# 4paradigm/OpenEmbedding

Measured on AMD Instinct MI355X. Metric: samples/sec DeepFM Criteo, higher is better.
Workload: dtype bf16; 1 GPU; model=deepfm-dim9, global_batch=4096, fields=26, dense_features=13, optimizer=adagrad, graph=True, prefetch=False, table=array, cache_mb=0, parallelism=single-gpu

## Files before the change

### openembedding_amd/core/tiered_gpu.py

```python

from __future__ import annotations

from typing import Optional

import torch

from .variable import VariableMeta, VariableShard
from .variable_gpu import HipVariableShard


class HipTieredVariableShard(HipVariableShard):
    HOST_INITIAL_ROWS = 1 << 14
    HOST_INITIAL_TABLE = 1 << 16

    def __init__(self, meta: VariableMeta, shard_id: int = 0,
                 shard_num: int = 1, device: str = "cuda", seed: int = 0,
                 cache_rows: int = 1 << 22):
        if not meta.use_hash_table:
            raise ValueError("the capacity tier requires hash mode")
        super().__init__(meta, shard_id, shard_num, device, seed)
        self.cache_rows = int(cache_rows)
        self.work_id = 0
        dev = self.device
        self._touch = torch.zeros(self.weights.shape[0] + 1,
                                  dtype=torch.int64, device=dev)
        self._host_cap = self.HOST_INITIAL_TABLE
        self.host_tk = torch.full((self._host_cap,), -1, dtype=torch.int64,
                                  device=dev)
        self.host_tv = torch.empty(self._host_cap, dtype=torch.int32,
                                   device=dev)
        self.host_nrows_dev = torch.zeros(1, dtype=torch.int32, device=dev)
        self.host_slot_keys = torch.empty(self.HOST_INITIAL_ROWS,
                                          dtype=torch.int64, device=dev)
        pin = torch.cuda.is_available()
        self._host_weights = torch.zeros((self.HOST_INITIAL_ROWS, self.dim),
                                         dtype=self.dtype, pin_memory=pin)
        self._host_state = torch.zeros((self.HOST_INITIAL_ROWS, 0),
                                       dtype=self.dtype, pin_memory=pin)
        self._host_rows_upper = 0
        self._host_live = False
        self._faulted = torch.zeros(1, dtype=torch.int32, device=dev)
        self._evict_epoch = 0
        self._last_batch_upper = 0
        self._evict_streak = 0
        self._checkpoint_work_id = None
        self._cache_full_since_ckpt = False


    def _host_ensure(self, rows: int) -> None:
        cap = self._host_weights.shape[0]
        if rows <= cap:
            return
        new_cap = max(rows, cap * 2)
        torch.cuda.synchronize()
        pin = torch.cuda.is_available()
        hw = torch.zeros((new_cap, self.dim), dtype=self.dtype,
                         pin_memory=pin)
        hw[:cap] = self._host_weights
        self._host_weights = hw
        hs = torch.zeros((new_cap, self._host_state.shape[1]),
                         dtype=self.dtype, pin_memory=pin)
        hs[:cap] = self._host_state
        self._host_state = hs
        sk = torch.empty(new_cap, dtype=torch.int64, device=self.device)
        sk[:self.host_slot_keys.shape[0]] = self.host_slot_keys
        self.host_slot_keys = sk

    def _host_maybe_rehash(self) -> None:
        if self._host_rows_upper * 2 <= self._host_cap:
            return
        new_cap = self._host_cap
        while self._host_rows_upper * 2 > new_cap:
            new_cap *= 2
        tk_new = torch.empty(new_cap, dtype=torch.int64, device=self.device)
        tv_new = torch.empty(new_cap, dtype=torch.int32, device=self.device)
        self.ext.ht_rehash(self.host_tk, self.host_tv, tk_new, tv_new)
        self.host_tk, self.host_tv = tk_new, tv_new
        self._host_cap = new_cap

    def set_optimizer(self, category: str, **cfg) -> None:
        super().set_optimizer(category, **cfg)
        if self._host_state.shape[1] != self.state_dim:
            if self._host_live:
                raise RuntimeError("cannot change optimizer state layout "
                                   "after rows were spilled to the host "
                                   "tier")
            pin = torch.cuda.is_available()
            self._host_state = torch.zeros(
                (self._host_weights.shape[0], self.state_dim),
                dtype=self.dtype, pin_memory=pin)

    def _ensure_rows(self, need: int) -> None:
        super()._ensure_rows(need)
        if self._touch.numel() < self.weights.shape[0] + 1:
            t = torch.zeros(self.weights.shape[0] + 1, dtype=torch.int64,
                            device=self.device)
            t[:self._touch.numel()] = self._touch
            self._touch = t

    def reserve_rows(self, rows: int) -> None:
        super().reserve_rows(min(int(rows), self.cache_rows))


    def _lookup_or_insert(self, keys: torch.Tensor, u_dev=None):
        if self._in_graph_capture():
            raise RuntimeError("the capacity tier is not hipGraph-"
                               "capturable (evictions need host control); "
                               "run eager with prefetch overlap")
        slots, new_mask = super()._lookup_or_insert(keys, u_dev)
        if self._host_live:
            self.ext.fault_in(keys, u_dev, self.host_tk, self.host_tv,
                              self._host_weights,
                              self._host_state if self.state_dim else None,
                              self.weights, self.state, slots, new_mask,
                              self._faulted)
        self._touch.scatter_(0, slots + 1, self.work_id)
        slots._oe_epoch = self._evict_epoch
        self._last_batch_upper = max(self._last_batch_upper, keys.numel())
        return slots, new_mask

    def push_slots(self, keys_buf, u_dev, slots, grads, counts) -> None:
        if getattr(slots, "_oe_epoch", self._evict_epoch) != self._evict_epoch:
            raise RuntimeError(
                "stale pull handle: the cache was compacted (eviction) "
                "after this pull; pull handles must be pushed before the "
                "commit that follows them")
        super().push_slots(keys_buf, u_dev, slots, grads, counts)

    def pull_readonly(self, keys: torch.Tensor) -> torch.Tensor:
        slots = self._lookup_readonly(keys)
        empty = torch.empty(0, dtype=torch.uint8, device=self.device)
        out = self.ext.gather_init(self.weights, self.state, slots, empty,
                                   keys, None, 0, 0.0, 0.0, 0.0, self.seed,
                                   torch.empty(0, dtype=self.dtype,
                                               device=self.device), True,
                                   None)
        if self._host_live:
            self.ext.gather_host(keys, slots, self.host_tk, self.host_tv,
                                 self._host_weights, out)
        return out

    fused_pooled_readonly = False

    def pull_pooled_readonly(self, values: torch.Tensor,
                             offsets: torch.Tensor, mode: str,
                             weights: torch.Tensor = None) -> torch.Tensor:
        return VariableShard.pull_pooled_readonly(self, values, offsets,
                                                  mode, weights)

    def update_weights(self) -> None:
        super().update_weights()
        self.work_id += 1
        if self._nrows_upper + self._last_batch_upper > self.cache_rows:
            self._evict()
        else:
            self._evict_streak = 0


    def _sync_nrows(self) -> None:
        self._nrows_exact = int(self.nrows_dev.item())
        self._nrows_upper = self._nrows_exact

    def _spill(self, evict_slots: torch.Tensor) -> None:
        n_ev = evict_slots.numel()
        if n_ev == 0:
            return
        keys = self.host_keys_of_slots(evict_slots)
        self._host_ensure(self._host_rows_upper + n_ev)
        self._host_rows_upper += n_ev
        self._host_maybe_rehash()
        hslots, _ = self.ext.ht_lookup(self.host_tk, self.host_tv, keys,
                                       self.host_nrows_dev,
                                       self.host_slot_keys, True, None)
        self.ext.spill_rows(evict_slots, hslots, self.weights, self.state,
                            self._host_weights,
                            self._host_state if self.state_dim else None)
        self._host_live = True
        self._host_rows_upper = int(self.host_nrows_dev.item())

    def host_keys_of_slots(self, slots: torch.Tensor) -> torch.Tensor:
        return self.slot_keys.index_select(0, slots)

    def _evict(self) -> None:
        self._sync_nrows()
        n = self._nrows_exact
        margin = self._last_batch_upper
        if n + margin <= self.cache_rows:
            return
        self._evict_streak += 1
        keep_frac = 4 if self._evict_streak >= 4 else (4 * 3)
        keep_target = max(1, (self.cache_rows * keep_frac) // 16 - margin)
        n_evict = n - keep_target
        if n_evict <= 0:
            return
        self._cache_full_since_ckpt = True
        touches = self._touch[1:n + 1]
        evict_slots = torch.topk(touches, n_evict, largest=False,
                                 sorted=False).indices
        evict_mask = torch.zeros(n, dtype=torch.bool, device=self.device)
        evict_mask[evict_slots] = True
        self._spill(evict_slots)
        keep_slots = (~evict_mask).nonzero(as_tuple=True)[0]
        kk = self.slot_keys.index_select(0, keep_slots)
        kw = self.weights.index_select(0, keep_slots)
        ks = (self.state.index_select(0, keep_slots)
              if self.state_dim else None)
        kt = touches.index_select(0, keep_slots)
        self.tk.fill_(-1)
        self.nrows_dev.zero_()
        self._nrows_upper = 0
        self._nrows_exact = 0
        m = keep_slots.numel()
        if m:
            slots, _ = self.ext.ht_lookup(self.tk, self.tv, kk,
                                          self.nrows_dev, self.slot_keys,
                                          True, None)
            self.weights[slots] = kw
            if ks is not None:
                self.state[slots] = ks
            self._touch.zero_()
            self._touch.scatter_(0, slots + 1, kt)
            self._nrows_exact = m
            self._nrows_upper = m
        else:
            self._touch.zero_()
        self._evict_epoch += 1


    def fault_count(self) -> int:
        return int(self._faulted.item())


    def should_persist(self) -> bool:
        return self._cache_full_since_ckpt and self._checkpoint_work_id is None

    def persist(self) -> int:
        self._sync_nrows()
        n = self._nrows_exact
        if n:
            self._spill(torch.arange(n, dtype=torch.int64,
                                     device=self.device))
        self._checkpoint_work_id = self.work_id
        self._cache_full_since_ckpt = False
        return self.work_id

    def checkpoint_committed(self) -> None:
        self._checkpoint_work_id = None

    def _host_only(self):
        hn = int(self.host_nrows_dev.item())
        if hn == 0:
            e = torch.empty(0, dtype=torch.int64, device=self.device)
            return e, e
        hkeys = self.host_slot_keys[:hn]
        cache_slots, _ = self.ext.ht_lookup(self.tk, self.tv, hkeys,
                                            self.nrows_dev, self.slot_keys,
                                            False, None)
        mask = cache_slots < 0
        return hkeys[mask], torch.arange(hn, device=self.device)[mask]

    @property
    def num_rows(self) -> int:
        n = int(self.nrows_dev.item())
        hkeys, _ = self._host_only()
        return n + hkeys.numel()

    def export_rows(self, include_state: bool = True):
        keys_c, w_c, s_c = super().export_rows(include_state)
        hkeys, hslots = self._host_only()
        if hkeys.numel() == 0:
            return keys_c, w_c, s_c
        hs_cpu = hslots.cpu()
        keys = torch.cat([keys_c, hkeys])
# ... 24 lines not shown
```

### openembedding_amd/core/variable_gpu.py

```python

from __future__ import annotations

from typing import Optional, Tuple

import torch

from ..ops import require_hip
from .variable import VariableMeta, VariableShard

_OPT_IDS = {"default": 0, "adadelta": 1, "adagrad": 2, "adam": 3,
            "adamax": 4, "ftrl": 5, "rmsprop": 6, "sgd": 7, "test": 8}

_INIT_IDS = {"constant": 0, "uniform": 1, "normal": 2}


def _opt_cfg_vector(opt) -> list:
    c = opt.cfg
    cat = opt.category
    if cat == "default":
        return [c["learning_rate"]]
    if cat == "adadelta":
        return [c["learning_rate"], c["rho"], c["epsilon"]]
    if cat == "adagrad":
        return [c["learning_rate"], c["initial_accumulator_value"], c["epsilon"]]
    if cat == "adam" or cat == "adamax":
        return [c["learning_rate"], c["beta_1"], c["beta_2"], c["epsilon"]]
    if cat == "ftrl":
        return [c["learning_rate"], c["l1_regularization_strength"],
                c["l2_regularization_strength"],
                c["l2_shrinkage_regularization_strength"],
                c["learning_rate_power"], c["beta"]]
    if cat == "rmsprop":
        return [c["learning_rate"], c["rho"], c["momentum"], c["epsilon"]]
    if cat == "sgd":
        return [c["learning_rate"], c["momentum"], 1.0 if c["nesterov"] else 0.0]
    if cat == "test":
        return [c["learning_rate"], c["flip"]]
    raise ValueError(cat)


def _init_params(init) -> Tuple[int, float, float, float]:
    cat = _INIT_IDS[init.category]
    c = init.cfg
    if init.category == "constant":
        return cat, c["value"], 0.0, 0.0
    if init.category == "uniform":
        return cat, c["minval"], c["maxval"], 0.0
    return cat, c["mean"], c["stddev"], c["truncated"]


class HipVariableShard(VariableShard):

    INITIAL_TABLE_CAP = 1 << 16
    INITIAL_ROW_CAP = 1 << 14
    fused_pooled_readonly = True

    def __init__(self, meta: VariableMeta, shard_id: int = 0, shard_num: int = 1,
                 device: str = "cuda", seed: int = 0):
        self.ext = require_hip()
        if self.ext is None:
            raise RuntimeError("HIP extension missing (OEAMD_ALLOW_TORCH_FALLBACK "
                               "cannot be used with HipVariableShard)")
        if meta.dtype != torch.float32:
            raise NotImplementedError("GPU shards are float32 (reference default); "
                                      "float64 runs on the CPU backend")
        super().__init__(meta, shard_id, shard_num, device, seed)
        self._pending_bounded = []
        dev = self.device
        if meta.use_hash_table:
            self._cap = self.INITIAL_TABLE_CAP
            self.tk = torch.full((self._cap,), -1, dtype=torch.int64, device=dev)
            self.tv = torch.empty(self._cap, dtype=torch.int32, device=dev)
            self.nrows_dev = torch.zeros(1, dtype=torch.int32, device=dev)
            self.slot_keys = torch.empty(self.INITIAL_ROW_CAP, dtype=torch.int64,
                                         device=dev)
            self.weights = torch.zeros((self.INITIAL_ROW_CAP, self.dim),
                                       dtype=self.dtype, device=dev)
            self.state = torch.zeros((self.INITIAL_ROW_CAP, 0),
                                     dtype=self.dtype, device=dev)
            self._nrows_upper = 0
            self._nrows_exact = 0
        else:
            self.valid_u8 = torch.zeros(self._array_cap, dtype=torch.uint8,
                                        device=dev)
            del self.valid


    def _ensure_rows(self, need: int) -> None:
        cap = self.weights.shape[0]
        if need <= cap:
            return
        new_cap = max(need, cap * 2)
        for name in ("weights", "state"):
            old = getattr(self, name)
            neww = torch.zeros((new_cap, old.shape[1]), dtype=self.dtype,
                               device=self.device)
            neww[:cap] = old
            setattr(self, name, neww)
        sk = torch.empty(new_cap, dtype=torch.int64, device=self.device)
        sk[:self.slot_keys.shape[0]] = self.slot_keys
        self.slot_keys = sk
        if self._tracking:
            self._grow_row_epoch(new_cap)

    def _maybe_rehash(self) -> None:
        if self._nrows_upper * 2 <= self._cap:
            return
        new_cap = self._cap
        while self._nrows_upper * 2 > new_cap:
            new_cap *= 2
        tk_new = torch.empty(new_cap, dtype=torch.int64, device=self.device)
        tv_new = torch.empty(new_cap, dtype=torch.int32, device=self.device)
        self.ext.ht_rehash(self.tk, self.tv, tk_new, tv_new)
        self.tk, self.tv, self._cap = tk_new, tv_new, new_cap


    def reserve_rows(self, rows: int) -> None:
        rows = int(rows)
        self._ensure_rows(max(rows, 1024))
        want_cap = 1 << max(16, (2 * rows - 1).bit_length())
        if want_cap > self._cap:
            old_upper = self._nrows_upper
            self._nrows_upper = want_cap // 2
            self._maybe_rehash()
            self._nrows_upper = old_upper
        self._reserved_rows = rows

    def _lookup_or_insert(self, keys: torch.Tensor, u_dev=None):
        n = keys.numel()
        if self.meta.use_hash_table:
            if self._in_graph_capture():
                if getattr(self, "_reserved_rows", 0) <= 0:
                    raise RuntimeError(
                        "hash-table insert path is not hipGraph-capturable "
                        "without reserve_rows()")
            else:
                self._ensure_rows(self._nrows_upper + n)
                self._maybe_rehash()
                self._nrows_upper += n
            slots, new_mask = self.ext.ht_lookup(self.tk, self.tv, keys,
                                                 self.nrows_dev, self.slot_keys,
                                                 True, u_dev)
        else:
            slots, new_mask = self.ext.array_touch(self.valid_u8, keys,
                                                   self.shard_num, u_dev)
        if self._tracking:
            self._mark(slots, new_mask, u_dev)
        return slots, new_mask

    def _mark(self, slots, mask=None, u_dev=None) -> None:
        self.ext.mark_rows(slots, mask, u_dev, self.epoch_dev,
                           self.row_epoch)

    def _apply(self, opt_id, slots, grads, counts, cfg, u_dev) -> None:
        self.ext.apply_optimizer(opt_id, self.weights, self.state, slots,
                                 grads.contiguous(), counts, cfg, u_dev)
        if self._tracking:
            self._mark(slots, None, u_dev)

    def _lookup_readonly(self, keys: torch.Tensor) -> torch.Tensor:
        if self.meta.use_hash_table:
            slots, _ = self.ext.ht_lookup(self.tk, self.tv, keys,
                                          self.nrows_dev, self.slot_keys,
                                          False, None)
            return slots
        slots = torch.div(keys, self.shard_num, rounding_mode="floor")
        hit = self.valid_u8[slots.clamp(0, self._array_cap - 1)] != 0
        return torch.where(hit, slots, torch.full_like(slots, -1))


    def _gather(self, keys, slots, new_mask, want_out: bool,
                inverse=None, u_dev=None) -> torch.Tensor:
        cat, p0, p1, p2 = _init_params(self.initializer)
        sir = self._state_init_row
        if sir is None:
            sir = self._make_state_init_row()
            self._state_init_row = sir
        return self.ext.gather_init(self.weights, self.state, slots,
                                    new_mask if new_mask is not None
                                    else torch.empty(0, dtype=torch.uint8,
                                                     device=self.device),
                                    keys, inverse, cat, p0, p1, p2, self.seed,
                                    sir.reshape(-1), want_out, u_dev)

    def pull(self, keys: torch.Tensor) -> torch.Tensor:
        slots, new_mask = self._lookup_or_insert(keys)
        return self._gather(keys, slots, new_mask, True)

    def pull_bounded(self, keys_buf: torch.Tensor, u_dev: torch.Tensor,
                     inverse: torch.Tensor):
        slots, new_mask = self._lookup_or_insert(keys_buf, u_dev)
        out = self._gather(keys_buf, slots, new_mask, True,
                           inverse=inverse, u_dev=u_dev)
        return out, slots

    def pull_pooled_bounded(self, keys_buf: torch.Tensor,
                            u_dev: torch.Tensor, inverse: torch.Tensor,
                            offsets: torch.Tensor, mode: int,
                            weights: torch.Tensor = None):
        slots, new_mask = self._lookup_or_insert(keys_buf, u_dev)
        self._gather(keys_buf, slots, new_mask, False, u_dev=u_dev)
        if weights is not None:
            out, bag_of, bag_scale = self.ext.pool_fwd_weighted(
                self.weights, inverse, slots, offsets, weights, mode)
            return out, slots, bag_of, bag_scale
        out, bag_of = self.ext.pool_fwd(self.weights, inverse, slots,
                                        offsets, mode, True)
        return out, slots, bag_of

    def pool_wgrad_slots(self, inverse: torch.Tensor, slots: torch.Tensor,
                         weights: torch.Tensor, bag_of: torch.Tensor,
                         bag_scale: torch.Tensor, out: torch.Tensor,
                         grad_out: torch.Tensor, mode: int) -> torch.Tensor:
        return self.ext.pool_wgrad(self.weights, inverse, slots, weights,
                                   bag_of, bag_scale, out, grad_out, mode)

    def push_slots(self, keys_buf, u_dev, slots, grads, counts) -> None:
        self._pending_bounded.append((keys_buf, u_dev, slots, grads, counts))

    def pull_readonly(self, keys: torch.Tensor) -> torch.Tensor:
        slots = self._lookup_readonly(keys)
        empty = torch.empty(0, dtype=torch.uint8, device=self.device)
        return self.ext.gather_init(self.weights, self.state, slots, empty,
                                    keys, None, 0, 0.0, 0.0, 0.0, self.seed,
                                    torch.empty(0, dtype=self.dtype,
                                                device=self.device), True,
                                    None)

    def pull_pooled_readonly(self, values: torch.Tensor,
                             offsets: torch.Tensor, mode: str,
                             weights: torch.Tensor = None) -> torch.Tensor:
        from ..ops.dispatch import POOL_MODES
        if mode not in POOL_MODES:
            raise ValueError(f"unknown pooling mode {mode!r}")
        if weights is not None:
            weights = weights.to(self.dtype).contiguous()
        values = values.contiguous()
        offsets = offsets.contiguous()
        if self.meta.use_hash_table:
            return self.ext.pool_lookup(self.weights, values, offsets,
                                        POOL_MODES[mode], weights,
                                        tk=self.tk, tv=self.tv)
        return self.ext.pool_lookup(self.weights, values, offsets,
                                    POOL_MODES[mode], weights,
                                    valid=self.valid_u8,
                                    shard_num=self.shard_num)

    def update_weights(self) -> None:
        if not self._pending and not self._pending_bounded:
            return
        if self.optimizer is None:
            raise RuntimeError("update_weights called before set_optimizer")
        opt_id = _OPT_IDS[self.optimizer.category]
        cfg = _opt_cfg_vector(self.optimizer)
        blocks = self._pending_bounded
        self._pending_bounded = []
        if len(blocks) > 1:
            blocks = [self._merge_bounded(blocks)]
        for keys_buf, u_dev, slots, grads, counts in blocks:
            self._apply(opt_id, slots, grads, counts, cfg, u_dev)
        if self._pending:
            if len(self._pending) == 1:
                keys, grads, counts = self._pending[0]
            else:
                keys0 = torch.cat([b[0] for b in self._pending])
                grads0 = torch.cat([b[1] for b in self._pending])
                counts0 = torch.cat([b[2] for b in self._pending])
                keys, inv = self.ext.unique_inverse(keys0)
                grads, _ = self.ext.reduce_by_inverse(inv, grads0, keys.numel())
                counts = torch.zeros(keys.numel(), dtype=counts0.dtype,
                                     device=self.device)
                counts.index_add_(0, inv, counts0)
            self._pending = []
            slots, new_mask = self._lookup_or_insert(keys)
            self._gather(keys, slots, new_mask, False)
            self._apply(opt_id, slots, grads, counts, cfg, None)
        if self.meta.use_hash_table and not self._in_graph_capture():
            self._commits = getattr(self, "_commits", 0) + 1
            if self._commits % 16 == 0 or self._nrows_upper > (
                    self.weights.shape[0] * 3) // 4:
                self._nrows_exact = int(self.nrows_dev.item())
                self._nrows_upper = self._nrows_exact

    def _merge_bounded(self, blocks):
        ks, ps = [], []
        for keys_buf, u_dev, slots, grads, counts in blocks:
            self.ext.mask_tail(keys_buf, grads, counts, u_dev)
            ks.append(keys_buf)
            ps.append(torch.cat([grads,
                                 counts.to(grads.dtype).unsqueeze(1)],
                                dim=1))
        keys = torch.cat(ks)
        payload = torch.cat(ps)
        uk, inv, u_dev = self.ext.unique_bounded(keys)
        g2c, _ = self.ext.reduce_by_inverse(inv, payload.contiguous(),
                                            keys.numel())
        g2, c2 = self.ext.split_payload(g2c, u_dev)
        slots, new_mask = self._lookup_or_insert(uk, u_dev)
        self._gather(uk, slots, new_mask, False, u_dev=u_dev)
        return uk, u_dev, slots, g2, c2

    @staticmethod
    def _in_graph_capture() -> bool:
        try:
            return torch.cuda.is_current_stream_capturing()
        except Exception:
            return False


    @property
    def num_rows(self) -> int:
        if self.meta.use_hash_table:
            return int(self.nrows_dev.item())
        return int((self.valid_u8 != 0).sum())

    def export_rows(self, include_state: bool = True):
        if self.meta.use_hash_table:
            n = int(self.nrows_dev.item())
            keys = self.slot_keys[:n].clone()
            w = self.weights[:n].clone()
            s = self.state[:n].clone() if (include_state and self.state_dim) else None
            return keys, w, s
        slots = (self.valid_u8 != 0).nonzero(as_tuple=True)[0]
        keys = slots * self.shard_num + self.shard_id
        w = self.weights[slots].clone()
        s = self.state[slots].clone() if (include_state and self.state_dim) else None
        return keys, w, s

    def import_rows(self, keys, weights, state=None):
        slots, new_mask = self._lookup_or_insert(keys)
        self._gather(keys, slots, new_mask, False)
        self.weights[slots] = weights.to(self.device, self.dtype)
        if state is not None and self.state_dim:
            self.state[slots] = state.to(self.device, self.dtype)
        if self._tracking:
            self._mark(slots)
        if self.meta.use_hash_table:
            self._nrows_exact = int(self.nrows_dev.item())
            self._nrows_upper = self._nrows_exact

    def get_weights(self, keys):
        return self.pull_readonly(keys)

    def clear(self) -> None:
        if self.meta.use_hash_table:
            self.tk.fill_(-1)
            self.nrows_dev.zero_()
            self._nrows_upper = 0
            self._nrows_exact = 0
        else:
            self.valid_u8.zero_()
            self.weights.zero_()
            self.state.zero_()
        if self._tracking:
            self.row_epoch.zero_()


    def track_changes(self, enable: bool = True) -> None:
        was = self._tracking
        super().track_changes(enable)
        if enable and not was:
            self.epoch_dev = torch.ones(1, dtype=torch.int32,
                                        device=self.device)

    def set_epoch(self, epoch: int, reset: bool = False) -> None:
        super().set_epoch(epoch, reset)
        self.epoch_dev.fill_(self._epoch)

    def select_changed(self, since: int):
        self._need_tracking()
        if self.meta.use_hash_table:
            return self.ext.select_changed(self.row_epoch, int(since),
                                           nrows_dev=self.nrows_dev)
        return self.ext.select_changed(self.row_epoch, int(since),
                                       valid=self.valid_u8)

    def export_changed(self, since: int, include_state: bool = True,
                       selection=None):
        from .. import checkpoint
        slots, n_dev = selection if selection is not None \
            else self.select_changed(since)
        n = n_dev if isinstance(n_dev, int) else int(n_dev.item())
        if not n:
            return
        if isinstance(n_dev, int):
            n_dev = torch.full((1,), n, dtype=torch.int32,
                               device=self.device)
        step = min(int(checkpoint.BLOCK_ROWS), n)
        want_state = bool(include_state and self.state_dim)
        k_out = torch.empty(step, dtype=torch.int64, device=self.device)
        w_out = torch.empty((step, self.dim), dtype=self.dtype,
                            device=self.device)
        state = self.state if want_state else self.state[:, :0]
        s_out = torch.empty((step, state.shape[1]), dtype=self.dtype,
                            device=self.device)
        hashed = self.meta.use_hash_table
        for start in range(0, n, step):
            cnt = min(step, n - start)
            self.ext.gather_rows_by_slot(
                self.weights, state,
                slot_keys=self.slot_keys if hashed else None,
                shard_num=self.shard_num, shard_id=self.shard_id,
                slots=slots, start=start, count=cnt, n_dev=n_dev,
                keys_out=k_out, w_out=w_out, s_out=s_out)
            yield (k_out[:cnt], w_out[:cnt],
                   s_out[:cnt] if want_state else None)


    def set_optimizer(self, category: str, **cfg) -> None:
# ... 8 lines not shown
```

### openembedding_amd/ops/csrc/bindings.cpp

```cpp

#include <torch/extension.h>
#include <ATen/cuda/CUDAContext.h>
#include <c10/cuda/CUDAGuard.h>

#include <cstdint>
#include <tuple>
#include <vector>

typedef unsigned long long u64;
typedef int64_t i64;
typedef struct ihipStream_t* hipStream_t_;

extern "C" {
void emb_unique(const i64*, long, u64*, int*, long, int*, unsigned char*,
                i64*, i64*, int*, const i64*, int, hipStream_t_);
void emb_unique_indexed(const i64*, long, u64*, int*, long, int*,
                        unsigned char*, i64*, i64*, int*, const i64*, int,
                        int*, int*, int*, int*, int*, int*, int*, long, int*,
                        int*, hipStream_t_);
int emb_seg_threshold();
int emb_seg_max_dim();
void emb_reduce_by_index(const int*, const int*, const int*, const int*,
                         const int*, long, const float*, long, long,
                         const int*, float*, u64*, hipStream_t_);
void emb_ht_lookup(u64*, int*, long, const i64*, long, int*, i64*, i64*,
                   unsigned char*, int, const int*, long, hipStream_t_);
void emb_ht_rehash(const u64*, const int*, long, u64*, int*, long,
                   hipStream_t_);
void emb_array_touch(unsigned char*, const i64*, long, long, long, i64*,
                     unsigned char*, const int*, hipStream_t_);
void emb_gather_init(float*, float*, long, long, const i64*,
                     const unsigned char*, const i64*, long, const i64*,
                     float*, int, float, float, float, u64, const float*,
                     const int*, hipStream_t_);
void emb_reduce_by_inverse(const i64*, const float*, long, long, float*, u64*,
                           long, hipStream_t_);
void emb_reduce_bags_by_inverse(const i64*, const float*, long, long,
                                const int*, const i64*, long, int, float*,
                                u64*, long, hipStream_t_);
void emb_pool_fwd(const float*, long, long, const i64*, long, const void*,
                  int, long, const i64*, long, int, float*, int*,
                  hipStream_t_);
void emb_pool_fwd_weighted(const float*, long, long, const i64*, long,
                           const void*, int, long, const i64*, long, int,
                           const float*, float*, int*, float*, hipStream_t_);
void emb_reduce_bags_weighted_by_inverse(const i64*, const float*, long, long,
                                         const int*, const float*,
                                         const float*, long, float*, u64*,
                                         long, hipStream_t_);
void emb_pool_wgrad(const float*, long, long, const i64*, long, const void*,
                    int, long, const float*, const int*, const float*,
                    const float*, const float*, long, int, float*,
                    hipStream_t_);
void emb_pool_lookup(const float*, long, long, const i64*, long, const i64*,
                     long, int, const float*, const u64*, const int*, long,
                     const unsigned char*, long, float*, hipStream_t_);
long emb_quant_stride(int, long);
void emb_quantize_rows(int, const float*, long, long, const i64*, void*,
                       long, hipStream_t_);
void emb_pool_lookup_q(int, const void*, long, long, const i64*, long,
                       const i64*, long, int, const float*, const u64*,
                       const int*, long, const unsigned char*, long, float*,
                       hipStream_t_);
void emb_gather_lookup_q(int, const void*, long, long, const i64*, long,
                         const u64*, const int*, long, const unsigned char*,
                         long, float*, hipStream_t_);
void emb_apply_optimizer(int, float*, float*, long, long, const i64*, long,
                         const float*, const u64*, const float*, const int*,
                         hipStream_t_);
void emb_ctr_head_fwd(const float*, const float*, const float*, const float*, long,
                      long, long, long, long, void*, float*, float*, int,
                      int, hipStream_t_);
void emb_ctr_head_bwd(const float*, const float*, const float*, const void*,
                      const float*, const float*, long, long, long, long,
                      long, float*, float*, float*, float*, int, int,
                      hipStream_t_);
void emb_mlp3_bias_bwd(const float*, const void*, const void*, const void*,
                       const void*, long, long, float*, void*, void*, void*,
                       void*, void*, int, int, hipStream_t_);
void emb_mlp3_wgrad(const void*, const void*, const void*, const void*,
                    const void*, const void*, long, long, long, long,
                    float*, void*, void*, void*, float*, long, hipStream_t_);
void emb_mlp3_pack(const void*, void*, long, long, long, long, int,
                   const void*, void*, long, long, long, long, int,
                   const void*, void*, long, long, long, long, int,
                   hipStream_t_);
void emb_bce_fwd(const float*, const float*, long, float*, hipStream_t_);
void emb_bce_bwd(const float*, const float*, long, const float*, float*,
                 hipStream_t_);
void emb_bucketize_pad(const i64*, long, const int*, long, long, i64*, int*,
                       int*, int*, int*, hipStream_t_);
void emb_mask_tail(i64*, float*, u64*, long, long, const int*, hipStream_t_);
void emb_mark_rows(const i64*, long, const unsigned char*, const int*,
                   const int*, int*, long, hipStream_t_);
long emb_delta_tile_rows();
long emb_delta_tiles(long);
void emb_delta_count(const int*, long, int, const int*, const unsigned char*,
                     int*, hipStream_t_);
void emb_delta_compact(const int*, long, int, const int*,
                       const unsigned char*, const int*, i64*, hipStream_t_);
void emb_delta_gather(const float*, const float*, long, long, long,
                      const i64*, long, long, const i64*, long, long, long,
                      const int*, i64*, float*, float*, hipStream_t_);
void emb_fault_in(const i64*, long, const int*, const u64*, const int*, long,
                  const float*, const float*, float*, float*, long, long,
                  const i64*, unsigned char*, int*, hipStream_t_);
void emb_spill_rows(const i64*, const i64*, long, const float*, const float*,
                    float*, float*, long, long, hipStream_t_);
void emb_gather_host(const i64*, long, const i64*, const u64*, const int*,
                     long, const float*, float*, long, hipStream_t_);
void emb_gather_pad(const float*, const u64*, long, const int*, long, float*,
                    hipStream_t_);
void emb_scatter_out(const float*, const i64*, long, const int*, long, float*,
                     hipStream_t_);
void emb_split_payload(const float*, long, long, const int*, float*, u64*,
                       hipStream_t_);
void emb_flat_step_scalars(float*, float, float, hipStream_t_);
void emb_flat_opt(int, void*, float*, float*, float*, void*,
                  const float*, long, int, float, float, float, float,
                  hipStream_t_);
void emb_flat_adagrad_f32(float*, float*, const float*, long, float, float,
                          hipStream_t_);
void emb_flat_adagrad_bf16(float*, float*, const void*, void*, long, float,
                           float, hipStream_t_);
void emb_cin_fwd(const float*, const float*, const void*, float*, long,
                 long, long, long, long, hipStream_t_);
void emb_cin_dw(const void*, const void*, const void*, float*, long, long,
                long, long, long, hipStream_t_);
void emb_cin_dx(const float*, const void*, const float*, const float*,
                float*, float*, long, long, long, long, long, hipStream_t_);
void emb_mlp3_fwd(const void*, long, long, const void*, const void*,
                  const void*, const void*, const void*, const void*,
                  const void*, const void*, const float*, long, long, void*,
                  void*, void*, float*, int, int, hipStream_t_);
void emb_mlp3_bwd(const float*, long, long, const void*, const void*,
                  const void*, const void*, const void*, const void*,
                  const void*, long, long, void*, void*, void*, void*,
                  float*, int, int, hipStream_t_);
void emb_mlp3_pack_frag(int, const void* const*, void* const*, const long*,
                        const long*, const long*, const long*, const long*,
                        const int*, hipStream_t_);
}

namespace {

using OptTensor = c10::optional<torch::Tensor>;

hipStream_t_ cur_stream() {
    return reinterpret_cast<hipStream_t_>(
        at::cuda::getCurrentCUDAStream().stream());
}

long next_pow2(long x) {
    long p = 16;
    while (p < x) p <<= 1;
    return p;
}

const int* u_ptr(const OptTensor& u_dev) {
    if (!u_dev.has_value()) return nullptr;
    TORCH_CHECK(u_dev->dtype() == torch::kInt32, "u_dev must be int32");
    return u_dev->data_ptr<int>();
}

#define CHECK_GPU(t) TORCH_CHECK((t).is_cuda(), #t " must be on GPU")
#define CHECK_CONT(t) TORCH_CHECK((t).is_contiguous(), #t " must be contiguous")


std::vector<torch::Tensor> unique_bounded_impl(
    torch::Tensor keys, OptTensor field_offsets, bool indexed) {
    CHECK_GPU(keys); CHECK_CONT(keys);
    TORCH_CHECK(keys.dtype() == torch::kInt64);
    const i64* foff = nullptr;
    int F = 0;
    if (field_offsets.has_value() && field_offsets->numel()) {
        CHECK_GPU(*field_offsets); CHECK_CONT(*field_offsets);
        TORCH_CHECK(field_offsets->dtype() == torch::kInt64,
                    "field_offsets must be int64");
        TORCH_CHECK(keys.numel() % field_offsets->numel() == 0,
                    "keys length must be a multiple of field_offsets");
        foff = field_offsets->data_ptr<i64>();
        F = (int)field_offsets->numel();
    }
    const c10::cuda::CUDAGuard guard(keys.device());
    long n = keys.numel();
    auto opts_i64 = keys.options();
    auto opts_i32 = keys.options().dtype(torch::kInt32);
    auto opts_u8 = keys.options().dtype(torch::kUInt8);
    long cap = next_pow2(2 * n);
    auto tk = torch::empty({cap}, opts_i64);
    auto tv = torch::empty({cap}, opts_i32);
    auto slot_of = torch::empty({n}, opts_i32);
    auto is_first = torch::empty({n}, opts_u8);
    auto uk = torch::empty({n}, opts_i64);
    auto inverse = torch::empty({n}, opts_i64);
    auto counter = torch::empty({1}, opts_i32);
    if (!indexed) {
        emb_unique(keys.data_ptr<i64>(), n, (u64*)tk.data_ptr<i64>(),
                   tv.data_ptr<int>(), cap, slot_of.data_ptr<int>(),
                   is_first.data_ptr<uint8_t>(), uk.data_ptr<i64>(),
                   inverse.data_ptr<i64>(), counter.data_ptr<int>(), foff, F,
                   cur_stream());
        return {uk, inverse, counter};
    }
    TORCH_CHECK(n < (1L << 31), "unique_bounded_indexed: n must fit int32");
    auto tct = torch::empty({2, cap}, opts_i32);
    auto segs = torch::empty({4, n}, opts_i32);
    long long_cap = n / (emb_seg_threshold() + 1) + 1;
    auto long_list = torch::empty({long_cap}, opts_i32);
    auto ctr = torch::empty({32}, opts_i32);
    auto seg_off = segs.select(0, 0), seg_cnt = segs.select(0, 1);
    auto perm = segs.select(0, 2), rank = segs.select(0, 3);
    auto n_long = ctr.narrow(0, 16, 1);
    emb_unique_indexed(keys.data_ptr<i64>(), n, (u64*)tk.data_ptr<i64>(),
                       tv.data_ptr<int>(), cap, slot_of.data_ptr<int>(),
                       is_first.data_ptr<uint8_t>(), uk.data_ptr<i64>(),
                       inverse.data_ptr<i64>(), counter.data_ptr<int>(), foff,
                       F, tct.data_ptr<int>(), tct.data_ptr<int>() + cap,
                       rank.data_ptr<int>(), seg_off.data_ptr<int>(),
                       seg_cnt.data_ptr<int>(), perm.data_ptr<int>(),
                       long_list.data_ptr<int>(), long_cap,
                       ctr.data_ptr<int>(), n_long.data_ptr<int>(),
                       cur_stream());
    return {uk, inverse, counter, seg_off, seg_cnt, perm, long_list, n_long};
}

std::tuple<torch::Tensor, torch::Tensor, torch::Tensor> unique_bounded(
    torch::Tensor keys, OptTensor field_offsets) {
    auto r = unique_bounded_impl(keys, field_offsets, false);
    return {r[0], r[1], r[2]};
}

std::tuple<torch::Tensor, torch::Tensor, torch::Tensor, torch::Tensor,
           torch::Tensor, torch::Tensor, torch::Tensor, torch::Tensor>
unique_bounded_indexed(torch::Tensor keys, OptTensor field_offsets) {
    auto r = unique_bounded_impl(keys, field_offsets, true);
    return {r[0], r[1], r[2], r[3], r[4], r[5], r[6], r[7]};
}

std::tuple<torch::Tensor, torch::Tensor> unique_inverse(torch::Tensor keys) {
    auto r = unique_bounded(keys, c10::nullopt);
    long u = std::get<2>(r).item<int>();
    return {std::get<0>(r).narrow(0, 0, u), std::get<1>(r)};
}


std::tuple<torch::Tensor, torch::Tensor> ht_lookup(
    torch::Tensor tk, torch::Tensor tv, torch::Tensor keys,
    torch::Tensor nrows, torch::Tensor slot_keys, bool insert,
    OptTensor u_dev) {
    CHECK_GPU(keys); CHECK_CONT(keys);
    const c10::cuda::CUDAGuard guard(keys.device());
    long n = keys.numel();
    auto slots = torch::empty({n}, keys.options());
    auto new_mask = torch::empty({n}, keys.options().dtype(torch::kUInt8));
    if (n)
        emb_ht_lookup((u64*)tk.data_ptr<i64>(), tv.data_ptr<int>(),
                      tk.numel(), keys.data_ptr<i64>(), n,
                      nrows.data_ptr<int>(), slot_keys.data_ptr<i64>(),
                      slots.data_ptr<i64>(), new_mask.data_ptr<uint8_t>(),
                      insert ? 1 : 0, u_ptr(u_dev), slot_keys.numel(),
                      cur_stream());
    return {slots, new_mask};
}

void ht_rehash(torch::Tensor tk_old, torch::Tensor tv_old, torch::Tensor tk_new,
               torch::Tensor tv_new) {
    const c10::cuda::CUDAGuard guard(tk_old.device());
    emb_ht_rehash((u64*)tk_old.data_ptr<i64>(), tv_old.data_ptr<int>(),
                  tk_old.numel(), (u64*)tk_new.data_ptr<i64>(),
                  tv_new.data_ptr<int>(), tk_new.numel(), cur_stream());
}


std::tuple<torch::Tensor, torch::Tensor> array_touch(
    torch::Tensor valid, torch::Tensor keys, int64_t shard_num,
    OptTensor u_dev) {
    const c10::cuda::CUDAGuard guard(valid.device());
    long n = keys.numel();
    auto slots = torch::empty({n}, keys.options());
    auto new_mask = torch::empty({n}, keys.options().dtype(torch::kUInt8));
    if (n)
        emb_array_touch(valid.data_ptr<uint8_t>(), keys.data_ptr<i64>(), n,
                        shard_num, valid.numel(), slots.data_ptr<i64>(),
                        new_mask.data_ptr<uint8_t>(), u_ptr(u_dev),
                        cur_stream());
    return {slots, new_mask};
}


torch::Tensor gather_init(torch::Tensor weights, torch::Tensor state,
                          torch::Tensor slots, torch::Tensor new_mask,
                          torch::Tensor keys, OptTensor inverse,
                          int64_t init_cat, double p0, double p1, double p2,
                          int64_t seed, torch::Tensor state_init_row,
                          bool want_out, OptTensor u_dev) {
    CHECK_GPU(weights); CHECK_CONT(weights);
    const c10::cuda::CUDAGuard guard(weights.device());
    long n = inverse.has_value() ? inverse->numel() : keys.numel();
    long dim = weights.size(1);
    long sd = state.numel() ? state.size(1) : 0;
    torch::Tensor out;
    float* out_ptr = nullptr;
    if (want_out) {
        out = torch::empty({n, dim}, weights.options());
        out_ptr = out.data_ptr<float>();
    } else {
        out = torch::empty({0}, weights.options());
    }
    if (init_cat == 1) p1 = p1 - p0;
    emb_gather_init(weights.data_ptr<float>(),
                    sd ? state.data_ptr<float>() : nullptr, dim, sd,
                    slots.data_ptr<i64>(),
                    new_mask.numel() ? new_mask.data_ptr<uint8_t>() : nullptr,
                    keys.data_ptr<i64>(), n,
                    inverse.has_value() ? inverse->data_ptr<i64>() : nullptr,
                    out_ptr, (int)init_cat,
                    (float)p0, (float)p1, (float)p2, (u64)seed,
                    sd ? state_init_row.data_ptr<float>() : nullptr,
                    u_ptr(u_dev), cur_stream());
    return out;
}


std::tuple<torch::Tensor, torch::Tensor> reduce_by_inverse(
    torch::Tensor inverse, torch::Tensor grads, int64_t u) {
    CHECK_GPU(grads); CHECK_CONT(grads);
    TORCH_CHECK(grads.dtype() == torch::kFloat32,
                "reduce_by_inverse: grads must be float32");
    const c10::cuda::CUDAGuard guard(grads.device());
    long n = grads.size(0);
    long dim = grads.size(1);
    auto ugrads = torch::empty({u, dim}, grads.options());
    auto counts = torch::empty({u}, grads.options().dtype(torch::kInt64));
    emb_reduce_by_inverse(inverse.data_ptr<i64>(), grads.data_ptr<float>(), n,
                          dim, ugrads.data_ptr<float>(),
                          (u64*)counts.data_ptr<i64>(), u, cur_stream());
    return {ugrads, counts};
}

std::tuple<torch::Tensor, torch::Tensor> reduce_by_index(
    torch::Tensor seg_off, torch::Tensor seg_cnt, torch::Tensor perm,
    torch::Tensor long_list, torch::Tensor n_long, torch::Tensor grads,
    torch::Tensor u_dev) {
    CHECK_GPU(grads); CHECK_CONT(grads);
    TORCH_CHECK(grads.dtype() == torch::kFloat32 && grads.dim() == 2,
                "reduce_by_index: grads must be float32 [n, dim]");
    long n = grads.size(0);
    long dim = grads.size(1);
    TORCH_CHECK(dim <= emb_seg_max_dim(),
                "reduce_by_index: dim above the kernel's ladder");
    for (const auto* t : {&seg_off, &seg_cnt, &perm, &long_list, &n_long,
                          &u_dev}) {
        CHECK_GPU(*t); CHECK_CONT(*t);
        TORCH_CHECK(t->dtype() == torch::kInt32,
                    "reduce_by_index: index tensors must be int32");
    }
    TORCH_CHECK(seg_off.numel() == n && seg_cnt.numel() == n
                && perm.numel() == n,
                "reduce_by_index: index does not match grads");
    TORCH_CHECK(n_long.numel() == 1 && u_dev.numel() == 1);
    const c10::cuda::CUDAGuard guard(grads.device());
    auto ugrads = torch::empty({n, dim}, grads.options());
    auto counts = torch::empty({n}, grads.options().dtype(torch::kInt64));
    emb_reduce_by_index(seg_off.data_ptr<int>(), seg_cnt.data_ptr<int>(),
                        perm.data_ptr<int>(), long_list.data_ptr<int>(),
                        n_long.data_ptr<int>(), long_list.numel(),
                        grads.data_ptr<float>(), n, dim,
                        u_dev.data_ptr<int>(), ugrads.data_ptr<float>(),
                        (u64*)counts.data_ptr<i64>(), cur_stream());
    return {ugrads, counts};
}


std::tuple<torch::Tensor, torch::Tensor> pool_fwd(
    torch::Tensor rows, OptTensor inverse, OptTensor map,
    torch::Tensor offsets, int64_t mode, bool want_bag_of) {
    CHECK_GPU(rows); CHECK_CONT(rows);
    CHECK_GPU(offsets); CHECK_CONT(offsets);
    TORCH_CHECK(rows.dtype() == torch::kFloat32 && rows.dim() == 2,
                "pool_fwd: rows must be float32 [R, dim]");
    TORCH_CHECK(offsets.dtype() == torch::kInt64 && offsets.dim() == 1
                && offsets.numel() >= 1,
                "pool_fwd: offsets must be int64 [B+1]");
    TORCH_CHECK(mode >= 0 && mode <= 2, "pool_fwd: bad mode");
    const void* map_ptr = nullptr;
    int map_kind = 0;
    long u = 0;
    if (map.has_value()) {
        CHECK_GPU(*map); CHECK_CONT(*map);
        u = map->numel();
        if (map->dtype() == torch::kInt64) {
            map_kind = 1;
            map_ptr = map->data_ptr<i64>();
        } else {
            TORCH_CHECK(map->dtype() == torch::kInt32,
                        "pool_fwd: map must be int64 or int32");
            map_kind = 2;
            map_ptr = map->data_ptr<int>();
        }
    }
    long R = rows.size(0), dim = rows.size(1);
    long nnz = map_kind ? u : R;
    const i64* inv_ptr = nullptr;
    if (inverse.has_value()) {
        CHECK_GPU(*inverse); CHECK_CONT(*inverse);
        TORCH_CHECK(inverse->dtype() == torch::kInt64,
                    "pool_fwd: inverse must be int64");
        nnz = inverse->numel();
        inv_ptr = inverse->data_ptr<i64>();
    }
    const c10::cuda::CUDAGuard guard(rows.device());
    long B = offsets.numel() - 1;
    auto out = torch::empty({B, dim}, rows.options());
    auto bag_of = torch::empty({want_bag_of ? nnz : 0},
                               rows.options().dtype(torch::kInt32));
    emb_pool_fwd(rows.data_ptr<float>(), R, dim, inv_ptr, nnz, map_ptr,
                 map_kind, u, offsets.data_ptr<i64>(), B, (int)mode,
                 out.data_ptr<float>(),
                 want_bag_of ? bag_of.data_ptr<int>() : nullptr,
                 cur_stream());
    return {out, bag_of};
}

std::tuple<torch::Tensor, torch::Tensor> reduce_bags_by_inverse(
    torch::Tensor inverse, torch::Tensor grad_out, torch::Tensor bag_of,
    torch::Tensor offsets, int64_t mode, int64_t u) {
    CHECK_GPU(grad_out); CHECK_CONT(grad_out);
    CHECK_GPU(inverse); CHECK_CONT(inverse);
    CHECK_GPU(bag_of); CHECK_CONT(bag_of);
    CHECK_GPU(offsets); CHECK_CONT(offsets);
    TORCH_CHECK(grad_out.dtype() == torch::kFloat32 && grad_out.dim() == 2,
                "reduce_bags_by_inverse: grad_out must be float32 [B, dim]");
    TORCH_CHECK(inverse.dtype() == torch::kInt64
                && bag_of.dtype() == torch::kInt32
                && offsets.dtype() == torch::kInt64,
                "reduce_bags_by_inverse dtypes");
    TORCH_CHECK(bag_of.numel() == inverse.numel(),
                "reduce_bags_by_inverse: bag_of/inverse length mismatch");
    TORCH_CHECK(offsets.numel() == grad_out.size(0) + 1,
                "reduce_bags_by_inverse: offsets must be [B+1]");
    TORCH_CHECK(mode >= 0 && mode <= 2, "reduce_bags_by_inverse: bad mode");
    const c10::cuda::CUDAGuard guard(grad_out.device());
    long n = inverse.numel();
    long B = grad_out.size(0);
    long dim = grad_out.size(1);
    auto ugrads = torch::empty({u, dim}, grad_out.options());
    auto counts = torch::empty({u}, grad_out.options().dtype(torch::kInt64));
    emb_reduce_bags_by_inverse(inverse.data_ptr<i64>(),
                               grad_out.data_ptr<float>(), n, dim,
                               bag_of.data_ptr<int>(),
                               offsets.data_ptr<i64>(), B, (int)mode,
                               ugrads.data_ptr<float>(),
                               (u64*)counts.data_ptr<i64>(), u,
                               cur_stream());
    return {ugrads, counts};
}


struct PoolChain {
    const i64* inv_ptr = nullptr;
    const void* map_ptr = nullptr;
    int map_kind = 0;
    long u = 0, nnz = 0;
};

static PoolChain pool_chain(const char* who, const torch::Tensor& rows,
                            const OptTensor& inverse, const OptTensor& map) {
    PoolChain c;
    if (map.has_value()) {
        CHECK_GPU(*map); CHECK_CONT(*map);
        c.u = map->numel();
        if (map->dtype() == torch::kInt64) {
            c.map_kind = 1;
            c.map_ptr = map->data_ptr<i64>();
        } else {
            TORCH_CHECK(map->dtype() == torch::kInt32, who,
                        ": map must be int64 or int32");
            c.map_kind = 2;
            c.map_ptr = map->data_ptr<int>();
        }
    }
    c.nnz = c.map_kind ? c.u : rows.size(0);
    if (inverse.has_value()) {
        CHECK_GPU(*inverse); CHECK_CONT(*inverse);
        TORCH_CHECK(inverse->dtype() == torch::kInt64, who,
                    ": inverse must be int64");
        c.nnz = inverse->numel();
        c.inv_ptr = inverse->data_ptr<i64>();
    }
    return c;
}

std::tuple<torch::Tensor, torch::Tensor, torch::Tensor> pool_fwd_weighted(
    torch::Tensor rows, OptTensor inverse, OptTensor map,
    torch::Tensor offsets, torch::Tensor weights, int64_t mode,
    OptTensor out_buf, OptTensor scale_buf) {
    CHECK_GPU(rows); CHECK_CONT(rows);
    CHECK_GPU(offsets); CHECK_CONT(offsets);
    CHECK_GPU(weights); CHECK_CONT(weights);
    TORCH_CHECK(rows.dtype() == torch::kFloat32 && rows.dim() == 2
                && rows.size(1) >= 1,
                "pool_fwd_weighted: rows must be float32 [R, dim >= 1]");
    TORCH_CHECK(offsets.dtype() == torch::kInt64 && offsets.dim() == 1
                && offsets.numel() >= 1,
                "pool_fwd_weighted: offsets must be int64 [B+1]");
    TORCH_CHECK(mode >= 0 && mode <= 2, "pool_fwd_weighted: bad mode");
    PoolChain c = pool_chain("pool_fwd_weighted", rows, inverse, map);
    TORCH_CHECK(weights.dtype() == torch::kFloat32 && weights.dim() == 1
                && weights.numel() == c.nnz,
                "pool_fwd_weighted: weights must be float32 [nnz]");
    const c10::cuda::CUDAGuard guard(rows.device());
    long R = rows.size(0), dim = rows.size(1);
    long B = offsets.numel() - 1;
    auto out = out_buf.has_value() ? *out_buf
                                   : torch::empty({B, dim}, rows.options());
    auto bag_scale = scale_buf.has_value()
        ? *scale_buf : torch::empty({B}, rows.options());
    CHECK_GPU(out); CHECK_CONT(out);
    CHECK_GPU(bag_scale); CHECK_CONT(bag_scale);
    TORCH_CHECK(out.dtype() == torch::kFloat32 && out.dim() == 2
                && out.size(0) == B && out.size(1) == dim,
                "pool_fwd_weighted: out must be float32 [B, dim]");
    TORCH_CHECK(bag_scale.dtype() == torch::kFloat32
// ... 860 lines not shown
    for (size_t i = 0; i < n; i++) {
        const torch::Tensor &s = srcs[i], &d = dsts[i];
        CHECK_GPU(s); CHECK_GPU(d); CHECK_CONT(d);
        TORCH_CHECK(s.dtype() == torch::kBFloat16
                    && d.dtype() == torch::kBFloat16
                    && s.dim() == 2 && d.dim() == 2 && s.stride(1) == 1
                    && s.stride(0) >= s.size(1)
                    && s.device() == d.device(),
                    "mlp3_pack_frag dtypes/shapes");
        rows[i] = s.size(0); cols[i] = s.size(1); sld[i] = s.stride(0);
        N[i] = d.size(0); Kp[i] = d.size(1);
        tt[i] = trans[i];
        TORCH_CHECK(N[i] > 0 && N[i] % 16 == 0 && Kp[i] > 0
                    && Kp[i] % 32 == 0,
                    "mlp3_pack_frag: dst must be [x16, x32]");
        TORCH_CHECK((tt[i] ? cols[i] : rows[i]) <= N[i]
                    && (tt[i] ? rows[i] : cols[i]) <= Kp[i],
                    "mlp3_pack_frag: dst too small");
        TORCH_CHECK(N[i] * Kp[i] < (1L << 31)
                    && rows[i] * sld[i] < (1L << 31),
                    "mlp3_pack_frag: 32-bit indices");
        TORCH_CHECK((reinterpret_cast<uintptr_t>(d.data_ptr()) & 15) == 0,
                    "mlp3_pack_frag: dst must be 16-byte aligned");
        sp[i] = s.data_ptr(); dp[i] = d.data_ptr();
    }
    const c10::cuda::CUDAGuard guard(srcs[0].device());
    emb_mlp3_pack_frag((int)n, sp, dp, rows, cols, sld, N, Kp, tt,
                       cur_stream());
}


torch::Tensor bce_fwd(torch::Tensor logits, torch::Tensor labels) {
    CHECK_GPU(logits); CHECK_CONT(logits); CHECK_CONT(labels);
    TORCH_CHECK(logits.dtype() == torch::kFloat32 &&
                labels.dtype() == torch::kFloat32, "bce_fwd wants fp32");
    TORCH_CHECK(logits.numel() == labels.numel(), "logits/labels mismatch");
    const c10::cuda::CUDAGuard guard(logits.device());
    auto loss = torch::empty({}, logits.options());
    emb_bce_fwd(logits.data_ptr<float>(), labels.data_ptr<float>(),
                logits.numel(), loss.data_ptr<float>(), cur_stream());
    return loss;
}

torch::Tensor bce_bwd(torch::Tensor logits, torch::Tensor labels,
                      torch::Tensor grad_out) {
    CHECK_GPU(logits); CHECK_CONT(logits); CHECK_CONT(labels);
    TORCH_CHECK(grad_out.numel() == 1, "grad_out must be scalar");
    const c10::cuda::CUDAGuard guard(logits.device());
    auto g = torch::empty_like(logits);
    emb_bce_bwd(logits.data_ptr<float>(), labels.data_ptr<float>(),
                logits.numel(), grad_out.contiguous().data_ptr<float>(),
                g.data_ptr<float>(), cur_stream());
    return g;
}


std::tuple<torch::Tensor, torch::Tensor, torch::Tensor, torch::Tensor>
mlp3_fwd(torch::Tensor x0, torch::Tensor w1, torch::Tensor b1,
         torch::Tensor w2, torch::Tensor b2, torch::Tensor w3,
         torch::Tensor b3, torch::Tensor w4, torch::Tensor b4,
         c10::optional<torch::Tensor> partial, long bm, bool frag) {
    CHECK_GPU(x0); CHECK_CONT(x0);
    TORCH_CHECK(x0.dtype() == torch::kBFloat16, "mlp3_fwd: x0 must be bf16");
    const c10::cuda::CUDAGuard guard(x0.device());
    long M = x0.size(0), K0p = x0.size(1), H = w1.size(0);
    long Hp = w2.size(1);
    TORCH_CHECK(H % 16 == 0 && H <= 416, "mlp3_fwd: H must be <=416, x16");
    TORCH_CHECK(K0p % 32 == 0 && Hp % 32 == 0,
                "mlp3_fwd: padded K dims must be x32");
    TORCH_CHECK(w1.size(1) == K0p && w2.size(0) == H && w3.size(0) == H
                && w3.size(1) == Hp && w4.numel() == H);
    TORCH_CHECK(bm == 0 || bm == 16 || ((bm == 32 || bm == 64)
                                        && K0p <= 416),
                "mlp3_fwd: bm must be 0, 16, 32 or 64 (32/64: K0p <= 416)");
    if (frag) {
        CHECK_CONT(w1); CHECK_CONT(w2); CHECK_CONT(w3);
    }
    auto a1 = torch::empty({M, H}, x0.options());
    auto a2 = torch::empty({M, H}, x0.options());
    auto a3 = torch::empty({M, H}, x0.options());
    auto out = torch::empty({M}, x0.options().dtype(torch::kFloat32));
    const float* pp = nullptr;
    if (partial.has_value()) {
        TORCH_CHECK(partial->is_contiguous() && partial->numel() == M &&
                    partial->dtype() == torch::kFloat32,
                    "mlp3_fwd: partial must be contiguous fp32 [M]");
        pp = partial->data_ptr<float>();
    }
    emb_mlp3_fwd(x0.data_ptr(), M, K0p,
                 w1.data_ptr(), b1.data_ptr(), w2.data_ptr(), b2.data_ptr(),
                 w3.data_ptr(), b3.data_ptr(), w4.data_ptr(), b4.data_ptr(),
                 pp, H, Hp, a1.data_ptr(), a2.data_ptr(), a3.data_ptr(),
                 out.data_ptr<float>(), (int)bm, (int)frag, cur_stream());
    return {out, a1, a2, a3};
}

std::tuple<torch::Tensor, torch::Tensor, torch::Tensor, torch::Tensor>
mlp3_bwd(torch::Tensor dout, torch::Tensor a1, torch::Tensor a2,
         torch::Tensor a3, torch::Tensor w4, torch::Tensor w3t,
         torch::Tensor w2t, torch::Tensor w1t, OptTensor bias_scratch,
         long bm, bool frag) {
    CHECK_GPU(dout); CHECK_CONT(dout); CHECK_CONT(w3t); CHECK_CONT(w2t);
    CHECK_CONT(w1t);
    const c10::cuda::CUDAGuard guard(dout.device());
    long M = a1.size(0), H = a1.size(1), K0p = w1t.size(0);
    long Hp = w3t.size(1);
    TORCH_CHECK(Hp % 32 == 0 && w2t.size(1) == Hp && w1t.size(1) == Hp);
    TORCH_CHECK(H % 16 == 0 && H <= 416 && K0p % 16 == 0,
                "mlp3_bwd: H must be <=416, x16");
    TORCH_CHECK(bm == 0 || bm == 16 || bm == 32 || bm == 64,
                "mlp3_bwd: bm must be 0, 16, 32 or 64");
    auto dz1 = torch::empty_like(a1);
    auto dz2 = torch::empty_like(a2);
    auto dz3 = torch::empty_like(a3);
    auto dx0 = torch::empty({M, K0p}, a1.options());
    float* bptr = nullptr;
    if (bias_scratch.has_value()) {
        CHECK_CONT(*bias_scratch);
        TORCH_CHECK(bias_scratch->numel() >= 4 * H + 1
                    && bias_scratch->dtype() == torch::kFloat32,
                    "bias_scratch layout");
        bptr = bias_scratch->data_ptr<float>();
    }
    emb_mlp3_bwd(dout.data_ptr<float>(), M, K0p, a1.data_ptr(),
                 a2.data_ptr(), a3.data_ptr(), w4.data_ptr(), w3t.data_ptr(),
                 w2t.data_ptr(), w1t.data_ptr(), H, Hp, dz1.data_ptr(),
                 dz2.data_ptr(), dz3.data_ptr(), dx0.data_ptr(), bptr,
                 (int)bm, (int)frag, cur_stream());
    return {dx0, dz1, dz2, dz3};
}

}

PYBIND11_MODULE(TORCH_EXTENSION_NAME, m) {
    m.def("unique_inverse", &unique_inverse, "hash-based unique+inverse");
    m.def("unique_bounded", &unique_bounded,
          "unique+inverse without host sync (n-sized buffer + device "
          "count); optional fused per-field key offsets",
          pybind11::arg("keys"),
          pybind11::arg("field_offsets") = pybind11::none());
    m.def("ht_lookup", &ht_lookup, "hash table lookup/insert");
    m.def("ht_rehash", &ht_rehash, "hash table rehash into larger table");
    m.def("array_touch", &array_touch,
          "array-table slot compute + valid-bitmap touch");
    m.def("gather_init", &gather_init,
          "row gather with fused lazy init (+ optional duplicate scatter)");
    m.def("reduce_by_inverse", &reduce_by_inverse,
          "grad reduce-by-key with counts (LDS-aggregated)");
    m.def("unique_bounded_indexed", &unique_bounded_indexed,
          "unique_bounded plus the batch's inverted index (seg_off, "
          "seg_cnt, perm, long_list, n_long)",
          pybind11::arg("keys"),
          pybind11::arg("field_offsets") = pybind11::none());
    m.def("reduce_by_index", &reduce_by_index,
          "grad reduce-by-key with counts through the inverted index "
          "(segmented, no atomics)");
    m.def("seg_reduce_threshold", &emb_seg_threshold,
          "list length above which a uid is in long_list");
    m.def("seg_reduce_max_dim", &emb_seg_max_dim,
          "widest dim reduce_by_index covers");
    m.def("pool_fwd", &pool_fwd,
          "segment-pooled gather (sum/mean/sqrtn) over ragged bags; also "
          "emits each element's bag for the backward",
          pybind11::arg("rows"), pybind11::arg("inverse"),
          pybind11::arg("map"), pybind11::arg("offsets"),
          pybind11::arg("mode"), pybind11::arg("want_bag_of") = true);
    m.def("reduce_bags_by_inverse", &reduce_bags_by_inverse,
          "grad reduce-by-key reading the pooled [B, dim] gradient through "
          "bag_of (no [nnz, dim] expansion)");
    m.def("pool_fwd_weighted", &pool_fwd_weighted,
          "pool_fwd with per-sample weights; also emits bag_of and the "
          "per-bag combiner scale for the backward",
          pybind11::arg("rows"), pybind11::arg("inverse"),
          pybind11::arg("map"), pybind11::arg("offsets"),
          pybind11::arg("weights"), pybind11::arg("mode"),
          pybind11::arg("out") = pybind11::none(),
          pybind11::arg("bag_scale") = pybind11::none());
    m.def("reduce_bags_weighted_by_inverse",
          &reduce_bags_weighted_by_inverse,
          "bag-indirected grad reduce with the per-element factor "
          "weights[e] * bag_scale[bag_of[e]]");
    m.def("pool_wgrad", &pool_wgrad,
          "gradient of the weighted pool w.r.t. its per-sample weights",
          pybind11::arg("rows"), pybind11::arg("inverse"),
          pybind11::arg("map"), pybind11::arg("weights"),
          pybind11::arg("bag_of"), pybind11::arg("bag_scale"),
          pybind11::arg("out"), pybind11::arg("grad_out"),
          pybind11::arg("mode"), pybind11::arg("dw") = pybind11::none());
    m.def("pool_lookup", &pool_lookup,
          "read-only pooled lookup, keys -> pooled rows in one launch "
          "(hash: tk/tv; array: valid/shard_num)",
          pybind11::arg("rows"), pybind11::arg("values"),
          pybind11::arg("offsets"), pybind11::arg("mode"),
          pybind11::arg("weights") = pybind11::none(),
          pybind11::arg("tk") = pybind11::none(),
          pybind11::arg("tv") = pybind11::none(),
          pybind11::arg("valid") = pybind11::none(),
          pybind11::arg("shard_num") = 1);
    m.def("quantize_rows", &quantize_rows,
          "fp32 rows -> packed rows at the given slots of a slab (slots "
          "unique within a call)",
          pybind11::arg("w"), pybind11::arg("slots"), pybind11::arg("slab"),
          pybind11::arg("fmt"));
    m.def("pool_lookup_q", &pool_lookup_q,
          "read-only pooled lookup over a packed slab, keys -> pooled fp32 "
          "rows in one launch (hash: tk/tv; array: valid/shard_num)",
          pybind11::arg("slab"), pybind11::arg("dim"), pybind11::arg("fmt"),
          pybind11::arg("values"), pybind11::arg("offsets"),
          pybind11::arg("mode"),
          pybind11::arg("weights") = pybind11::none(),
          pybind11::arg("tk") = pybind11::none(),
          pybind11::arg("tv") = pybind11::none(),
          pybind11::arg("valid") = pybind11::none(),
          pybind11::arg("shard_num") = 1);
    m.def("gather_lookup_q", &gather_lookup_q,
          "flat read over a packed slab, keys -> fp32 rows in one launch",
          pybind11::arg("slab"), pybind11::arg("dim"), pybind11::arg("fmt"),
          pybind11::arg("keys"),
          pybind11::arg("tk") = pybind11::none(),
          pybind11::arg("tv") = pybind11::none(),
          pybind11::arg("valid") = pybind11::none(),
          pybind11::arg("shard_num") = 1);
    m.def("apply_optimizer", &apply_optimizer, "fused sparse optimizer step");
    m.def("mask_tail", &mask_tail,
          "zero the garbage tail of a bounded block (enables multi-block "
          "merge by concatenation)");
    m.def("mark_rows", &mark_rows,
          "delta checkpoints: row_epoch[slot] = *epoch_dev for the named "
          "rows (optional byte mask and device count)",
          pybind11::arg("slots"), pybind11::arg("mask") = pybind11::none(),
          pybind11::arg("u_dev") = pybind11::none(),
          pybind11::arg("epoch_dev"), pybind11::arg("row_epoch"));
    m.attr("DELTA_TILE_ROWS") = emb_delta_tile_rows();
    m.def("select_changed", &select_changed,
          "delta checkpoints: ascending slots of the live rows with "
          "row_epoch >= since -> (slots [R] with a -1 tail, n_dev int32[1])",
          pybind11::arg("row_epoch"), pybind11::arg("since"),
          pybind11::arg("nrows_dev") = pybind11::none(),
          pybind11::arg("valid") = pybind11::none());
    m.def("gather_rows_by_slot", &gather_rows_by_slot,
          "delta checkpoints: keys, weights and state of "
          "slots[start:start+count] into staging buffers",
          pybind11::arg("weights"), pybind11::arg("state"),
          pybind11::arg("slot_keys") = pybind11::none(),
          pybind11::arg("shard_num") = 1, pybind11::arg("shard_id") = 0,
          pybind11::arg("slots"), pybind11::arg("start"),
          pybind11::arg("count"), pybind11::arg("n_dev"),
          pybind11::arg("keys_out") = pybind11::none(),
          pybind11::arg("w_out") = pybind11::none(),
          pybind11::arg("s_out") = pybind11::none());
    m.def("fault_in", &fault_in,
          "tier v2: copy host-resident rows into fresh cache slots, "
          "clearing their lazy-init mask");
    m.def("spill_rows", &spill_rows,
          "tier v2: copy cache rows into the pinned host slab");
    m.def("gather_host", &gather_host,
          "tier v2: read-only host-row gather for cache misses");
    m.def("bucketize_pad", &bucketize_pad,
          "owner-bucketize unique keys into a fixed padded [world, cap] "
          "wire block (sync-free multi-rank route)");
    m.def("gather_pad", &gather_pad,
          "gather grads+counts payload into the padded send layout");
    m.def("scatter_out", &scatter_out,
          "padded pull: wire rows -> per-element output (fused dup scatter)");
    m.def("split_payload", &split_payload,
          "split owner-reduced payload into grads + int64 counts");
    m.def("ctr_head_fwd", &ctr_head_fwd,
          "fused CTR head fwd: deep_in assembly (+cast) + FM + first-order "
          "+ dense linear");
    m.def("ctr_head_bwd", &ctr_head_bwd, "fused CTR head backward");
    m.def("mlp3_bwd", &mlp3_bwd,
          "fused dgrad chain backward of the 3-layer MLP (optionally "
          "carrying the head wgrad/bias sums)",
          pybind11::arg("dout"), pybind11::arg("a1"), pybind11::arg("a2"),
          pybind11::arg("a3"), pybind11::arg("w4"), pybind11::arg("w3t"),
          pybind11::arg("w2t"), pybind11::arg("w1t"),
          pybind11::arg("bias_scratch") = pybind11::none(),
          pybind11::arg("bm") = 0, pybind11::arg("frag") = false);
    m.def("mlp3_pack", &mlp3_pack,
          "refresh three padded (or transposed) weight copies in one "
          "launch");
    m.def("mlp3_pack_frag", &mlp3_pack_frag,
          "write up to six fragment-major weight images (pads included) "
          "in one launch",
          pybind11::arg("srcs"), pybind11::arg("dsts"),
          pybind11::arg("trans"));
    m.def("mlp3_fwd", &mlp3_fwd,
          "fused 3-hidden-layer MLP forward (bf16 MFMA, bias+ReLU fused)",
          pybind11::arg("x0"), pybind11::arg("w1"), pybind11::arg("b1"),
          pybind11::arg("w2"), pybind11::arg("b2"), pybind11::arg("w3"),
          pybind11::arg("b3"), pybind11::arg("w4"), pybind11::arg("b4"),
          pybind11::arg("partial"), pybind11::arg("bm") = 0,
          pybind11::arg("frag") = false);
    m.def("mlp3_wgrad", &mlp3_wgrad,
          pybind11::arg("dz1"), pybind11::arg("dz2"), pybind11::arg("dz3"),
          pybind11::arg("x0"), pybind11::arg("a1"), pybind11::arg("a2"),
          pybind11::arg("scratch"), pybind11::arg("dw1"),
          pybind11::arg("dw2"), pybind11::arg("dw3"),
          pybind11::arg("bias_scratch") = pybind11::none(),
          pybind11::arg("m_split") = 0,
          "all three MLP weight grads in one MFMA launch (+= into bf16 "
          "grads via fp32 scratch)");
    m.def("mlp3_bias_bwd", &mlp3_bias_bwd,
          "MLP bias grads + head wgrad in one pass over the dz mirrors "
          "(with_dz=false when the fused wgrad carried the dz sums)",
          pybind11::arg("dout"), pybind11::arg("dz1"), pybind11::arg("dz2"),
          pybind11::arg("dz3"), pybind11::arg("a3"),
          pybind11::arg("scratch"), pybind11::arg("db1"),
          pybind11::arg("db2"), pybind11::arg("db3"), pybind11::arg("dw4"),
// ... 19 lines not shown
```

### openembedding_amd/ops/csrc/embops.hip

```cpp

#include <hip/hip_runtime.h>
#include <cstdint>

#define DEV static __device__ __forceinline__

typedef unsigned long long u64;
typedef long long i64;

static constexpr u64 EMPTY = ~0ull;
static constexpr int BLOCK = 256;

static inline int cdiv(long a, long b) { return (int)((a + b - 1) / b); }
static inline int grid1d(long n) {
    long g = (n + BLOCK - 1) / BLOCK;
    return (int)(g < 1 ? 1 : g);
}


template <typename T>
__global__ void k_fill(T* __restrict__ p, long n, T v) {
    long i = (long)blockIdx.x * blockDim.x + threadIdx.x;
    if (i < n) p[i] = v;
}

// ... 31 lines not shown
    long i = (long)blockIdx.x * blockDim.x + threadIdx.x;
    if (i < cap) {
        tk[i] = ~0ull;
        if constexpr (IDX) ix.tcount[i] = 0;
    }
    if (i < n) is_first[i] = 0;
    if (i == 0) {
        *counter = 0;
        if constexpr (IDX) { *ix.off_counter = 0; *ix.n_long = 0; }
    }
}

__global__ void k_reduce_reset(float* __restrict__ ugrads, long ne,
                               u64* __restrict__ counts, long u) {
    long i = (long)blockIdx.x * blockDim.x + threadIdx.x;
    if (i < ne) ugrads[i] = 0.0f;
    if (i < u) counts[i] = 0ull;
}

__global__ void k_pad_reset(u64* __restrict__ send_keys,
                            int* __restrict__ send_src, long total,
                            int* __restrict__ counts, long world) {
    long i = (long)blockIdx.x * blockDim.x + threadIdx.x;
    if (i < total) { send_keys[i] = ~0ull; send_src[i] = -1; }
    if (i < world) counts[i] = 0;
}


DEV u64 splitmix64(u64 z) {
    z += 0x9E3779B97F4A7C15ull;
    z = (z ^ (z >> 30)) * 0xBF58476D1CE4E5B9ull;
    z = (z ^ (z >> 27)) * 0x94D049BB133111EBull;
    return z ^ (z >> 31);
}

DEV u64 uniform_bits(u64 seed, u64 key, u64 col, u64 attempt) {
    u64 x = key * 0x100000ull + col + (attempt << 40);
    return splitmix64(splitmix64(x) ^ seed);
}

DEV float uniform01(u64 seed, u64 key, u64 col, u64 attempt) {
    return (float)(uniform_bits(seed, key, col, attempt) >> 40)
           * (1.0f / 16777216.0f);
}

enum { INIT_CONSTANT = 0, INIT_UNIFORM = 1, INIT_NORMAL = 2 };

DEV float normal01(u64 seed, u64 key, u64 col, u64 attempt) {
    float u1 = uniform01(seed, key, col, 2 * attempt);
    float u2 = uniform01(seed, key, col, 2 * attempt + 1);
    float r = sqrtf(-2.0f * logf(1.0f - u1));
    return r * cosf(2.0f * 3.14159265358979323846f * u2);
}

DEV float init_value(int cat, float p0, float p1, float p2,
                     u64 seed, u64 key, u64 col) {
    if (cat == INIT_CONSTANT) return p0;
    if (cat == INIT_UNIFORM) {
        float u = uniform01(seed, key, col, 0);
        return p0 + u * p1;
    }
    float z = normal01(seed, key, col, 0);
    if (p2 > 0.1f) {
        for (int attempt = 1; attempt < 16 && z > p2; ++attempt)
            z = normal01(seed, key, col, attempt);
    }
    return p0 + p1 * z;
}


#define ULDS 1024
#define UA_ITERS 8
#define UI_ILP 4
#define SEG_T 32

template <bool IDX>
__global__ void k_unique_insert(const i64* __restrict__ keys, long n,
                                u64* __restrict__ tk, long mask,
                                int* __restrict__ slot_of,
                                unsigned char* __restrict__ is_first,
                                const i64* __restrict__ foff, int F,
                                UIdx ix) {
    __shared__ u64 lkeys[ULDS];
    __shared__ int lslot[ULDS];
    __shared__ int lcnt[IDX ? ULDS : 1];
    __shared__ int lbase[IDX ? ULDS : 1];
    for (int t = threadIdx.x; t < ULDS; t += blockDim.x) {
        lkeys[t] = EMPTY;
        if constexpr (IDX) lcnt[t] = 0;
    }
    __syncthreads();

    long i = (long)blockIdx.x * blockDim.x + threadIdx.x;
    u64 k = 0;
    i64 kin = 0;
    if (i < n) {
        kin = keys[i];
        if (foff) kin += foff[(int)i % F];
    }
    int lh = -1;
    int lr = 0;
    bool lds_winner = false, lds_ok = false;
    if (i < n && (u64)kin == EMPTY) {
        is_first[i] = 1;
        slot_of[i] = -1;
    } else if (i < n) {
        k = (u64)kin;
        u64 hh = splitmix64(k);
        lh = (int)(hh & (ULDS - 1));
        for (int probes = 0; probes < 64; ++probes) {
            u64 cur = atomicCAS(&lkeys[lh], EMPTY, k);
            if (cur == EMPTY) { lds_winner = true; lds_ok = true; break; }
            if (cur == k) { lds_ok = true; break; }
            lh = (lh + 1) & (ULDS - 1);
        }
        if constexpr (IDX)
            if (lds_ok) lr = atomicAdd(&lcnt[lh], 1);
        if (lds_winner || !lds_ok) {
            u64 h = splitmix64(k) & (u64)mask;
            long found = -1;
            for (long p = 0; p <= mask; ++p) {
                u64 cur = tk[h];
                if (cur == k) { found = (long)h; break; }
                if (cur == EMPTY) {
                    u64 prev = atomicCAS(&tk[h], EMPTY, k);
                    if (prev == EMPTY) {
                        is_first[i] = 1; found = (long)h; break;
                    }
                    if (prev == k) { found = (long)h; break; }
                }
                h = (h + 1) & (u64)mask;
            }
            if (found < 0) is_first[i] = 1;
            slot_of[i] = found >= 0 ? (int)found : -1;
            if (lds_winner)
                lslot[lh] = found >= 0 ? (int)found : (int)(-2 - i);
            if constexpr (IDX)
                if (!lds_ok && found >= 0)
                    lr = atomicAdd(&ix.tcount[found], 1);
        }
    }
    __syncthreads();
    if (i < n && lds_ok && !lds_winner) slot_of[i] = lslot[lh];
    if constexpr (IDX) {
        if (lds_winner) {
            int s = lslot[lh];
            lbase[lh] = s >= 0 ? atomicAdd(&ix.tcount[s], lcnt[lh]) : 0;
        }
        __syncthreads();
        if (i < n) ix.rank[i] = lds_ok ? lbase[lh] + lr : lr;
    }
}

template <bool IDX>
__global__ void k_unique_assign(const i64* __restrict__ keys, long n,
                                const int* __restrict__ slot_of,
                                const unsigned char* __restrict__ is_first,
                                int* __restrict__ tv,
                                i64* __restrict__ unique_keys,
                                int* __restrict__ counter,
                                i64* __restrict__ inverse,
                                const i64* __restrict__ foff, int F,
                                UIdx ix) {
    const int lane = threadIdx.x & 63;
    const long stride = (long)gridDim.x * blockDim.x;
    long i0 = (long)blockIdx.x * blockDim.x + threadIdx.x;
    u64 ballots[UA_ITERS];
    int sl[IDX ? UA_ITERS : 1], c[IDX ? UA_ITERS : 1];
    int total = 0;
    #pragma unroll
    for (int t = 0; t < UA_ITERS; ++t) {
        long i = i0 + t * stride;
        if constexpr (IDX) sl[t] = (i < n) ? slot_of[i] : -1;
        bool first = (i < n) && is_first[i];
        ballots[t] = __ballot(first);
        total += __popcll(ballots[t]);
    }
    if (!total) return;
    int off = 0, wtot = 0;
    if constexpr (IDX) {
        int ctot = 0;
        #pragma unroll
        for (int t = 0; t < UA_ITERS; ++t) {
            c[t] = (ballots[t] >> lane & 1ull)
                       ? (sl[t] >= 0 ? ix.tcount[sl[t]] : 1) : 0;
            ctot += c[t];
        }
        int inc = ctot;
        #pragma unroll
        for (int d = 1; d < 64; d <<= 1) {
            int v = __shfl_up(inc, d, 64);
            if (lane >= d) inc += v;
        }
        wtot = __shfl(inc, 63, 64);
        off = inc - ctot;
    }
    int base = 0, obase = 0;
    if (lane == 0) {
        base = atomicAdd(counter, total);
        if constexpr (IDX) obase = atomicAdd(ix.off_counter, wtot);
    }
    base = __shfl(base, 0, 64);
    if constexpr (IDX) off += __shfl(obase, 0, 64);
    #pragma unroll
    for (int t = 0; t < UA_ITERS; ++t) {
        u64 b = ballots[t];
        if (b & (1ull << lane)) {
            long i = i0 + t * stride;
            int uid = base + __popcll(b & ((1ull << lane) - 1ull));
            i64 kin = keys[i];
            if (foff) kin += foff[(int)i % F];
            unique_keys[uid] = kin;
            int s;
            if constexpr (IDX) s = sl[t]; else s = slot_of[i];
            if (s >= 0) tv[s] = uid;
            else inverse[i] = uid;
            if constexpr (IDX) {
                ix.seg_off[uid] = off;
                ix.seg_cnt[uid] = c[t];
                if (s >= 0) ix.toff[s] = off;
                else if (off >= 0 && off < n) ix.perm[off] = (int)i;
                if (c[t] > SEG_T) {
                    int q = atomicAdd(ix.n_long, 1);
                    if (q < ix.long_cap) ix.long_list[q] = uid;
                }
                off += c[t];
            }
        }
        base += __popcll(b);
    }
}

template <bool IDX>
__global__ void k_unique_inverse(long n, const int* __restrict__ slot_of,
                                 const int* __restrict__ tv,
                                 i64* __restrict__ inverse, UIdx ix) {
    const long stride = (long)gridDim.x * blockDim.x;
    long i0 = (long)blockIdx.x * blockDim.x + threadIdx.x;
    int s[UI_ILP];
    #pragma unroll
    for (int t = 0; t < UI_ILP; ++t) {
        long i = i0 + t * stride;
        s[t] = (i < n) ? slot_of[i] : -1;
    }
    int v[UI_ILP];
    int r[IDX ? UI_ILP : 1], o[IDX ? UI_ILP : 1];
    #pragma unroll
    for (int t = 0; t < UI_ILP; ++t) {
        v[t] = (s[t] >= 0) ? tv[s[t]] : 0;
        if constexpr (IDX) {
            o[t] = (s[t] >= 0) ? ix.toff[s[t]] : 0;
            r[t] = (s[t] >= 0) ? ix.rank[i0 + t * stride] : 0;
        }
    }
    #pragma unroll
    for (int t = 0; t < UI_ILP; ++t) {
        long i = i0 + t * stride;
        if (i >= n) continue;
        if constexpr (IDX) {
            long p = (long)o[t] + r[t];
            if (s[t] >= 0 && p >= 0 && p < n) ix.perm[p] = (int)i;
        }
        if (s[t] >= 0) inverse[i] = (i64)v[t];
        else if (s[t] <= -2) inverse[i] = inverse[-2 - s[t]];
    }
}


__global__ void k_ht_lookup(u64* __restrict__ tk, int* __restrict__ tv,
                            long mask, const i64* __restrict__ keys, long n,
                            int* __restrict__ nrows,
                            i64* __restrict__ slot_keys,
                            i64* __restrict__ slots,
                            unsigned char* __restrict__ new_mask,
                            int insert, const int* __restrict__ u_dev,
                            long row_cap) {
    long i = (long)blockIdx.x * blockDim.x + threadIdx.x;
    if (i >= n) return;
    if (u_dev && i >= *u_dev) {
        slots[i] = -1;
        if (new_mask) new_mask[i] = 0;
        return;
    }
    u64 k = (u64)keys[i];
    if (k == EMPTY) {
        slots[i] = -1;
        if (new_mask) new_mask[i] = 0;
        return;
    }
    u64 h = splitmix64(k) & (u64)mask;
    i64 slot = -1;
    unsigned char is_new = 0;
    for (long p = 0; p <= mask; ++p) {
        u64 cur = tk[h];
        if (cur == k) { slot = (i64)tv[h]; break; }
        if (cur == EMPTY) {
            if (!insert) { slot = -1; break; }
            u64 prev = atomicCAS(&tk[h], EMPTY, k);
            if (prev == EMPTY) {
                int s = atomicAdd(nrows, 1);
                if (s >= row_cap) {
                    tv[h] = -1;
                    slot = -1;
                    break;
                }
                tv[h] = s;
                slot_keys[s] = (i64)k;
                slot = s;
                is_new = 1;
                break;
            }
            if (prev == k) { slot = (i64)tv[h]; break; }
        }
        h = (h + 1) & (u64)mask;
    }
    slots[i] = slot;
    if (new_mask) new_mask[i] = is_new;
}

__global__ void k_ht_rehash(const u64* __restrict__ tk_old,
                            const int* __restrict__ tv_old, long cap_old,
                            u64* __restrict__ tk_new, int* __restrict__ tv_new,
                            long mask_new) {
    long i = (long)blockIdx.x * blockDim.x + threadIdx.x;
    if (i >= cap_old) return;
    u64 k = tk_old[i];
    if (k == EMPTY) return;
    u64 h = splitmix64(k) & (u64)mask_new;
    for (long p = 0; p <= mask_new; ++p) {
        u64 prev = atomicCAS(&tk_new[h], EMPTY, k);
        if (prev == EMPTY) { tv_new[h] = tv_old[i]; return; }
        h = (h + 1) & (u64)mask_new;
    }
}


__global__ void k_array_touch(unsigned char* __restrict__ valid,
                              const i64* __restrict__ keys, long n,
                              long shard_num, long cap,
                              i64* __restrict__ slots,
                              unsigned char* __restrict__ new_mask,
                              const int* __restrict__ u_dev) {
    long i = (long)blockIdx.x * blockDim.x + threadIdx.x;
    if (i >= n) return;
    if (u_dev && i >= *u_dev) { slots[i] = -1; new_mask[i] = 0; return; }
    if (keys[i] < 0) {
        slots[i] = -1;
        new_mask[i] = 0;
        return;
    }
    i64 s = keys[i] / shard_num;
    if (s < 0 || s >= cap) s = -1;
    slots[i] = s;
    if (s < 0) { new_mask[i] = 0; return; }
    unsigned char was = valid[s];
    valid[s] = 1;
    new_mask[i] = !was;
}


#define GI_ILP 4
template <int G>
__global__ void k_gather_init(float* __restrict__ weights,
                              float* __restrict__ state,
                              long dim, long sd,
                              const i64* __restrict__ slots,
                              const unsigned char* __restrict__ new_mask,
                              const i64* __restrict__ keys, long n,
                              const i64* __restrict__ inverse,
                              float* __restrict__ out,
                              int init_cat, float p0, float p1, float p2,
                              u64 seed,
                              const float* __restrict__ state_init_row,
                              const int* __restrict__ u_dev) {
    const long stride = ((long)gridDim.x * blockDim.x) / G;
    long g0 = ((long)blockIdx.x * blockDim.x + threadIdx.x) / G;
    const int lane = threadIdx.x % G;
    const int live = u_dev ? *u_dev : 0;

    long uid[GI_ILP];
    i64 slot[GI_ILP];
    unsigned char nm[GI_ILP];
    u64 key[GI_ILP];
    #pragma unroll
    for (int t = 0; t < GI_ILP; ++t) {
        long g = g0 + t * stride;
        bool act = g < n && !(!inverse && u_dev && g >= live);
        uid[t] = act ? (inverse ? inverse[g] : g) : -1;
    }
    #pragma unroll
    for (int t = 0; t < GI_ILP; ++t)
        slot[t] = (uid[t] >= 0) ? slots[uid[t]] : -1;
    #pragma unroll
    for (int t = 0; t < GI_ILP; ++t) {
        nm[t] = (uid[t] >= 0 && new_mask) ? new_mask[uid[t]] : 0;
        key[t] = (uid[t] >= 0 && nm[t]) ? (u64)keys[uid[t]] : 0;
    }
    #pragma unroll
    for (int t = 0; t < GI_ILP; ++t) {
        long g = g0 + t * stride;
        if (uid[t] < 0)
            continue;
        if (slot[t] < 0) {
            if (out)
                for (long j = lane; j < dim; j += G) out[g * dim + j] = 0.0f;
            continue;
        }
        float* wrow = weights + (u64)slot[t] * dim;
        if (nm[t]) {
            for (long j = lane; j < dim; j += G) {
                float v = init_value(init_cat, p0, p1, p2, seed, key[t],
                                     (u64)j);
                wrow[j] = v;
                if (out) out[g * dim + j] = v;
            }
            if (sd > 0) {
                float* srow = state + (u64)slot[t] * sd;
                for (long j = lane; j < sd; j += G)
                    srow[j] = state_init_row[j];
            }
        } else if (out) {
            for (long j = lane; j < dim; j += G)
                out[g * dim + j] = wrow[j];
        }
    }
}


enum { POOL_SUM = 0, POOL_MEAN = 1, POOL_SQRTN = 2 };

DEV long pool_clamp(i64 v, long nnz) {
    return v < 0 ? 0 : (v > (i64)nnz ? nnz : (long)v);
}

DEV float pool_scale(int mode, long len) {
    if (len <= 0) return 0.0f;
    if (mode == POOL_MEAN) return 1.0f / (float)len;
    if (mode == POOL_SQRTN) return 1.0f / sqrtf((float)len);
    return 1.0f;
}

DEV float pool_wscale(int mode, float den) {
    if (mode == POOL_SUM) return 1.0f;
    if (den == 0.0f) return 0.0f;
    return mode == POOL_MEAN ? 1.0f / den : 1.0f / sqrtf(den);
}


template <typename MapT>
DEV long pool_row(long j, long e, const i64* __restrict__ inverse,
                  const MapT* __restrict__ map, long nidx, long R) {
    if (j >= e) return -1;
    long uid = inverse ? (long)inverse[j] : j;
    if (uid < 0 || uid >= nidx) return -1;
    long row = map ? (long)map[uid] : uid;
    return (row >= 0 && row < R) ? row : -1;
}

template <typename MapT>
struct PoolChain {
    const i64* __restrict__ inverse;
    const MapT* __restrict__ map;
    long nidx, R;
    __device__ __forceinline__ long operator()(long j, long e) const {
        return pool_row(j, e, inverse, map, nidx, R);
    }
};

struct PoolHashKeys {
    const i64* __restrict__ values;
    const u64* __restrict__ tk;
    const int* __restrict__ tv;
    long mask, R;
    __device__ __forceinline__ long operator()(long j, long e) const {
        if (j >= e) return -1;
        const u64 k = (u64)values[j];
        if (k == EMPTY) return -1;
        u64 h = splitmix64(k) & (u64)mask;
        for (long p = 0; p <= mask; ++p) {
            const u64 cur = tk[h];
            if (cur == k) {
                const long row = (long)tv[h];
                return (row >= 0 && row < R) ? row : -1;
            }
            if (cur == EMPTY) return -1;
            h = (h + 1) & (u64)mask;
        }
        return -1;
    }
};

struct PoolArrayKeys {
    const i64* __restrict__ values;
    const unsigned char* __restrict__ valid;
    long shard_num, cap, R;
    __device__ __forceinline__ long operator()(long j, long e) const {
        if (j >= e) return -1;
        const i64 k = values[j];
        if (k < 0) return -1;
        const i64 slot = k / shard_num;
        if (slot >= cap || slot >= R) return -1;
        return valid[slot] ? (long)slot : -1;
    }
};

template <int G, int PF_CF, int PF_ILP, bool WEIGHTED, typename Resolve>
DEV void pool_accumulate(const float* __restrict__ rows, long dim, long s,
                         long e, long b, int lane, int mode,
                         const float* __restrict__ weights,
                         float* __restrict__ out,
                         float* __restrict__ bag_scale,
                         const Resolve& resolve) {
    float scale = 1.0f;
    if constexpr (!WEIGHTED) scale = pool_scale(mode, e - s);
    for (long c0 = 0; c0 < dim; c0 += (long)G * PF_CF) {
        float acc[PF_CF];
        #pragma unroll
        for (int k = 0; k < PF_CF; ++k) acc[k] = 0.0f;
        long myrow = resolve(s + lane, e);
        float myw = 0.0f, den = 0.0f;
        if constexpr (WEIGHTED)
            if (s + lane < e) myw = weights[s + lane];
        for (long j0 = s; j0 < e; j0 += G) {
            const long nextrow = resolve(j0 + G + lane, e);
            float nextw = 0.0f;
            if constexpr (WEIGHTED)
                if (j0 + G + lane < e) nextw = weights[j0 + G + lane];
            const int cnt = (int)((e - j0) < G ? (e - j0) : G);
            for (int t0 = 0; t0 < cnt; t0 += PF_ILP) {
                long row[PF_ILP];
                float wt[WEIGHTED ? PF_ILP : 1];
                #pragma unroll
                for (int t = 0; t < PF_ILP; ++t) {
                    row[t] = __shfl(myrow, t0 + t, G);
                    if constexpr (WEIGHTED) wt[t] = __shfl(myw, t0 + t, G);
                }
                float v[PF_ILP][PF_CF];
                #pragma unroll
                for (int t = 0; t < PF_ILP; ++t) {
                    #pragma unroll
                    for (int k = 0; k < PF_CF; ++k) {
                        long c = c0 + lane + (long)k * G;
                        v[t][k] = (row[t] >= 0 && c < dim)
                                      ? rows[(u64)row[t] * dim + c] : 0.0f;
                    }
                }
                #pragma unroll
                for (int t = 0; t < PF_ILP; ++t) {
                    if (t0 + t < cnt) {
                        if constexpr (WEIGHTED) {
                            #pragma unroll
                            for (int k = 0; k < PF_CF; ++k)
                                acc[k] += wt[t] * v[t][k];
                            den += (mode == POOL_SQRTN) ? wt[t] * wt[t]
                                                        : wt[t];
                        } else {
                            #pragma unroll
                            for (int k = 0; k < PF_CF; ++k) acc[k] += v[t][k];
                        }
                    }
                }
            }
            myrow = nextrow;
            if constexpr (WEIGHTED) myw = nextw;
// ... 545 lines not shown
                float v[LR_ILP][CF];
                #pragma unroll
                for (int t = 0; t < LR_ILP; ++t)
                    #pragma unroll
                    for (int c = 0; c < CF; ++c)
                        v[t][c] = (e[t] >= 0 && lane + c * G < dim)
                            ? grads[(u64)e[t] * dim + lane + c * G] : 0.0f;
                #pragma unroll
                for (int t = 0; t < LR_ILP; ++t)
                    #pragma unroll
                    for (int c = 0; c < CF; ++c) acc[c] += v[t][c];
            }
            #pragma unroll
            for (int d = G; d < 64; d <<= 1)
                #pragma unroll
                for (int c = 0; c < CF; ++c)
                    acc[c] += __shfl_xor(acc[c], d, 64);
            if ((threadIdx.x & 63) < G) {
                #pragma unroll
                for (int c = 0; c < CF; ++c)
                    red[threadIdx.x / 64][lane + c * G] = acc[c];
            }
            __syncthreads();
            if (threadIdx.x < G * CF) {
                float s = 0.0f;
                #pragma unroll
                for (int w = 0; w < SEG_BLOCK / 64; ++w)
                    s += red[w][threadIdx.x];
                if (threadIdx.x < dim)
                    ugrads[(u64)uid * dim + threadIdx.x] = s;
            }
            if (threadIdx.x == 0) counts[uid] = (u64)cnt;
            __syncthreads();
        }
        return;
    }

    const long ngroups = (long)(gridDim.x - long_blocks) * (SEG_BLOCK / G);
    const long g0 = ((long)(blockIdx.x - long_blocks) * SEG_BLOCK
                     + threadIdx.x) / G;
    int off[SR_ILP], cnt[SR_ILP], e0[SR_ILP];
    #pragma unroll
    for (int t = 0; t < SR_ILP; ++t) {
        long uid = g0 + t * ngroups;
        off[t] = 0;
        cnt[t] = 0;
        if (uid < u) seg_range(seg_off, seg_cnt, uid, n, off[t], cnt[t]);
    }
    #pragma unroll
    for (int t = 0; t < SR_ILP; ++t) {
        e0[t] = (cnt[t] > 0 && cnt[t] <= SEG_T) ? perm[off[t]] : -1;
        if (e0[t] < 0 || e0[t] >= n) e0[t] = -1;
    }
    float acc[SR_ILP][CF];
    #pragma unroll
    for (int t = 0; t < SR_ILP; ++t)
        #pragma unroll
        for (int c = 0; c < CF; ++c)
            acc[t][c] = (e0[t] >= 0 && lane + c * G < dim)
                ? grads[(u64)e0[t] * dim + lane + c * G] : 0.0f;
    #pragma unroll
    for (int t = 0; t < SR_ILP; ++t) {
        long uid = g0 + t * ngroups;
        if (uid >= n || cnt[t] > SEG_T) continue;
        for (int k = 1; k < cnt[t]; k += SR_ILP) {
            int e[SR_ILP];
            #pragma unroll
            for (int q = 0; q < SR_ILP; ++q) {
                e[q] = (k + q < cnt[t]) ? perm[off[t] + k + q] : -1;
                if (e[q] < 0 || e[q] >= n) e[q] = -1;
            }
            float v[SR_ILP][CF];
            #pragma unroll
            for (int q = 0; q < SR_ILP; ++q)
                #pragma unroll
                for (int c = 0; c < CF; ++c)
                    v[q][c] = (e[q] >= 0 && lane + c * G < dim)
                        ? grads[(u64)e[q] * dim + lane + c * G] : 0.0f;
            #pragma unroll
            for (int q = 0; q < SR_ILP; ++q)
                #pragma unroll
                for (int c = 0; c < CF; ++c) acc[t][c] += v[q][c];
        }
        #pragma unroll
        for (int c = 0; c < CF; ++c)
            if (lane + c * G < dim)
                ugrads[(u64)uid * dim + lane + c * G] = acc[t][c];
        if (lane == 0) counts[uid] = (u64)cnt[t];
    }
}

#define WG_ILP 4
template <int G, typename MapT>
__global__ void k_pool_wgrad(const float* __restrict__ rows, long R,
                             long dim, const i64* __restrict__ inverse,
                             long nnz, const MapT* __restrict__ map, long u,
                             const float* __restrict__ weights,
                             const int* __restrict__ bag_of,
                             const float* __restrict__ bag_scale,
                             const float* __restrict__ out,
                             const float* __restrict__ grad_out, long B,
                             int mode, float* __restrict__ dw) {
    const long e = ((long)blockIdx.x * blockDim.x + threadIdx.x) / G;
    const int lane = threadIdx.x % G;
    if (e >= nnz) return;
    const int bag = bag_of[e];
    if (bag < 0 || bag >= B) {
        if (lane == 0) dw[e] = 0.0f;
        return;
    }
    const long nidx = map ? u : R;
    const long row = pool_row(e, nnz, inverse, map, nidx, R);
    const float scale = bag_scale[bag];
    const float* __restrict__ g = grad_out + (u64)bag * dim;
    const float* __restrict__ o = out + (u64)bag * dim;
    const float* __restrict__ r = rows + (u64)(row >= 0 ? row : 0) * dim;
    const bool need_o = mode != POOL_SUM;
    float gr = 0.0f, go = 0.0f;
    for (long c0 = lane; c0 < dim; c0 += (long)G * WG_ILP) {
        float gv[WG_ILP], rv[WG_ILP], ov[WG_ILP];
        #pragma unroll
        for (int k = 0; k < WG_ILP; ++k) {
            const long c = c0 + (long)k * G;
            const bool in = c < dim;
            gv[k] = in ? g[c] : 0.0f;
            rv[k] = (in && row >= 0) ? r[c] : 0.0f;
            ov[k] = (in && need_o) ? o[c] : 0.0f;
        }
        #pragma unroll
        for (int k = 0; k < WG_ILP; ++k) {
            gr += gv[k] * rv[k];
            go += gv[k] * ov[k];
        }
    }
    #pragma unroll
    for (int m = G / 2; m > 0; m >>= 1) {
        gr += __shfl_xor(gr, m, G);
        go += __shfl_xor(go, m, G);
    }
    if (lane == 0) {
        float cj = 0.0f;
        if (mode == POOL_MEAN) cj = 1.0f;
        else if (mode == POOL_SQRTN) cj = weights[e] * scale;
        dw[e] = need_o ? scale * (gr - cj * go) : scale * gr;
    }
}


enum {
    OPT_DEFAULT = 0, OPT_ADADELTA = 1, OPT_ADAGRAD = 2, OPT_ADAM = 3,
    OPT_ADAMAX = 4, OPT_FTRL = 5, OPT_RMSPROP = 6, OPT_SGD = 7, OPT_TEST = 8
};

template <int G, int OPT>
__global__ void k_apply_opt(float* __restrict__ weights,
                            float* __restrict__ state,
                            long dim, long sd,
                            const i64* __restrict__ slots, long n,
                            const float* __restrict__ grads,
                            const u64* __restrict__ counts,
                            float c0, float c1, float c2, float c3,
                            float c4, float c5, float c6,
                            const int* __restrict__ u_dev) {
    long g = ((long)blockIdx.x * blockDim.x + threadIdx.x) / G;
    int lane = threadIdx.x % G;
    if (g >= n) return;
    if (u_dev && g >= *u_dev) return;
    i64 slot = slots[g];
    if (slot < 0) return;
    float* w = weights + (u64)slot * dim;
    float* s = state + (u64)slot * sd;
    const float* gr = grads + (u64)g * dim;

    if (OPT == OPT_DEFAULT) {
        const float lr = c0;
        if (lr != 0.0f)
            for (long j = lane; j < dim; j += G) w[j] -= lr * gr[j];
    } else if (OPT == OPT_ADADELTA) {
        const float lr = c0, rho = c1, eps = c2;
        float* accum = s;
        float* au = s + dim;
        for (long j = lane; j < dim; j += G) {
            float gj = gr[j];
            float a = accum[j] * rho + gj * gj * (1.0f - rho);
            accum[j] = a;
            float upd = gj * sqrtf(au[j] + eps) / sqrtf(a + eps);
            au[j] = au[j] * rho + upd * upd * (1.0f - rho);
            w[j] -= lr * upd;
        }
    } else if (OPT == OPT_ADAGRAD) {
        const float lr = c0, eps = c2;
        float* accum = s;
        for (long j = lane; j < dim; j += G) {
            float gj = gr[j];
            float a = accum[j] + gj * gj;
            accum[j] = a;
            w[j] -= lr * gj / (sqrtf(a) + eps);
        }
    } else if (OPT == OPT_ADAM) {
        const float lr = c0, b1 = c1, b2 = c2, eps = c3;
        float* m = s;
        float* v = s + dim;
        float lr_t = 0.0f;
        if (lane == 0) {
            float b1t = s[2 * dim] * b1;
            float b2t = s[2 * dim + 1] * b2;
            s[2 * dim] = b1t;
            s[2 * dim + 1] = b2t;
            lr_t = lr * sqrtf(1.0f - b2t) / (1.0f - b1t);
        }
        lr_t = __shfl(lr_t, 0, G);
        for (long j = lane; j < dim; j += G) {
            float gj = gr[j];
            float mj = m[j] * b1 + gj * (1.0f - b1);
            float vj = v[j] * b2 + gj * gj * (1.0f - b2);
            m[j] = mj; v[j] = vj;
            w[j] -= lr_t * mj / (sqrtf(vj) + eps);
        }
    } else if (OPT == OPT_ADAMAX) {
        const float lr = c0, b1 = c1, b2 = c2, eps = c3;
        float* m = s;
        float* v = s + dim;
        float lr_t = 0.0f;
        if (lane == 0) {
            float b1t = s[2 * dim] * b1;
            s[2 * dim] = b1t;
            lr_t = lr / (1.0f - b1t);
        }
        lr_t = __shfl(lr_t, 0, G);
        for (long j = lane; j < dim; j += G) {
            float gj = gr[j];
            float mj = m[j] * b1 + gj * (1.0f - b1);
            float vj = fmaxf(fabsf(gj), v[j] * b2);
            m[j] = mj; v[j] = vj;
            w[j] -= lr_t * mj / (vj + eps);
        }
    } else if (OPT == OPT_FTRL) {
        const float lr = c0, l1 = c1, l2 = c2, l2s = c3, lrp = c4, beta = c5;
        float* accum = s;
        float* linear = s + dim;
        const float adj_l2 = l2 + beta / lr / 2.0f;
        for (long j = lane; j < dim; j += G) {
            float gj = gr[j];
            float wj = w[j];
            float gg = gj + 2.0f * l2s * wj;
            float a_old = accum[j];
            float a_new = a_old + gj * gj;
            float sigma, quad;
            if (lrp == -0.5f) {
                sigma = (sqrtf(a_new) - sqrtf(a_old)) / lr;
                quad = sqrtf(a_new) / lr + 2.0f * adj_l2;
            } else {
                float p = -lrp;
                sigma = (powf(a_new, p) - powf(a_old, p)) / lr;
                quad = powf(a_new, p) / lr + 2.0f * adj_l2;
            }
            float lin = linear[j] + gg - sigma * wj;
            linear[j] = lin;
            accum[j] = a_new;
            float l1a = fminf(fmaxf(lin, -l1), l1);
            w[j] = (l1a - lin) / quad;
        }
    } else if (OPT == OPT_RMSPROP) {
        const float lr = c0, rho = c1, mom = c2, eps = c3;
        float* accum = s;
        float* moment = s + dim;
        for (long j = lane; j < dim; j += G) {
            float gj = gr[j];
            float a = accum[j] * rho + gj * gj * (1.0f - rho);
            accum[j] = a;
            float mo = moment[j] * mom + lr * gj / sqrtf(a + eps);
            moment[j] = mo;
            w[j] -= mo;
        }
    } else if (OPT == OPT_SGD) {
        const float lr = c0, mom = c1;
        const bool nesterov = c2 != 0.0f;
        float* moment = s;
        for (long j = lane; j < dim; j += G) {
            float gj = gr[j];
            float mo = moment[j] * mom + lr * gj;
            moment[j] = mo;
            w[j] -= nesterov ? (mo * mom + lr * gj) : mo;
        }
    } else if (OPT == OPT_TEST) {
        const float lr = c0, flip = c1;
        float s0 = 0.0f;
        if (lane == 0) {
            s0 = flip - s[0];
            s[0] = s0;
        }
        s0 = __shfl(s0, 0, G);
        float cnt = (float)counts[g];
        for (long j = lane; j < dim; j += G)
            w[j] += lr * gr[j] / cnt + s0;
    }
}


#include <hip/hip_bf16.h>
typedef __hip_bfloat16 oebf16;

__global__ void k_flat_adagrad_f32(float* __restrict__ p,
                                   float* __restrict__ accum,
                                   const float* __restrict__ g,
                                   long n, float lr, float eps) {
    long i = (long)blockIdx.x * blockDim.x + threadIdx.x;
    if (i >= n) return;
    float gi = g[i];
    float a = accum[i] + gi * gi;
    accum[i] = a;
    p[i] -= lr * gi / (sqrtf(a) + eps);
}

__global__ void k_flat_adagrad_bf16(float* __restrict__ master,
                                    float* __restrict__ accum,
                                    const oebf16* __restrict__ g,
                                    oebf16* __restrict__ p,
                                    long n, float lr, float eps) {
    long i = (long)blockIdx.x * blockDim.x + threadIdx.x;
    if (i >= n) return;
    float gi = (float)g[i];
    float a = accum[i] + gi * gi;
    accum[i] = a;
    float m = master[i] - lr * gi / (sqrtf(a) + eps);
    master[i] = m;
    p[i] = (oebf16)m;
}


enum { FLAT_SGD = 0, FLAT_ADAGRAD = 1, FLAT_ADAM = 2 };

__global__ void k_flat_step_scalars(float* __restrict__ sc, float b1,
                                    float b2) {
    if (threadIdx.x || blockIdx.x) return;
    float t = sc[0] + 1.0f;
    sc[0] = t;
    sc[1] = 1.0f - powf(b1, t);
    sc[2] = 1.0f - powf(b2, t);
}

template <int OPT>
__device__ __forceinline__ float flat_opt_step(
        float w, float gi, float* __restrict__ s1, float* __restrict__ s2,
        long i, const float* __restrict__ sc, float lr, float c0, float c1,
        float c2) {
    if (OPT == FLAT_ADAGRAD) {
        float a = s1[i] + gi * gi;
        s1[i] = a;
        return w - lr * gi / (sqrtf(a) + c0);
    }
    if (OPT == FLAT_SGD) {
        if (c0 == 0.0f) return w - lr * gi;
        float b = c0 * s1[i] + gi;
        s1[i] = b;
        float d = (c1 != 0.0f) ? gi + c0 * b : b;
        return w - lr * d;
    }
    float m = c0 * s1[i] + (1.0f - c0) * gi;
    float v = c1 * s2[i] + (1.0f - c1) * gi * gi;
    s1[i] = m;
    s2[i] = v;
    float mh = m / sc[1];
    float vh = v / sc[2];
    return w - lr * mh / (sqrtf(vh) + c2);
}

template <int OPT>
__global__ void k_flat_opt_f32(float* __restrict__ p,
                               float* __restrict__ s1,
                               float* __restrict__ s2,
                               float* __restrict__ g,
                               const float* __restrict__ sc, long n,
                               float lr, float c0, float c1, float c2) {
    long i = (long)blockIdx.x * blockDim.x + threadIdx.x;
    if (i >= n) return;
    p[i] = flat_opt_step<OPT>(p[i], g[i], s1, s2, i, sc, lr, c0, c1, c2);
    g[i] = 0.0f;
}

template <int OPT>
__global__ void k_flat_opt_bf16(float* __restrict__ master,
                                float* __restrict__ s1,
                                float* __restrict__ s2,
                                oebf16* __restrict__ g,
                                oebf16* __restrict__ p,
                                const float* __restrict__ sc, long n,
                                float lr, float c0, float c1, float c2) {
    long i = (long)blockIdx.x * blockDim.x + threadIdx.x;
    if (i >= n) return;
    float m = flat_opt_step<OPT>(master[i], (float)g[i], s1, s2, i, sc, lr,
                                 c0, c1, c2);
    master[i] = m;
    p[i] = (oebf16)m;
    g[i] = (oebf16)0.0f;
}


__global__ void k_bce_fwd(const float* __restrict__ z,
                          const float* __restrict__ y, long n, float inv_n,
                          float* __restrict__ loss) {
    long i = (long)blockIdx.x * blockDim.x + threadIdx.x;
    float v = 0.f;
    if (i < n) {
        float zi = z[i];
        v = (fmaxf(zi, 0.f) - zi * y[i] + log1pf(__expf(-fabsf(zi)))) * inv_n;
    }
    for (int off = 32; off; off >>= 1) v += __shfl_down(v, off);
    if ((threadIdx.x & 63) == 0 && v != 0.f) atomicAdd(loss, v);
}

__global__ void k_bce_fwd_1blk(const float* __restrict__ z,
                               const float* __restrict__ y, long n,
                               float inv_n, float* __restrict__ loss) {
    __shared__ float wsum[16];
    float v = 0.f;
    for (long i = threadIdx.x; i < n; i += blockDim.x) {
        float zi = z[i];
        v += (fmaxf(zi, 0.f) - zi * y[i]
              + log1pf(__expf(-fabsf(zi)))) * inv_n;
    }
    for (int off = 32; off; off >>= 1) v += __shfl_down(v, off);
    if ((threadIdx.x & 63) == 0) wsum[threadIdx.x >> 6] = v;
    __syncthreads();
    if (threadIdx.x == 0) {
        float t = 0.f;
        for (int w = 0; w < (int)(blockDim.x >> 6); ++w) t += wsum[w];
        *loss = t;
    }
}

__global__ void k_bce_bwd(const float* __restrict__ z,
                          const float* __restrict__ y, long n, float inv_n,
                          const float* __restrict__ go,
                          float* __restrict__ g) {
    long i = (long)blockIdx.x * blockDim.x + threadIdx.x;
    if (i >= n) return;
    float zi = z[i];
    float s = 1.f / (1.f + __expf(-zi));
    g[i] = (s - y[i]) * inv_n * go[0];
}


__global__ void k_bucketize_pad(const i64* __restrict__ keys, long n,
                                const int* __restrict__ u_dev, long world,
                                long cap,
                                i64* __restrict__ send_keys,
                                int* __restrict__ send_src,
// ... 300 lines not shown
                            int mode, hipStream_t stream,
                            const float* weights = nullptr,
                            const float* bag_scale = nullptr) {
    {
        long ne = u * dim;
        long mx = ne > u ? ne : u;
        if (mx) k_reduce_reset<<<(int)((mx + 255) / 256), 256, 0, stream>>>(
            ugrads, ne, counts, u);
    }
    if (n == 0) return;
    int grid = cdiv(n, BLOCK);
    if (dim <= 16) {
        const int H = 512;
        size_t smem = H * 8 + (size_t)H * dim * 4;
        k_reduce_lds<H, 8, 4, BAG, WEIGHTED><<<grid, BLOCK, smem, stream>>>(
            inverse, grads, n, dim, ugrads, counts, bag_of, offsets, B,
            mode, weights, bag_scale);
    } else if (dim <= 96) {
        const int H = 256;
        size_t smem = H * 8 + (size_t)H * dim * 4;
        k_reduce_lds<H, 16, 8, BAG, WEIGHTED><<<grid, BLOCK, smem, stream>>>(
            inverse, grads, n, dim, ugrads, counts, bag_of, offsets, B,
            mode, weights, bag_scale);
    } else if (dim <= 128) {
        const int H = 128;
        size_t smem = H * 8 + (size_t)H * dim * 4;
        k_reduce_lds<H, 64, 4, BAG, WEIGHTED><<<grid, BLOCK, smem, stream>>>(
            inverse, grads, n, dim, ugrads, counts, bag_of, offsets, B,
            mode, weights, bag_scale);
    } else {
        k_reduce_grads<BAG, WEIGHTED><<<grid1d(n * dim), BLOCK, 0, stream>>>(
            inverse, grads, n, dim, ugrads, bag_of, offsets, B, mode,
            weights, bag_scale);
        k_reduce_counts<BAG><<<grid1d(n), BLOCK, 0, stream>>>(
            inverse, n, counts, bag_of, B);
    }
}

template <bool WEIGHTED>
static void pool_dispatch(const float* rows, long R, long dim,
                          const i64* inverse, long nnz, const void* map,
                          int map_kind, long u, const i64* offsets, long B,
                          int mode, float* out, int* bag_of,
                          const float* weights, float* bag_scale,
                          hipStream_t stream) {
    if (B == 0 && (!bag_of || nnz == 0)) return;
#define LAUNCH_POOL(G, CF, ILP)                                             \
    do {                                                                    \
        int gg = grid1d((B > 0 ? B : 1) * G);                               \
        if (map_kind == 2)                                                  \
            k_pool_fwd<G, CF, ILP, int, WEIGHTED><<<gg, BLOCK, 0, stream>>>(\
                rows, R, dim, inverse, nnz, (const int*)map, u, offsets, B, \
                mode, out, bag_of, weights, bag_scale);                     \
        else                                                                \
            k_pool_fwd<G, CF, ILP, i64, WEIGHTED><<<gg, BLOCK, 0, stream>>>(\
                rows, R, dim, inverse, nnz,                                 \
                map_kind ? (const i64*)map : nullptr, u, offsets, B, mode,  \
                out, bag_of, weights, bag_scale);                           \
    } while (0)
    if (dim <= 16) LAUNCH_POOL(16, 1, 16);
    else if (dim <= 32) LAUNCH_POOL(16, 2, 8);
    else if (dim <= 64) LAUNCH_POOL(64, 1, 16);
    else if (dim <= 128) LAUNCH_POOL(64, 2, 8);
    else LAUNCH_POOL(64, 4, 4);
#undef LAUNCH_POOL
}

template <bool WEIGHTED, typename Resolve>
static void pool_lookup_dispatch(const float* rows, long dim, long nnz,
                                 const i64* offsets, long B, int mode,
                                 const float* weights, float* out,
                                 const Resolve& resolve,
                                 hipStream_t stream) {
    if (B == 0) return;
#define LAUNCH_LOOKUP(G, CF, ILP)                                           \
    k_pool_lookup<G, CF, ILP, WEIGHTED, Resolve>                            \
        <<<grid1d(B * G), BLOCK, 0, stream>>>(rows, dim, nnz, offsets, B,   \
                                              mode, weights, out, resolve)
    if (dim <= 16) LAUNCH_LOOKUP(16, 1, 16);
    else if (dim <= 32) LAUNCH_LOOKUP(16, 2, 8);
    else if (dim <= 64) LAUNCH_LOOKUP(64, 1, 16);
    else if (dim <= 128) LAUNCH_LOOKUP(64, 2, 8);
    else LAUNCH_LOOKUP(64, 4, 4);
#undef LAUNCH_LOOKUP
}

#define Q_ROW_LADDER(ndw, LAUNCH)                                           \
    do {                                                                    \
        if ((ndw) <= 4) LAUNCH(4);                                          \
        else if ((ndw) <= 16) LAUNCH(16);                                   \
        else if ((ndw) <= 32) LAUNCH(32);                                   \
        else LAUNCH(64);                                                    \
    } while (0)

template <int FMT>
static void quantize_dispatch(const float* w, long n, long dim,
                              const i64* slots, unsigned int* slab, long R,
                              hipStream_t stream) {
#define LAUNCH_QUANT(G)                                                     \
    k_quantize_rows<FMT, G><<<grid1d(n * G), BLOCK, 0, stream>>>(           \
        w, n, dim, slots, slab, R)
    Q_ROW_LADDER(QFmt<FMT>::code_dwords(dim), LAUNCH_QUANT);
#undef LAUNCH_QUANT
}

template <int FMT, bool WEIGHTED, typename Resolve>
static void pool_lookup_q_dispatch(const unsigned int* slab, long dim,
                                   long nnz, const i64* offsets, long B,
                                   int mode, const float* weights, float* out,
                                   const Resolve& resolve,
                                   hipStream_t stream) {
    if (B == 0) return;
#define LAUNCH_LOOKUP_Q(G, CF, ILP)                                         \
    k_pool_lookup_q<FMT, G, CF, ILP, WEIGHTED, Resolve>                     \
        <<<grid1d(B * G), BLOCK, 0, stream>>>(slab, dim, nnz, offsets, B,   \
                                              mode, weights, out, resolve)
    const long ndw = QFmt<FMT>::code_dwords(dim);
    if (ndw <= 16) LAUNCH_LOOKUP_Q(16, 1, 8);
    else if (ndw <= 32) LAUNCH_LOOKUP_Q(32, 1, 8);
    else if (ndw <= 64) LAUNCH_LOOKUP_Q(64, 1, 8);
    else LAUNCH_LOOKUP_Q(64, 2, 4);
#undef LAUNCH_LOOKUP_Q
}

template <int FMT, typename Resolve>
static void pool_lookup_q_fmt(const unsigned int* slab, long dim, long nnz,
                              const i64* offsets, long B, int mode,
                              const float* weights, float* out,
                              const Resolve& resolve, hipStream_t stream) {
    if (weights)
        pool_lookup_q_dispatch<FMT, true>(slab, dim, nnz, offsets, B, mode,
                                          weights, out, resolve, stream);
    else
        pool_lookup_q_dispatch<FMT, false>(slab, dim, nnz, offsets, B, mode,
                                           nullptr, out, resolve, stream);
}

template <int FMT, typename Resolve>
static void gather_lookup_q_fmt(const unsigned int* slab, long dim, long n,
                                float* out, const Resolve& resolve,
                                hipStream_t stream) {
#define LAUNCH_GATHER_Q(G)                                                  \
    k_gather_lookup_q<FMT, G, Resolve>                                      \
        <<<grid1d(n * G), BLOCK, 0, stream>>>(slab, dim, n, out, resolve)
    Q_ROW_LADDER(QFmt<FMT>::code_dwords(dim), LAUNCH_GATHER_Q);
#undef LAUNCH_GATHER_Q
}

template <bool IDX>
static void unique_launch(const i64* keys, long n, u64* tk, int* tv, long cap,
                          int* slot_of, unsigned char* is_first,
                          i64* unique_keys, i64* inverse, int* counter,
                          const i64* foff, int F, const UIdx& ix,
                          hipStream_t stream) {
    {
        long mx = cap > n ? cap : n;
        k_unique_reset<IDX><<<(int)((mx + 255) / 256), 256, 0, stream>>>(
            tk, cap, is_first, n, counter, ix);
    }
    long mask = cap - 1;
    k_unique_insert<IDX><<<grid1d(n), BLOCK, 0, stream>>>(
        keys, n, tk, mask, slot_of, is_first, foff, F, ix);
    int ga = grid1d((n + UA_ITERS - 1) / UA_ITERS);
    int gi = grid1d((n + UI_ILP - 1) / UI_ILP);
    k_unique_assign<IDX><<<ga, BLOCK, 0, stream>>>(
        keys, n, slot_of, is_first, tv, unique_keys, counter, inverse, foff,
        F, ix);
    k_unique_inverse<IDX><<<gi, BLOCK, 0, stream>>>(n, slot_of, tv, inverse,
                                                    ix);
}

extern "C" {

void emb_unique(const i64* keys, long n, u64* tk, int* tv, long cap,
                int* slot_of, unsigned char* is_first, i64* unique_keys,
                i64* inverse, int* counter, const i64* foff, int F,
                hipStream_t stream) {
    unique_launch<false>(keys, n, tk, tv, cap, slot_of, is_first,
                         unique_keys, inverse, counter, foff, F, UIdx{},
                         stream);
}

void emb_unique_indexed(const i64* keys, long n, u64* tk, int* tv, long cap,
                        int* slot_of, unsigned char* is_first,
                        i64* unique_keys, i64* inverse, int* counter,
                        const i64* foff, int F, int* tcount, int* toff,
                        int* rank, int* seg_off, int* seg_cnt, int* perm,
                        int* long_list, long long_cap, int* off_counter,
                        int* n_long, hipStream_t stream) {
    UIdx ix{tcount, toff, rank, seg_off, seg_cnt, perm, long_list,
            off_counter, n_long, long_cap};
    unique_launch<true>(keys, n, tk, tv, cap, slot_of, is_first, unique_keys,
                        inverse, counter, foff, F, ix, stream);
}

int emb_seg_threshold() { return SEG_T; }
int emb_seg_max_dim() { return SEG_MAX_DIM; }

void emb_reduce_by_index(const int* seg_off, const int* seg_cnt,
                         const int* perm, const int* long_list,
                         const int* n_long, long long_cap,
                         const float* grads, long n, long dim,
                         const int* u_dev, float* ugrads, u64* counts,
                         hipStream_t stream) {
    if (n == 0) return;
    int lb = (int)(long_cap < SEG_LONG_BLOCKS ? long_cap : SEG_LONG_BLOCKS);
    long groups = (n + SR_ILP - 1) / SR_ILP;
#define LAUNCH_SEG(G, CF)                                                   \
    k_seg_reduce<G, CF>                                                     \
        <<<lb + cdiv(groups * G, SEG_BLOCK), SEG_BLOCK, 0, stream>>>(       \
            seg_off, seg_cnt, perm, long_list, n_long, long_cap, lb, grads, \
            n, dim, u_dev, ugrads, counts)
    if (dim <= 16) LAUNCH_SEG(16, 1);
    else if (dim <= 32) LAUNCH_SEG(16, 2);
    else if (dim <= 64) LAUNCH_SEG(64, 1);
    else LAUNCH_SEG(64, 2);
#undef LAUNCH_SEG
}

void emb_ht_lookup(u64* tk, int* tv, long cap, const i64* keys, long n,
                   int* nrows, i64* slot_keys, i64* slots,
                   unsigned char* new_mask, int insert, const int* u_dev,
                   long row_cap, hipStream_t stream) {
    k_ht_lookup<<<grid1d(n), BLOCK, 0, stream>>>(tk, tv, cap - 1, keys, n,
                                                 nrows, slot_keys, slots,
                                                 new_mask, insert, u_dev,
                                                 row_cap);
}

void emb_ht_rehash(const u64* tk_old, const int* tv_old, long cap_old,
                   u64* tk_new, int* tv_new, long cap_new,
                   hipStream_t stream) {
    fill_u64(tk_new, cap_new, EMPTY, stream);
    k_ht_rehash<<<grid1d(cap_old), BLOCK, 0, stream>>>(
        tk_old, tv_old, cap_old, tk_new, tv_new, cap_new - 1);
}

void emb_array_touch(unsigned char* valid, const i64* keys, long n,
                     long shard_num, long cap, i64* slots,
                     unsigned char* new_mask, const int* u_dev,
                     hipStream_t stream) {
    k_array_touch<<<grid1d(n), BLOCK, 0, stream>>>(valid, keys, n, shard_num,
                                                   cap, slots, new_mask,
                                                   u_dev);
}

void emb_gather_init(float* weights, float* state, long dim, long sd,
                     const i64* slots, const unsigned char* new_mask,
                     const i64* keys, long n, const i64* inverse, float* out,
                     int init_cat, float p0, float p1, float p2, u64 seed,
                     const float* state_init_row, const int* u_dev,
                     hipStream_t stream) {
    if (n == 0) return;
    long npg = (n + GI_ILP - 1) / GI_ILP;
    if (dim <= 32) {
        int gg = grid1d(npg * 16);
        k_gather_init<16><<<gg, BLOCK, 0, stream>>>(
            weights, state, dim, sd, slots, new_mask, keys, n, inverse, out,
            init_cat, p0, p1, p2, seed, state_init_row, u_dev);
    } else {
        int gg = grid1d(npg * 64);
        k_gather_init<64><<<gg, BLOCK, 0, stream>>>(
            weights, state, dim, sd, slots, new_mask, keys, n, inverse, out,
            init_cat, p0, p1, p2, seed, state_init_row, u_dev);
    }
}

void emb_reduce_by_inverse(const i64* inverse, const float* grads, long n,
                           long dim, float* ugrads, u64* counts, long u,
                           hipStream_t stream) {
    reduce_dispatch<false>(inverse, grads, n, dim, ugrads, counts, u,
                           nullptr, nullptr, 0, 0, stream);
}

void emb_reduce_bags_by_inverse(const i64* inverse, const float* grad_out,
                                long n, long dim, const int* bag_of,
                                const i64* offsets, long B, int mode,
                                float* ugrads, u64* counts, long u,
                                hipStream_t stream) {
    reduce_dispatch<true>(inverse, grad_out, n, dim, ugrads, counts, u,
                          bag_of, offsets, B, mode, stream);
}

void emb_pool_fwd(const float* rows, long R, long dim, const i64* inverse,
                  long nnz, const void* map, int map_kind, long u,
                  const i64* offsets, long B, int mode, float* out,
                  int* bag_of, hipStream_t stream) {
    pool_dispatch<false>(rows, R, dim, inverse, nnz, map, map_kind, u,
                         offsets, B, mode, out, bag_of, nullptr, nullptr,
                         stream);
}

void emb_pool_fwd_weighted(const float* rows, long R, long dim,
                           const i64* inverse, long nnz, const void* map,
                           int map_kind, long u, const i64* offsets, long B,
                           int mode, const float* weights, float* out,
                           int* bag_of, float* bag_scale,
                           hipStream_t stream) {
    pool_dispatch<true>(rows, R, dim, inverse, nnz, map, map_kind, u,
                        offsets, B, mode, out, bag_of, weights, bag_scale,
                        stream);
}

void emb_pool_lookup(const float* rows, long R, long dim, const i64* values,
                     long nnz, const i64* offsets, long B, int mode,
                     const float* weights, const u64* tk, const int* tv,
                     long cap, const unsigned char* valid, long shard_num,
                     float* out, hipStream_t stream) {
    if (tk) {
        const PoolHashKeys r{values, tk, tv, cap - 1, R};
        if (weights)
            pool_lookup_dispatch<true>(rows, dim, nnz, offsets, B, mode,
                                       weights, out, r, stream);
        else
            pool_lookup_dispatch<false>(rows, dim, nnz, offsets, B, mode,
                                        nullptr, out, r, stream);
    } else {
        const PoolArrayKeys r{values, valid, shard_num, cap, R};
        if (weights)
            pool_lookup_dispatch<true>(rows, dim, nnz, offsets, B, mode,
                                       weights, out, r, stream);
        else
            pool_lookup_dispatch<false>(rows, dim, nnz, offsets, B, mode,
                                        nullptr, out, r, stream);
    }
}

long emb_quant_stride(int fmt, long dim) {
    return fmt == QF_INT8 ? QFmt<QF_INT8>::stride(dim)
                          : QFmt<QF_FP16>::stride(dim);
}

void emb_quantize_rows(int fmt, const float* w, long n, long dim,
                       const i64* slots, void* slab, long R,
                       hipStream_t stream) {
    if (n == 0) return;
    if (fmt == QF_INT8)
        quantize_dispatch<QF_INT8>(w, n, dim, slots, (unsigned int*)slab, R,
                                   stream);
    else
        quantize_dispatch<QF_FP16>(w, n, dim, slots, (unsigned int*)slab, R,
                                   stream);
}

void emb_pool_lookup_q(int fmt, const void* slab, long R, long dim,
                       const i64* values, long nnz, const i64* offsets,
                       long B, int mode, const float* weights, const u64* tk,
                       const int* tv, long cap, const unsigned char* valid,
                       long shard_num, float* out, hipStream_t stream) {
    if (R == 0) {
        fill_f32(out, B * dim, 0.0f, stream);
        return;
    }
    const unsigned int* s = (const unsigned int*)slab;
    if (tk) {
        const PoolHashKeys r{values, tk, tv, cap - 1, R};
        if (fmt == QF_INT8)
            pool_lookup_q_fmt<QF_INT8>(s, dim, nnz, offsets, B, mode,
                                       weights, out, r, stream);
        else
            pool_lookup_q_fmt<QF_FP16>(s, dim, nnz, offsets, B, mode,
                                       weights, out, r, stream);
    } else {
        const PoolArrayKeys r{values, valid, shard_num, cap, R};
        if (fmt == QF_INT8)
            pool_lookup_q_fmt<QF_INT8>(s, dim, nnz, offsets, B, mode,
                                       weights, out, r, stream);
        else
            pool_lookup_q_fmt<QF_FP16>(s, dim, nnz, offsets, B, mode,
                                       weights, out, r, stream);
    }
}

void emb_gather_lookup_q(int fmt, const void* slab, long R, long dim,
                         const i64* keys, long n, const u64* tk,
                         const int* tv, long cap, const unsigned char* valid,
                         long shard_num, float* out, hipStream_t stream) {
    if (n == 0) return;
    if (R == 0) {
        fill_f32(out, n * dim, 0.0f, stream);
        return;
    }
    const unsigned int* s = (const unsigned int*)slab;
    if (tk) {
        const PoolHashKeys r{keys, tk, tv, cap - 1, R};
        if (fmt == QF_INT8)
            gather_lookup_q_fmt<QF_INT8>(s, dim, n, out, r, stream);
        else
            gather_lookup_q_fmt<QF_FP16>(s, dim, n, out, r, stream);
    } else {
        const PoolArrayKeys r{keys, valid, shard_num, cap, R};
        if (fmt == QF_INT8)
            gather_lookup_q_fmt<QF_INT8>(s, dim, n, out, r, stream);
        else
            gather_lookup_q_fmt<QF_FP16>(s, dim, n, out, r, stream);
    }
}

void emb_reduce_bags_weighted_by_inverse(const i64* inverse,
                                         const float* grad_out, long n,
                                         long dim, const int* bag_of,
                                         const float* weights,
                                         const float* bag_scale, long B,
                                         float* ugrads, u64* counts, long u,
                                         hipStream_t stream) {
    reduce_dispatch<true, true>(inverse, grad_out, n, dim, ugrads, counts, u,
                                bag_of, nullptr, B, 0, stream, weights,
                                bag_scale);
}

void emb_pool_wgrad(const float* rows, long R, long dim, const i64* inverse,
                    long nnz, const void* map, int map_kind, long u,
                    const float* weights, const int* bag_of,
                    const float* bag_scale, const float* out,
                    const float* grad_out, long B, int mode, float* dw,
                    hipStream_t stream) {
    if (nnz == 0) return;
#define LAUNCH_WGRAD(G)                                                     \
    do {                                                                    \
        int gg = grid1d(nnz * G);                                           \
        if (map_kind == 2)                                                  \
            k_pool_wgrad<G, int><<<gg, BLOCK, 0, stream>>>(                 \
                rows, R, dim, inverse, nnz, (const int*)map, u, weights,    \
                bag_of, bag_scale, out, grad_out, B, mode, dw);             \
        else                                                                \
            k_pool_wgrad<G, i64><<<gg, BLOCK, 0, stream>>>(                 \
                rows, R, dim, inverse, nnz,                                 \
                map_kind ? (const i64*)map : nullptr, u, weights, bag_of,   \
                bag_scale, out, grad_out, B, mode, dw);                     \
    } while (0)
    if (dim <= 32) LAUNCH_WGRAD(16);
    else LAUNCH_WGRAD(64);
#undef LAUNCH_WGRAD
}

#define LAUNCH_OPT(G, OPT)                                                  \
    k_apply_opt<G, OPT><<<grid1d(n * G), BLOCK, 0, stream>>>(               \
        weights, state, dim, sd, slots, n, grads, counts, c[0], c[1], c[2], \
        c[3], c[4], c[5], c[6], u_dev)

void emb_apply_optimizer(int opt, float* weights, float* state, long dim,
                         long sd, const i64* slots, long n,
                         const float* grads, const u64* counts,
                         const float* c, const int* u_dev,
                         hipStream_t stream) {
    if (n == 0) return;
    if (dim <= 32) {
        const int G = 16;
        switch (opt) {
            case OPT_DEFAULT: LAUNCH_OPT(16, OPT_DEFAULT); break;
            case OPT_ADADELTA: LAUNCH_OPT(16, OPT_ADADELTA); break;
            case OPT_ADAGRAD: LAUNCH_OPT(16, OPT_ADAGRAD); break;
            case OPT_ADAM: LAUNCH_OPT(16, OPT_ADAM); break;
            case OPT_ADAMAX: LAUNCH_OPT(16, OPT_ADAMAX); break;
            case OPT_FTRL: LAUNCH_OPT(16, OPT_FTRL); break;
            case OPT_RMSPROP: LAUNCH_OPT(16, OPT_RMSPROP); break;
            case OPT_SGD: LAUNCH_OPT(16, OPT_SGD); break;
            case OPT_TEST: LAUNCH_OPT(16, OPT_TEST); break;
        }
        (void)G;
    } else {
        const int G = 64;
        switch (opt) {
            case OPT_DEFAULT: LAUNCH_OPT(64, OPT_DEFAULT); break;
            case OPT_ADADELTA: LAUNCH_OPT(64, OPT_ADADELTA); break;
            case OPT_ADAGRAD: LAUNCH_OPT(64, OPT_ADAGRAD); break;
            case OPT_ADAM: LAUNCH_OPT(64, OPT_ADAM); break;
            case OPT_ADAMAX: LAUNCH_OPT(64, OPT_ADAMAX); break;
            case OPT_FTRL: LAUNCH_OPT(64, OPT_FTRL); break;
            case OPT_RMSPROP: LAUNCH_OPT(64, OPT_RMSPROP); break;
            case OPT_SGD: LAUNCH_OPT(64, OPT_SGD); break;
            case OPT_TEST: LAUNCH_OPT(64, OPT_TEST); break;
        }
        (void)G;
    }
}

void emb_mask_tail(i64* keys, float* grads, u64* counts, long n, long dim,
                   const int* u_dev, hipStream_t stream) {
    if (n)
        k_mask_tail<<<grid1d(n * dim), BLOCK, 0, stream>>>(keys, grads,
                                                           counts, n, dim,
                                                           u_dev);
}

void emb_mark_rows(const i64* slots, long n, const unsigned char* mask,
                   const int* u_dev, const int* epoch_dev, int* row_epoch,
                   long R, hipStream_t stream) {
    if (n && R)
        k_mark_rows<<<grid1d(n), BLOCK, 0, stream>>>(slots, n, mask, u_dev,
                                                     epoch_dev, row_epoch, R);
}

long emb_delta_tile_rows() { return DT_TILE; }
long emb_delta_tiles(long R) { return (R + DT_TILE - 1) / DT_TILE; }

void emb_delta_count(const int* row_epoch, long R, int since,
                     const int* nrows_dev, const unsigned char* valid,
                     int* tile_counts, hipStream_t stream) {
    if (R)
        k_delta_count<<<(int)emb_delta_tiles(R), BLOCK, 0, stream>>>(
            row_epoch, R, since, nrows_dev, valid, tile_counts);
}

void emb_delta_compact(const int* row_epoch, long R, int since,
                       const int* nrows_dev, const unsigned char* valid,
                       const int* tile_incl, i64* slots,
                       hipStream_t stream) {
    long T = emb_delta_tiles(R);
    if (R)
        k_delta_compact<<<(int)T, BLOCK, 0, stream>>>(
            row_epoch, R, since, nrows_dev, valid, tile_incl, T, slots);
}

void emb_delta_gather(const float* weights, const float* state, long R,
                      long dim, long sd, const i64* slot_keys,
                      long shard_num, long shard_id, const i64* slots,
                      long nslots, long start, long count, const int* n_dev,
                      i64* keys_out, float* w_out, float* s_out,
                      hipStream_t stream) {
    if (count <= 0 || !R) return;
    if (dim <= 32)
        k_delta_gather<16><<<grid1d(count * 16), BLOCK, 0, stream>>>(
            weights, state, R, dim, sd, slot_keys, shard_num, shard_id,
            slots, nslots, start, count, n_dev, keys_out, w_out, s_out);
    else
        k_delta_gather<64><<<grid1d(count * 64), BLOCK, 0, stream>>>(
            weights, state, R, dim, sd, slot_keys, shard_num, shard_id,
            slots, nslots, start, count, n_dev, keys_out, w_out, s_out);
}

void emb_fault_in(const i64* keys, long n, const int* u_dev, const u64* htk,
                  const int* htv, long hcap, const float* host_w,
                  const float* host_s, float* weights, float* state,
                  long dim, long sd, const i64* slots,
                  unsigned char* new_mask, int* faulted,
                  hipStream_t stream) {
    if (!n) return;
    if (dim <= 32)
        k_fault_in<16><<<grid1d(n * 16), BLOCK, 0, stream>>>(
            keys, n, u_dev, htk, htv, hcap - 1, host_w, host_s, weights,
            state, dim, sd, slots, new_mask, faulted);
    else
        k_fault_in<64><<<grid1d(n * 64), BLOCK, 0, stream>>>(
            keys, n, u_dev, htk, htv, hcap - 1, host_w, host_s, weights,
            state, dim, sd, slots, new_mask, faulted);
}

void emb_spill_rows(const i64* cache_slots, const i64* host_slots, long n,
                    const float* weights, const float* state, float* host_w,
                    float* host_s, long dim, long sd, hipStream_t stream) {
    if (!n) return;
    if (dim <= 32)
        k_spill_rows<16><<<grid1d(n * 16), BLOCK, 0, stream>>>(
            cache_slots, host_slots, n, weights, state, host_w, host_s, dim,
            sd);
    else
        k_spill_rows<64><<<grid1d(n * 64), BLOCK, 0, stream>>>(
            cache_slots, host_slots, n, weights, state, host_w, host_s, dim,
            sd);
}

void emb_gather_host(const i64* keys, long n, const i64* cache_slots,
                     const u64* htk, const int* htv, long hcap,
                     const float* host_w, float* out, long dim,
                     hipStream_t stream) {
    if (!n) return;
    if (dim <= 32)
        k_gather_host<16><<<grid1d(n * 16), BLOCK, 0, stream>>>(
            keys, n, cache_slots, htk, htv, hcap - 1, host_w, out, dim);
    else
        k_gather_host<64><<<grid1d(n * 64), BLOCK, 0, stream>>>(
            keys, n, cache_slots, htk, htv, hcap - 1, host_w, out, dim);
}

void emb_bucketize_pad(const i64* keys, long n, const int* u_dev, long world,
                       long cap, i64* send_keys, int* send_src, int* pos_of,
                       int* counts, int* overflow, hipStream_t stream) {
    long total = world * cap;
    if (total) k_pad_reset<<<grid1d(total), BLOCK, 0, stream>>>(
        (u64*)send_keys, send_src, total, counts, world);
    if (n) k_bucketize_pad<<<grid1d(n), BLOCK, 0, stream>>>(
        keys, n, u_dev, world, cap, send_keys, send_src, pos_of, counts,
        overflow);
}

void emb_gather_pad(const float* ugrads, const u64* counts, long dim,
                    const int* send_src, long total, float* send_p,
                    hipStream_t stream) {
    if (total)
        k_gather_pad<<<grid1d(total * (dim + 1)), BLOCK, 0, stream>>>(
            ugrads, counts, dim, send_src, total, send_p);
}

void emb_scatter_out(const float* rows_recv, const i64* inverse, long n_elems,
                     const int* pos_of, long dim, float* out,
                     hipStream_t stream) {
    if (n_elems)
        k_scatter_out<<<grid1d(n_elems * dim), BLOCK, 0, stream>>>(
            rows_recv, inverse, n_elems, pos_of, dim, out);
}

void emb_split_payload(const float* g2c, long u, long dim, const int* u_dev,
                       float* grads, u64* counts, hipStream_t stream) {
    if (u)
        k_split_payload<<<grid1d(u * (dim + 1)), BLOCK, 0, stream>>>(
            g2c, u, dim, u_dev, grads, counts);
}

void emb_flat_adagrad_f32(float* p, float* accum, const float* g, long n,
                          float lr, float eps, hipStream_t stream) {
    if (n) k_flat_adagrad_f32<<<grid1d(n), BLOCK, 0, stream>>>(p, accum, g, n,
                                                               lr, eps);
}

void emb_flat_adagrad_bf16(float* master, float* accum, const void* g,
                           void* p, long n, float lr, float eps,
                           hipStream_t stream) {
    if (n) k_flat_adagrad_bf16<<<grid1d(n), BLOCK, 0, stream>>>(
        master, accum, (const oebf16*)g, (oebf16*)p, n, lr, eps);
}

void emb_flat_step_scalars(float* sc, float b1, float b2,
                           hipStream_t stream) {
    k_flat_step_scalars<<<1, 64, 0, stream>>>(sc, b1, b2);
}

#define LAUNCH_FLAT(OPT)                                                    \
    do {                                                                    \
        if (bf16)                                                           \
// ... 41 lines not shown
```

### openembedding_amd/ops/dispatch.py

```python

from __future__ import annotations

from typing import Tuple

import torch

from . import require_hip


def _use_hip(t: torch.Tensor) -> bool:
    return t.is_cuda



def unique_inverse(keys: torch.Tensor) -> Tuple[torch.Tensor, torch.Tensor]:
    if keys.numel() == 0:
        return keys.clone(), torch.empty(0, dtype=torch.int64, device=keys.device)
    if _use_hip(keys):
        ext = require_hip()
        if ext is not None:
            return ext.unique_inverse(keys)
    return torch.unique(keys, return_inverse=True)



def reduce_by_inverse(inverse: torch.Tensor, grads: torch.Tensor, u: int
                      ) -> Tuple[torch.Tensor, torch.Tensor]:
    if _use_hip(grads) and grads.dtype == torch.float32:
        ext = require_hip()
        if ext is not None:
            return ext.reduce_by_inverse(inverse, grads, u)
    ugrads = torch.zeros((u, grads.shape[1]), dtype=grads.dtype,
                         device=grads.device)
    ugrads.index_add_(0, inverse, grads)
    counts = torch.bincount(inverse, minlength=u).to(torch.int64)
    return ugrads, counts


def seg_reduce_covers(grads: torch.Tensor) -> bool:
    if not (_use_hip(grads) and grads.dtype == torch.float32):
        return False
    ext = require_hip()
    return ext is not None and grads.shape[1] <= ext.seg_reduce_max_dim()


def reduce_by_index(index, grads: torch.Tensor, u_dev
                    ) -> Tuple[torch.Tensor, torch.Tensor]:
    seg_off, seg_cnt, perm, long_list, n_long = index
    if seg_reduce_covers(grads):
        return require_hip().reduce_by_index(seg_off, seg_cnt, perm,
                                             long_list, n_long, grads, u_dev)
    n = grads.shape[0]
    u = int(u_dev)
    dev = grads.device
    cnt = seg_cnt[:u].to(dev, torch.int64)
    start = seg_off[:u].to(dev, torch.int64)
    uid = torch.repeat_interleave(torch.arange(u, device=dev), cnt)
    first = torch.cumsum(cnt, 0) - cnt
    pos = (torch.arange(uid.numel(), device=dev)
           + torch.repeat_interleave(start - first, cnt))
    elems = perm.to(dev, torch.int64).index_select(0, pos)
    ugrads = torch.zeros((n, grads.shape[1]), dtype=grads.dtype, device=dev)
    ugrads.index_add_(0, uid, grads.index_select(0, elems))
    counts = torch.zeros(n, dtype=torch.int64, device=dev)
    counts[:u] = cnt
    return ugrads, counts



POOL_MODES = {"sum": 0, "mean": 1, "sqrtn": 2}


def _sqrt(t: torch.Tensor) -> torch.Tensor:
    if t.dtype == torch.float32:
        return t.double().sqrt().to(torch.float32)
    return t.sqrt()


def _bag_scale(offsets: torch.Tensor, nnz: int, mode: str,
               dtype: torch.dtype) -> torch.Tensor:
    off = offsets.clamp(0, nnz)
    length = (off[1:] - off[:-1]).clamp(min=0).to(dtype)
    if mode == "sum":
        scale = torch.ones_like(length)
    elif mode == "mean":
        scale = 1.0 / length
    else:
        scale = 1.0 / _sqrt(length)
    return torch.where(length > 0, scale, torch.zeros_like(scale))


def _bag_of(offsets: torch.Tensor, nnz: int) -> torch.Tensor:
    off = offsets.clamp(0, nnz)
    pos = torch.arange(nnz, device=offsets.device)
    bag = torch.bucketize(pos, off[1:].contiguous(), right=True)
    bag = torch.where(bag < off.numel() - 1, bag, torch.full_like(bag, -1))
    return bag.to(torch.int32)


def pool_fwd(rows: torch.Tensor, inverse, row_map, offsets: torch.Tensor,
             mode: str, want_bag_of: bool = True
             ) -> Tuple[torch.Tensor, torch.Tensor]:
    if mode not in POOL_MODES:
        raise ValueError(f"unknown pooling mode {mode!r}")
    if _use_hip(rows) and rows.dtype == torch.float32:
        ext = require_hip()
        if ext is not None:
            return ext.pool_fwd(rows, inverse, row_map, offsets,
                                POOL_MODES[mode], want_bag_of)
    if inverse is not None:
        nnz = inverse.numel()
        idx = inverse
    else:
        nnz = row_map.numel() if row_map is not None else rows.shape[0]
        idx = torch.arange(nnz, device=rows.device)
    if row_map is not None:
        idx = row_map.long().index_select(0, idx)
    elems = rows.index_select(0, idx.clamp(min=0))
    return pool_rows(elems, offsets, mode, live=idx >= 0)


def pool_rows(elems: torch.Tensor, offsets: torch.Tensor, mode: str,
              live: torch.Tensor = None, weights: torch.Tensor = None
              ) -> Tuple[torch.Tensor, torch.Tensor]:
    nnz = elems.shape[0]
    bag_of = _bag_of(offsets, nnz)
    bag = bag_of.long()
    keep = bag >= 0
    if live is not None:
        keep = keep & live
    elems = torch.where(keep.unsqueeze(1), elems, torch.zeros_like(elems))
    if weights is not None:
        w, scale = _weighted_scale(weights.to(elems.dtype), bag,
                                   offsets.numel() - 1, mode)
        elems = elems * w.unsqueeze(1)
    else:
        scale = _bag_scale(offsets, nnz, mode, elems.dtype)
    out = torch.zeros((offsets.numel() - 1, elems.shape[1]),
                      dtype=elems.dtype, device=elems.device)
    out = out.index_add(0, bag.clamp(min=0), elems)
    out = out * scale.unsqueeze(1)
    return out, bag_of


def reduce_bags_by_inverse(inverse: torch.Tensor, grad_out: torch.Tensor,
                           bag_of: torch.Tensor, offsets: torch.Tensor,
                           mode: str, u: int
                           ) -> Tuple[torch.Tensor, torch.Tensor]:
    if mode not in POOL_MODES:
        raise ValueError(f"unknown pooling mode {mode!r}")
    if _use_hip(grad_out) and grad_out.dtype == torch.float32:
        ext = require_hip()
        if ext is not None:
            return ext.reduce_bags_by_inverse(inverse, grad_out, bag_of,
                                              offsets, POOL_MODES[mode], u)
    nnz = inverse.numel()
    bag = bag_of.long()
    live = bag >= 0
    b = bag.clamp(min=0)
    scale = _bag_scale(offsets, nnz, mode, grad_out.dtype)
    g = grad_out.index_select(0, b) * scale.index_select(0, b).unsqueeze(1)
    g = torch.where(live.unsqueeze(1), g, torch.zeros_like(g))
    ugrads = torch.zeros((u, grad_out.shape[1]), dtype=grad_out.dtype,
                         device=grad_out.device)
    ugrads.index_add_(0, inverse, g)
    counts = torch.zeros(u, dtype=torch.int64, device=grad_out.device)
    counts.index_add_(0, inverse, live.to(torch.int64))
    return ugrads, counts



def _weighted_scale(weights: torch.Tensor, bag: torch.Tensor, B: int,
                    mode: str) -> Tuple[torch.Tensor, torch.Tensor]:
    w = torch.where(bag >= 0, weights, torch.zeros_like(weights))
    if mode == "sum":
        return w, torch.ones(B, dtype=w.dtype, device=w.device)
    den = torch.zeros(B, dtype=w.dtype, device=w.device)
    den = den.index_add(0, bag.clamp(min=0), w if mode == "mean" else w * w)
    nz = den != 0
    safe = torch.where(nz, den, torch.ones_like(den))
    scale = 1.0 / safe if mode == "mean" else 1.0 / _sqrt(safe)
    return w, torch.where(nz, scale, torch.zeros_like(scale))


def _gather_rows(rows: torch.Tensor, inverse, row_map, nnz: int
                 ) -> torch.Tensor:
    idx = inverse if inverse is not None \
        else torch.arange(nnz, device=rows.device)
    if row_map is not None:
        idx = row_map.long().index_select(0, idx)
    elems = rows.index_select(0, idx.clamp(min=0))
    return torch.where((idx >= 0).unsqueeze(1), elems,
                       torch.zeros_like(elems))


def pool_fwd_weighted(rows: torch.Tensor, inverse, row_map,
                      offsets: torch.Tensor, weights: torch.Tensor, mode: str
                      ) -> Tuple[torch.Tensor, torch.Tensor, torch.Tensor]:
    if mode not in POOL_MODES:
        raise ValueError(f"unknown pooling mode {mode!r}")
    if _use_hip(rows) and rows.dtype == torch.float32:
        ext = require_hip()
        if ext is not None:
            return ext.pool_fwd_weighted(rows, inverse, row_map, offsets,
                                         weights, POOL_MODES[mode])
    nnz = weights.numel()
    B = offsets.numel() - 1
    elems = _gather_rows(rows, inverse, row_map, nnz)
    bag_of = _bag_of(offsets, nnz)
    bag = bag_of.long()
    w, scale = _weighted_scale(weights.to(rows.dtype), bag, B, mode)
    out = torch.zeros((B, rows.shape[1]), dtype=rows.dtype,
                      device=rows.device)
    out.index_add_(0, bag.clamp(min=0), elems * w.unsqueeze(1))
    return out * scale.unsqueeze(1), bag_of, scale


def reduce_bags_weighted_by_inverse(inverse: torch.Tensor,
                                    grad_out: torch.Tensor,
# ... 171 lines not shown
```

### openembedding_amd/parallel/sharded.py

```python

from __future__ import annotations

import dataclasses
import os
from typing import Dict, List, Optional

import torch

from ..core.variable import VariableShard
from ..ops import dispatch as ops
from ..utils.metrics import REGISTRY, stage_timer
from . import comm


_SEG_REDUCE = os.environ.get("OEAMD_SEG_REDUCE", "1") != "0"


def _unique_bounded(ext, flat: torch.Tensor, field_offsets):
    if not _SEG_REDUCE:
        return (*ext.unique_bounded(flat, field_offsets), None)
    r = ext.unique_bounded_indexed(flat, field_offsets)
    return r[0], r[1], r[2], tuple(r[3:])


class _PaddedPlan:

    def __init__(self, world: int, n: int, device: torch.device):
        slack = float(os.environ.get("OEAMD_A2A_SLACK", "2.0"))
        cap = int(-(-n * slack // world))
        cap = (cap + 255) // 256 * 256
        self.cap = max(1, min(n, cap))
        self.world = world
        total = world * self.cap
        self.send_keys = torch.full((total,), -1, dtype=torch.int64,
                                    device=device)
        self.send_src = torch.full((total,), -1, dtype=torch.int32,
                                   device=device)
        self.pos_of = torch.full((n,), -1, dtype=torch.int32, device=device)
        self.counts = torch.zeros(world, dtype=torch.int32, device=device)
        self.overflow = torch.zeros(1, dtype=torch.int32, device=device)
        self.overflow_host = 0


@dataclasses.dataclass
class PullHandle:

    shape: torch.Size
    unique: Optional[torch.Tensor] = None
    inverse: Optional[torch.Tensor] = None
    order: Optional[torch.Tensor] = None
    send_splits: Optional[List[int]] = None
    recv_splits: Optional[List[int]] = None
    owner_unique: Optional[torch.Tensor] = None
    owner_inverse: Optional[torch.Tensor] = None
    bounded: bool = False
    u_dev: Optional[torch.Tensor] = None
    slots: Optional[torch.Tensor] = None
    owner_u_dev: Optional[torch.Tensor] = None
    owner_slots: Optional[torch.Tensor] = None
    padded: bool = False
    plan: Optional["_PaddedPlan"] = None
    owner_cpu: Optional[tuple] = None
    bag_of: Optional[torch.Tensor] = None
    bag_scale: Optional[torch.Tensor] = None
    pooled_rows: Optional[torch.Tensor] = None
    index: Optional[tuple] = None


class ShardedVariable:

    def __init__(self, shard: VariableShard, storage=None):
        self.shard = shard
        self.storage = storage
        self.world_size = shard.shard_num
        self.rank = shard.shard_id
        self.stat_pull_indices = 0
        self.stat_pull_unique = 0
        self._plans: Dict[int, Optional[_PaddedPlan]] = {}
        self._commits_since_check = 0


    @property
    def meta(self):
        return self.shard.meta

    @property
    def variable_id(self):
        return self.shard.meta.variable_id

    @property
    def embedding_dim(self):
        return self.shard.dim

    def set_initializer(self, category: str, **cfg):
        self.shard.set_initializer(category, **cfg)

    def set_optimizer(self, category: str, **cfg):
        self.shard.set_optimizer(category, **cfg)

    def reserve_rows(self, total_rows: int) -> None:
        fn = getattr(self.shard, "reserve_rows", None)
        if fn is not None:
            fn((int(total_rows) + self.world_size - 1) // self.world_size)


    _force_remote = False

    def pull(self, indices: torch.Tensor, readonly: bool = False,
             field_offsets: torch.Tensor = None):
        bounded_ok = (not readonly
                      and getattr(self.shard, "pull_bounded", None)
                      is not None)
        if field_offsets is not None and not bounded_ok:
            indices = indices + field_offsets
            field_offsets = None
        flat = indices.reshape(-1).to(torch.int64)
        n = flat.numel()
        self.stat_pull_indices += n
        remote = self.world_size > 1 or self._force_remote
        if not remote and bounded_ok:
            return self._pull_local_bounded(indices, flat, field_offsets)
        if remote and not readonly:
            if self._use_padded():
                r = self._pull_remote_padded(indices, flat, field_offsets)
                if r is not None:
                    return r
            if bounded_ok:
                return self._pull_remote_bounded(indices, flat,
                                                 field_offsets)
        unique, inverse = ops.unique_inverse(flat)
        self.stat_pull_unique += unique.numel()
        REGISTRY.add("pull_indices", n)
        REGISTRY.add("pull_unique", unique.numel())
        h = PullHandle(shape=indices.shape, unique=unique, inverse=inverse)
        if self.world_size == 1:
            rows_u = (self.shard.pull_readonly(unique) if readonly
                      else self.shard.pull(unique))
        else:
            rows_u = self._pull_remote(h, readonly)
        out = rows_u.index_select(0, inverse)
        out = out.view(*h.shape, self.shard.dim)
        return out, h

    def _pull_local_bounded(self, indices: torch.Tensor, flat: torch.Tensor,
                            field_offsets: torch.Tensor = None):
        ext = self.shard.ext
        uk_buf, inverse, u_dev, index = _unique_bounded(ext, flat,
                                                        field_offsets)
        out, slots = self.shard.pull_bounded(uk_buf, u_dev, inverse)
        h = PullHandle(shape=indices.shape, unique=uk_buf, inverse=inverse,
                       bounded=True, u_dev=u_dev, slots=slots, index=index)
        return out.view(*indices.shape, self.shard.dim), h

    def pull_pooled(self, values: torch.Tensor, offsets: torch.Tensor,
                    mode: str, readonly: bool = False, pre=None,
                    weights: torch.Tensor = None, wgrad: bool = False):
        flat = values.reshape(-1).to(torch.int64)
        dim = self.shard.dim
        gpu = getattr(self.shard, "pull_bounded", None) is not None
        remote = self.world_size > 1 or self._force_remote
        if gpu and not remote and not readonly and pre is None:
            self.stat_pull_indices += flat.numel()
            ext = self.shard.ext
            uk_buf, inverse, u_dev = ext.unique_bounded(flat, None)
            bag_scale = None
            if weights is None:
                out, slots, bag_of = self.shard.pull_pooled_bounded(
                    uk_buf, u_dev, inverse, offsets, ops.POOL_MODES[mode])
            else:
                out, slots, bag_of, bag_scale = \
                    self.shard.pull_pooled_bounded(
                        uk_buf, u_dev, inverse, offsets,
                        ops.POOL_MODES[mode], weights)
            h = PullHandle(shape=flat.shape, unique=uk_buf, inverse=inverse,
                           bounded=True, u_dev=u_dev, slots=slots,
                           bag_of=bag_of, bag_scale=bag_scale)
            return out, h
        if (gpu and not remote and readonly and pre is None
                and getattr(self.shard, "fused_pooled_readonly", False)):
            self.stat_pull_indices += flat.numel()
            out = self.shard.pull_pooled_readonly(flat, offsets, mode,
                                                  weights)
            return out, PullHandle(shape=flat.shape)
        if pre is None:
            if not gpu:
                flat = flat[:max(0, int(offsets[-1]))]
            pre = self.pull(flat, readonly=readonly)
        rows, h = pre
        rows = rows.reshape(-1, dim)
        if weights is None:
            out, h.bag_of = ops.pool_fwd(rows, None, None, offsets, mode)
            return out, h
        out, h.bag_of, h.bag_scale = ops.pool_fwd_weighted(
            rows, None, None, offsets,
            weights[:rows.shape[0]].contiguous(), mode)
        if wgrad:
            h.pooled_rows = rows
        return out, h

    def _pull_remote_bounded(self, indices: torch.Tensor,
                             flat: torch.Tensor,
                             field_offsets: torch.Tensor = None):
        world = self.world_size
        ext = self.shard.ext
        dev = flat.device
        uk_buf, inverse, u_dev = ext.unique_bounded(flat,
                                                    field_offsets)
        n = uk_buf.numel()
        valid = torch.arange(n, device=dev) < u_dev.to(torch.int64)
        owner = torch.where(valid, uk_buf % world,
                            torch.full_like(uk_buf, world))
        send_counts = torch.bincount(owner, minlength=world + 1)[:world]
        recv_counts = comm.all_to_all_lengths(send_counts)
        both = torch.cat([send_counts, recv_counts]).tolist()
        send_splits, recv_splits = both[:world], both[world:]
        u = int(sum(send_splits))
        self.stat_pull_unique += u
        REGISTRY.add("pull_indices", n)
        REGISTRY.add("pull_unique", u)
        order = torch.argsort(owner, stable=True)[:u]
        send_keys = uk_buf.index_select(0, order)
        recv_keys = comm.all_to_all_v(send_keys, send_splits, recv_splits)
        h = PullHandle(shape=indices.shape, unique=uk_buf, inverse=inverse,
                       order=order, send_splits=send_splits,
                       recv_splits=recv_splits, u_dev=u_dev)
        if recv_keys.numel():
            uk2_buf, inv2, u2_dev = ext.unique_bounded(recv_keys)
            rows_back, slots2 = self.shard.pull_bounded(uk2_buf, u2_dev,
                                                        inv2)
            h.owner_unique = uk2_buf
            h.owner_inverse = inv2
            h.owner_u_dev = u2_dev
            h.owner_slots = slots2
        else:
            h.owner_unique = recv_keys
            rows_back = torch.empty(0, self.shard.dim, dtype=torch.float32,
                                    device=dev)
        rows_sorted = comm.all_to_all_v(rows_back, recv_splits, send_splits)
        rows_u = torch.zeros(n, self.shard.dim, dtype=rows_sorted.dtype,
                             device=dev)
        rows_u.index_copy_(0, order, rows_sorted)
        out = rows_u.index_select(0, inverse)
        return out.view(*indices.shape, self.shard.dim), h


    _padded = None

    def _use_padded(self) -> bool:
        if self._padded is not None:
            return bool(self._padded)
        env = os.environ.get("OEAMD_PADDED_A2A", "auto")
        if env == "0":
            return False
        if env == "1":
            return True
        return getattr(self.shard, "pull_bounded", None) is not None

    def _get_padded_plan(self, n: int,
                         device: torch.device) -> Optional[_PaddedPlan]:
        pair = self._plans.get(n, False)
        if pair is None:
            return None
        if pair is False:
            import torch.distributed as dist
            if comm.dist_ready() and dist.get_world_size() > 1:
                dev = device if comm.backend() == "nccl" else "cpu"
                t = torch.tensor([n, -n], dtype=torch.int64, device=dev)
                dist.all_reduce(t, op=dist.ReduceOp.MIN)
                if int(t[0]) != n or int(-t[1]) != n:
                    self._plans[n] = None
                    return None
            pair = [_PaddedPlan(self.world_size, n, device),
                    _PaddedPlan(self.world_size, n, device), 0]
            self._plans[n] = pair
        pair[2] ^= 1
        return pair[pair[2]]

    def _pull_remote_padded(self, indices: torch.Tensor,
                            flat: torch.Tensor,
                            field_offsets: torch.Tensor = None):
        world = self.world_size
        dim = self.shard.dim
        dev = flat.device
        n = flat.numel()
        plan = self._get_padded_plan(n, dev)
        if plan is None:
            return None
        gpu = getattr(self.shard, "pull_bounded", None) is not None
        index = None
        if gpu:
            ext = self.shard.ext
            uk_buf, inverse, u_dev, index = _unique_bounded(ext, flat,
                                                            field_offsets)
            ext.bucketize_pad(uk_buf, u_dev, world, plan.cap,
                              plan.send_keys, plan.send_src, plan.pos_of,
                              plan.counts, plan.overflow)
        else:
            uk_buf, inverse = ops.unique_inverse(flat)
            u_dev = None
            self._bucketize_pad_torch(uk_buf, plan)
        REGISTRY.add("pull_indices", n)
        REGISTRY.add("pull_wire_keys", plan.send_keys.numel())
        h = PullHandle(shape=indices.shape, unique=uk_buf, inverse=inverse,
                       u_dev=u_dev, padded=True, plan=plan, index=index)
        recv_keys = comm.all_to_all_equal(plan.send_keys, world)
        if gpu:
            uk2_buf, inv2, u2_dev = ext.unique_bounded(recv_keys)
            rows_back, slots2 = self.shard.pull_bounded(uk2_buf, u2_dev,
                                                        inv2)
            h.owner_unique = uk2_buf
            h.owner_inverse = inv2
            h.owner_u_dev = u2_dev
            h.owner_slots = slots2
        else:
            rows_back = self._owner_pull_padded_torch(recv_keys, h)
        rows_recv = comm.all_to_all_equal(rows_back, world)
        if gpu:
            out = ext.scatter_out(rows_recv, inverse, plan.pos_of, n)
        else:
            pos = plan.pos_of.index_select(0, inverse).long()
            out = rows_recv.index_select(0, pos.clamp(min=0))
            out = out.masked_fill((pos < 0).unsqueeze(1), 0.0)
        return out.view(*indices.shape, dim), h

    def _bucketize_pad_torch(self, uk: torch.Tensor,
                             plan: _PaddedPlan) -> None:
        world, cap = plan.world, plan.cap
        plan.send_keys.fill_(-1)
        plan.send_src.fill_(-1)
        plan.pos_of.fill_(-1)
        nz = (uk >= 0).nonzero(as_tuple=True)[0]
        k = uk.index_select(0, nz)
        own = k % world
        order = torch.argsort(own, stable=True)
        k_s, nz_s, own_s = k[order], nz[order], own[order]
        cnt = torch.bincount(own_s, minlength=world)
        start = torch.cumsum(cnt, 0) - cnt
        pos = torch.arange(k_s.numel(), device=uk.device) - start[own_s]
        ok = pos < cap
        slot = (own_s * cap + pos)[ok]
        plan.send_keys[slot] = k_s[ok]
        plan.send_src[slot] = nz_s[ok].to(torch.int32)
        plan.pos_of[nz_s[ok]] = slot.to(torch.int32)
        plan.overflow_host += int((~ok).sum())

    def _owner_pull_padded_torch(self, recv_keys: torch.Tensor,
                                 h: PullHandle) -> torch.Tensor:
        dim = self.shard.dim
        valid = recv_keys >= 0
        vk = recv_keys[valid]
        uk2, inv2 = ops.unique_inverse(vk)
        rows_back = torch.zeros(recv_keys.numel(), dim,
                                dtype=self.shard.dtype,
                                device=recv_keys.device)
        if uk2.numel():
            rows = self.shard.pull(uk2)
            rows_back[valid] = rows.index_select(0, inv2)
        h.owner_cpu = (valid, uk2, inv2)
        return rows_back

    def _apply_padded(self, h: PullHandle, ugrads: torch.Tensor,
                      counts: torch.Tensor) -> None:
        dim = self.shard.dim
        plan = h.plan
        world = self.world_size
        if h.u_dev is not None:
            ext = self.shard.ext
            send_p = ext.gather_pad(ugrads, counts, plan.send_src)
            recv_p = comm.all_to_all_equal(send_p, world)
            g2c, _ = ops.reduce_by_inverse(h.owner_inverse,
                                           recv_p.contiguous(),
                                           h.owner_unique.numel())
            g2, c2 = ext.split_payload(g2c, h.owner_u_dev)
            self.shard.push_slots(h.owner_unique, h.owner_u_dev,
                                  h.owner_slots, g2, c2)
            return
        payload = torch.cat([ugrads,
                             counts.to(ugrads.dtype).unsqueeze(1)], dim=1)
        src = plan.send_src.long()
        send_p = payload.index_select(0, src.clamp(min=0))
        send_p = send_p.masked_fill((src < 0).unsqueeze(1), 0.0)
        recv_p = comm.all_to_all_equal(send_p, world)
        valid, uk2, inv2 = h.owner_cpu
        if uk2.numel() == 0:
            return
        g2c = torch.zeros(uk2.numel(), dim + 1, dtype=recv_p.dtype,
                          device=recv_p.device)
        g2c.index_add_(0, inv2, recv_p[valid])
        g2 = g2c[:, :dim].contiguous()
        c2 = g2c[:, dim].round().to(torch.int64)
        self.shard.push(uk2, g2, c2)

    def check_padded_overflow(self) -> None:
        for pair in self._plans.values():
            if pair is None:
                continue
            for plan in pair[:2]:
                ov = plan.overflow_host + int(plan.overflow.sum().item())
                if ov:
                    raise RuntimeError(
                        f"padded all-to-all overflow on variable "
                        f"{self.variable_id}: {ov} keys were dropped "
                        f"(bucket capacity {plan.cap}/peer). Raise "
                        f"OEAMD_A2A_SLACK (default 2.0) or set "
                        f"OEAMD_PADDED_A2A=0.")

    def _pull_remote(self, h: PullHandle, readonly: bool) -> torch.Tensor:
        with stage_timer("pull", "remote"):
            return self._pull_remote_impl(h, readonly)

    def _pull_remote_impl(self, h: PullHandle, readonly: bool) -> torch.Tensor:
        world = self.world_size
        owner = h.unique % world
        order = torch.argsort(owner, stable=True)
        send_keys = h.unique.index_select(0, order)
        send_counts = torch.bincount(owner, minlength=world)
        recv_counts = comm.all_to_all_lengths(send_counts)
        send_splits = send_counts.tolist()
        recv_splits = recv_counts.tolist()
        recv_keys = comm.all_to_all_v(send_keys, send_splits, recv_splits)
        if (not readonly
                and getattr(self.shard, "pull_bounded", None) is not None
                and recv_keys.numel()):
            uk2_buf, inv2, u2_dev = self.shard.ext.unique_bounded(recv_keys)
            rows_back, slots2 = self.shard.pull_bounded(uk2_buf, u2_dev, inv2)
            h.owner_unique = uk2_buf
            h.owner_inverse = inv2
            h.owner_u_dev = u2_dev
            h.owner_slots = slots2
        else:
            uk2, inv2 = ops.unique_inverse(recv_keys)
            rows_u2 = (self.shard.pull_readonly(uk2) if readonly
                       else self.shard.pull(uk2))
            rows_back = rows_u2.index_select(0, inv2)
            h.owner_unique = uk2
            h.owner_inverse = inv2
        rows_sorted = comm.all_to_all_v(rows_back, recv_splits, send_splits)
        rows_u = torch.empty_like(rows_sorted)
        rows_u.index_copy_(0, order, rows_sorted)
        h.order = order
        h.send_splits = send_splits
        h.recv_splits = recv_splits
        return rows_u


    def push(self, h: PullHandle, grads: torch.Tensor) -> None:
        dim = self.shard.dim
        g = grads.reshape(-1, dim)
        if h.index is not None and ops.seg_reduce_covers(g):
            ugrads, counts = ops.reduce_by_index(h.index, g, h.u_dev)
        else:
            ugrads, counts = ops.reduce_by_inverse(h.inverse, g,
                                                   h.unique.numel())
        self._apply_reduced(h, ugrads, counts)

    def push_pooled(self, h: PullHandle, grad_out: torch.Tensor,
                    offsets: torch.Tensor, mode: str,
                    weights: torch.Tensor = None, out: torch.Tensor = None,
                    wgrad: bool = False):
        g = grad_out.reshape(-1, self.shard.dim)
        if weights is None:
            ugrads, counts = ops.reduce_bags_by_inverse(
                h.inverse, g, h.bag_of, offsets, mode, h.unique.numel())
            self._apply_reduced(h, ugrads, counts)
            return None
        nnz = h.bag_of.numel()
        w = weights[:nnz].contiguous()
        ugrads, counts = ops.reduce_bags_weighted_by_inverse(
            h.inverse, g, h.bag_of, w, h.bag_scale, h.unique.numel())
        dw = None
        if wgrad:
            if h.pooled_rows is not None:
                dw = ops.pool_wgrad(h.pooled_rows, None, None, w, h.bag_of,
                                    h.bag_scale, out, g, mode)
                h.pooled_rows = None
            else:
                dw = self.shard.pool_wgrad_slots(
                    h.inverse, h.slots, w, h.bag_of, h.bag_scale, out, g,
                    ops.POOL_MODES[mode])
            if nnz < weights.numel():
                dw = torch.cat([dw, dw.new_zeros(weights.numel() - nnz)])
        self._apply_reduced(h, ugrads, counts)
        return dw

    def _apply_reduced(self, h: PullHandle, ugrads: torch.Tensor,
                       counts: torch.Tensor) -> None:
        dim = self.shard.dim
        if h.padded:
            self._apply_padded(h, ugrads, counts)
            return
        if h.bounded:
            self.shard.push_slots(h.unique, h.u_dev, h.slots, ugrads, counts)
            return
        if h.send_splits is None:
            self.shard.push(h.unique, ugrads, counts)
            return
        payload = torch.cat([ugrads, counts.to(ugrads.dtype).unsqueeze(1)],
                            dim=1)
        send_p = payload.index_select(0, h.order)
        recv_p = comm.all_to_all_v(send_p, h.send_splits, h.recv_splits)
        u2 = h.owner_unique.numel()
        if u2 == 0:
            return
        g2c, _ = ops.reduce_by_inverse(h.owner_inverse,
                                       recv_p.contiguous(), u2)
        g2 = g2c[:, :dim].contiguous()
        c2 = g2c[:, dim].round().to(torch.int64)
        if h.owner_slots is not None:
            self.shard.push_slots(h.owner_unique, h.owner_u_dev,
                                  h.owner_slots, g2, c2)
        else:
            self.shard.push(h.owner_unique, g2, c2)


    def update_weights(self) -> None:
        self.shard.update_weights()
        if self._plans:
            self._commits_since_check += 1
            if self._commits_since_check >= 64:
                capturing = (torch.cuda.is_available()
                             and torch.cuda.is_current_stream_capturing())
                if not capturing:
                    self._commits_since_check = 0
                    self.check_padded_overflow()


    def pull_dense(self, start: int, count: int,
                   readonly: bool = False) -> torch.Tensor:
        keys = torch.arange(start, start + count, dtype=torch.int64,
                            device=self.shard.device)
        out, _ = self.pull(keys, readonly=readonly)
        return out
```

Baseline: 19.19 million samples/s.

## Fuse unique/assign with gather-init pull and fuse reduce with optimizer apply

Adds a fused pull path that stops the indexed unique after the assign kernel and finishes inverse, index filing and gather/lazy-init in one kernel. Also adds a fused push that defers gradients with their inverted index, then reduces by segment and applies the optimizer in one kernel at commit. Both are meant to cut kernel launches and intermediate buffers (ugrads, counts, the separate gather) per step. The cost is more complex kernels, extra validation, and a fallback when several blocks are pending.

```diff
diff --git a/openembedding_amd/core/tiered_gpu.py b/openembedding_amd/core/tiered_gpu.py
--- a/openembedding_amd/core/tiered_gpu.py
+++ b/openembedding_amd/core/tiered_gpu.py
@@ -119,6 +119,9 @@
         self._last_batch_upper = max(self._last_batch_upper, keys.numel())
         return slots, new_mask
 
+    fused_apply = False
+    fused_pull = False
+
     def push_slots(self, keys_buf, u_dev, slots, grads, counts) -> None:
         if getattr(slots, "_oe_epoch", self._evict_epoch) != self._evict_epoch:
             raise RuntimeError(
diff --git a/openembedding_amd/core/variable_gpu.py b/openembedding_amd/core/variable_gpu.py
--- a/openembedding_amd/core/variable_gpu.py
+++ b/openembedding_amd/core/variable_gpu.py
@@ -54,6 +54,8 @@
     INITIAL_TABLE_CAP = 1 << 16
     INITIAL_ROW_CAP = 1 << 14
     fused_pooled_readonly = True
+    fused_apply = True
+    fused_pull = True
 
     def __init__(self, meta: VariableMeta, shard_id: int = 0, shard_num: int = 1,
                  device: str = "cuda", seed: int = 0):
@@ -194,6 +196,31 @@
                            inverse=inverse, u_dev=u_dev)
         return out, slots
 
+    def pull_bounded_fused(self, flat: torch.Tensor, field_offsets=None,
+                           want_out: bool = True):
+        hash_mode = self.meta.use_hash_table
+        r = self.ext.unique_bounded_assign(
+            flat, field_offsets, None if hash_mode else self.valid_u8,
+            self.shard_num)
+        uk, inverse, u_dev = r[0], r[1], r[2]
+        index = tuple(r[3:8])
+        slot_of, tv, toff, rank, slots, new_mask = r[8:14]
+        if hash_mode:
+            slots, new_mask = self._lookup_or_insert(uk, u_dev)
+        cat, p0, p1, p2 = _init_params(self.initializer)
+        sir = self._state_init_row
+        if sir is None:
+            sir = self._make_state_init_row()
+            self._state_init_row = sir
+        out = self.ext.pull_merged(
+            self.weights, self.state, flat, field_offsets, slot_of, tv, toff,
+            rank, inverse, index[2], slots, new_mask,
+            0 if hash_mode else self.valid_u8.numel(), self.shard_num, cat,
+            p0, p1, p2, self.seed, sir.reshape(-1), want_out, u_dev)
+        if self._tracking and not hash_mode:
+            self._mark(slots, new_mask, u_dev)
+        return out, uk, inverse, u_dev, index, slots
+
     def pull_pooled_bounded(self, keys_buf: torch.Tensor,
                             u_dev: torch.Tensor, inverse: torch.Tensor,
                             offsets: torch.Tensor, mode: int,
@@ -218,6 +245,17 @@
     def push_slots(self, keys_buf, u_dev, slots, grads, counts) -> None:
         self._pending_bounded.append((keys_buf, u_dev, slots, grads, counts))
 
+    def push_index(self, keys_buf, u_dev, slots, grads, index) -> None:
+        self._pending_bounded.append((keys_buf, u_dev, slots, grads, None,
+                                      tuple(index)))
+
+    def _reduce_block(self, block):
+        if len(block) == 5:
+            return block
+        keys_buf, u_dev, slots, grads, _, index = block
+        ugrads, counts = self.ext.reduce_by_index(*index, grads, u_dev)
+        return keys_buf, u_dev, slots, ugrads, counts
+
     def pull_readonly(self, keys: torch.Tensor) -> torch.Tensor:
         slots = self._lookup_readonly(keys)
         empty = torch.empty(0, dtype=torch.uint8, device=self.device)
@@ -255,6 +293,15 @@
         cfg = _opt_cfg_vector(self.optimizer)
         blocks = self._pending_bounded
         self._pending_bounded = []
+        if len(blocks) == 1 and len(blocks[0]) == 6 and not self._pending:
+            keys_buf, u_dev, slots, grads, _, index = blocks[0]
+            self.ext.reduce_apply_by_index(opt_id, self.weights, self.state,
+                                           slots, *index, grads, cfg, u_dev)
+            if self._tracking:
+                self._mark(slots, None, u_dev)
+            blocks = []
+        else:
+            blocks = [self._reduce_block(b) for b in blocks]
         if len(blocks) > 1:
             blocks = [self._merge_bounded(blocks)]
         for keys_buf, u_dev, slots, grads, counts in blocks:
diff --git a/openembedding_amd/ops/csrc/bindings.cpp b/openembedding_amd/ops/csrc/bindings.cpp
--- a/openembedding_amd/ops/csrc/bindings.cpp
+++ b/openembedding_amd/ops/csrc/bindings.cpp
@@ -18,11 +18,25 @@
                         unsigned char*, i64*, i64*, int*, const i64*, int,
                         int*, int*, int*, int*, int*, int*, int*, long, int*,
                         int*, hipStream_t_);
+void emb_unique_indexed_assign(const i64*, long, u64*, int*, long, int*,
+                               unsigned char*, i64*, i64*, int*, const i64*,
+                               int, int*, int*, int*, int*, int*, int*, int*,
+                               long, int*, int*, unsigned char*, long, long,
+                               i64*, unsigned char*, hipStream_t_);
+void emb_pull_merged(float*, float*, long, long, const i64*, const i64*, int,
+                     long, const int*, const int*, const int*, const int*,
+                     i64*, int*, i64*, unsigned char*, int, long, long,
+                     float*, int, float, float, float, u64, const float*,
+                     const int*, hipStream_t_);
 int emb_seg_threshold();
 int emb_seg_max_dim();
 void emb_reduce_by_index(const int*, const int*, const int*, const int*,
                          const int*, long, const float*, long, long,
                          const int*, float*, u64*, hipStream_t_);
+void emb_reduce_apply_by_index(int, const int*, const int*, const int*,
+                               const int*, const int*, long, const float*,
+                               long, long, const int*, const i64*, float*,
+                               float*, long, const float*, hipStream_t_);
 void emb_ht_lookup(u64*, int*, long, const i64*, long, int*, i64*, i64*,
                    unsigned char*, int, const int*, long, hipStream_t_);
 void emb_ht_rehash(const u64*, const int*, long, u64*, int*, long,
@@ -168,7 +182,9 @@
 
 
 std::vector<torch::Tensor> unique_bounded_impl(
-    torch::Tensor keys, OptTensor field_offsets, bool indexed) {
+    torch::Tensor keys, OptTensor field_offsets, bool indexed,
+    bool stop_after_assign = false, OptTensor valid = c10::nullopt,
+    int64_t shard_num = 1) {
     CHECK_GPU(keys); CHECK_CONT(keys);
     TORCH_CHECK(keys.dtype() == torch::kInt64);
     const i64* foff = nullptr;
@@ -212,6 +228,33 @@
     auto seg_off = segs.select(0, 0), seg_cnt = segs.select(0, 1);
     auto perm = segs.select(0, 2), rank = segs.select(0, 3);
     auto n_long = ctr.narrow(0, 16, 1);
+    if (stop_after_assign) {
+        auto slots = torch::empty({n}, opts_i64);
+        auto new_mask = torch::empty({n}, opts_u8);
+        unsigned char* vptr = nullptr;
+        long vcap = 0;
+        if (valid.has_value()) {
+            CHECK_GPU(*valid); CHECK_CONT(*valid);
+            TORCH_CHECK(valid->dtype() == torch::kUInt8 && shard_num >= 1,
+                        "unique_bounded_assign: valid must be uint8");
+            vptr = valid->data_ptr<uint8_t>();
+            vcap = valid->numel();
+        }
+        emb_unique_indexed_assign(
+            keys.data_ptr<i64>(), n, (u64*)tk.data_ptr<i64>(),
+            tv.data_ptr<int>(), cap, slot_of.data_ptr<int>(),
+            is_first.data_ptr<uint8_t>(), uk.data_ptr<i64>(),
+            inverse.data_ptr<i64>(), counter.data_ptr<int>(), foff, F,
+            tct.data_ptr<int>(), tct.data_ptr<int>() + cap,
+            rank.data_ptr<int>(), seg_off.data_ptr<int>(),
+            seg_cnt.data_ptr<int>(), perm.data_ptr<int>(),
+            long_list.data_ptr<int>(), long_cap, ctr.data_ptr<int>(),
+            n_long.data_ptr<int>(), vptr, shard_num, vcap,
+            slots.data_ptr<i64>(), new_mask.data_ptr<uint8_t>(),
+            cur_stream());
+        return {uk, inverse, counter, seg_off, seg_cnt, perm, long_list,
+                n_long, slot_of, tv, tct.select(0, 1), rank, slots, new_mask};
+    }
     emb_unique_indexed(keys.data_ptr<i64>(), n, (u64*)tk.data_ptr<i64>(),
                        tv.data_ptr<int>(), cap, slot_of.data_ptr<int>(),
                        is_first.data_ptr<uint8_t>(), uk.data_ptr<i64>(),
@@ -236,6 +279,90 @@
 unique_bounded_indexed(torch::Tensor keys, OptTensor field_offsets) {
     auto r = unique_bounded_impl(keys, field_offsets, true);
     return {r[0], r[1], r[2], r[3], r[4], r[5], r[6], r[7]};
+}
+
+std::vector<torch::Tensor> unique_bounded_assign(
+    torch::Tensor keys, OptTensor field_offsets, OptTensor valid,
+    int64_t shard_num) {
+    return unique_bounded_impl(keys, field_offsets, true, true, valid,
+                               shard_num);
+}
+
+torch::Tensor pull_merged(torch::Tensor weights, torch::Tensor state,
+                          torch::Tensor keys, OptTensor field_offsets,
+                          torch::Tensor slot_of, torch::Tensor tv,
+                          torch::Tensor toff, torch::Tensor rank,
+                          torch::Tensor inverse, torch::Tensor perm,
+                          torch::Tensor slots, torch::Tensor new_mask,
+                          int64_t array_cap, int64_t shard_num,
+                          int64_t init_cat, double p0, double p1, double p2,
+                          int64_t seed, torch::Tensor state_init_row,
+                          bool want_out, torch::Tensor u_dev) {
+    CHECK_GPU(weights); CHECK_CONT(weights);
+    CHECK_GPU(keys); CHECK_CONT(keys);
+    TORCH_CHECK(weights.dtype() == torch::kFloat32 && weights.dim() == 2
+                && keys.dtype() == torch::kInt64, "pull_merged dtypes");
+    long n = keys.numel();
+    TORCH_CHECK(n < (1L << 31), "pull_merged: n must fit int32");
+    for (const auto* t : {&slot_of, &tv, &toff, &rank, &perm, &u_dev}) {
+        CHECK_GPU(*t); CHECK_CONT(*t);
+        TORCH_CHECK(t->dtype() == torch::kInt32,
+                    "pull_merged: index tensors must be int32");
+    }
+    CHECK_GPU(inverse); CHECK_CONT(inverse); CHECK_GPU(slots);
+    CHECK_CONT(slots); CHECK_GPU(new_mask); CHECK_CONT(new_mask);
+    TORCH_CHECK(inverse.dtype() == torch::kInt64
+                && slots.dtype() == torch::kInt64
+                && new_mask.dtype() == torch::kUInt8, "pull_merged dtypes");
+    TORCH_CHECK(slot_of.numel() == n && rank.numel() == n
+                && perm.numel() == n && inverse.numel() == n
+                && slots.numel() == n && new_mask.numel() == n
+                && tv.numel() == toff.numel() && u_dev.numel() == 1,
+                "pull_merged: scratch does not match keys");
+    TORCH_CHECK(array_cap >= 0 && array_cap <= weights.size(0)
+                && shard_num >= 1, "pull_merged: array_cap beyond the table");
+    const i64* foff = nullptr;
+    int F = 0;
+    if (field_offsets.has_value() && field_offsets->numel()) {
+        CHECK_GPU(*field_offsets); CHECK_CONT(*field_offsets);
+        TORCH_CHECK(field_offsets->dtype() == torch::kInt64
+                    && n % field_offsets->numel() == 0,
+                    "pull_merged: field_offsets");
+        foff = field_offsets->data_ptr<i64>();
+        F = (int)field_offsets->numel();
+    }
+    const c10::cuda::CUDAGuard guard(weights.device());
+    long dim = weights.size(1);
+    long sd = state.numel() ? state.size(1) : 0;
+    if (sd) {
+        CHECK_GPU(state); CHECK_CONT(state);
+        CHECK_GPU(state_init_row); CHECK_CONT(state_init_row);
+        TORCH_CHECK(state.size(0) == weights.size(0)
+                    && state_init_row.numel() >= sd,
+                    "pull_merged: state does not match the table");
+    }
+    torch::Tensor out;
+    float* out_ptr = nullptr;
+    if (want_out) {
+        out = torch::empty({n, dim}, weights.options());
+        out_ptr = out.data_ptr<float>();
+    } else {
+        out = torch::empty({0}, weights.options());
+    }
+    if (init_cat == 1) p1 = p1 - p0;
+    emb_pull_merged(weights.data_ptr<float>(),
+                    sd ? state.data_ptr<float>() : nullptr, dim, sd,
+                    keys.data_ptr<i64>(), foff, F, n,
+                    slot_of.data_ptr<int>(), tv.data_ptr<int>(),
+                    toff.data_ptr<int>(), rank.data_ptr<int>(),
+                    inverse.data_ptr<i64>(), perm.data_ptr<int>(),
+                    slots.data_ptr<i64>(), new_mask.data_ptr<uint8_t>(),
+                    array_cap > 0 ? 1 : 0, shard_num, array_cap, out_ptr,
+                    (int)init_cat, (float)p0, (float)p1, (float)p2,
+                    (u64)seed,
+                    sd ? state_init_row.data_ptr<float>() : nullptr,
+                    u_dev.data_ptr<int>(), cur_stream());
+    return out;
 }
 
 std::tuple<torch::Tensor, torch::Tensor> unique_inverse(torch::Tensor keys) {
@@ -370,6 +497,56 @@
                         u_dev.data_ptr<int>(), ugrads.data_ptr<float>(),
                         (u64*)counts.data_ptr<i64>(), cur_stream());
     return {ugrads, counts};
+}
+
+void reduce_apply_by_index(
+    int64_t opt, torch::Tensor weights, torch::Tensor state,
+    torch::Tensor slots, torch::Tensor seg_off, torch::Tensor seg_cnt,
+    torch::Tensor perm, torch::Tensor long_list, torch::Tensor n_long,
+    torch::Tensor grads, std::vector<double> cfg, torch::Tensor u_dev) {
+    CHECK_GPU(grads); CHECK_CONT(grads);
+    CHECK_GPU(weights); CHECK_CONT(weights);
+    CHECK_GPU(slots); CHECK_CONT(slots);
+    TORCH_CHECK(grads.dtype() == torch::kFloat32 && grads.dim() == 2,
+                "reduce_apply_by_index: grads must be float32 [n, dim]");
+    TORCH_CHECK(weights.dtype() == torch::kFloat32 && weights.dim() == 2,
+                "reduce_apply_by_index: weights must be float32 [R, dim]");
+    TORCH_CHECK(opt >= 0 && opt <= 8, "reduce_apply_by_index: optimizer id");
+    long n = grads.size(0);
+    long dim = grads.size(1);
+    TORCH_CHECK(dim == weights.size(1),
+                "reduce_apply_by_index: grads do not match the table's dim");
+    TORCH_CHECK(dim <= emb_seg_max_dim(),
+                "reduce_apply_by_index: dim above the kernel's ladder");
+    for (const auto* t : {&seg_off, &seg_cnt, &perm, &long_list, &n_long,
+                          &u_dev}) {
+        CHECK_GPU(*t); CHECK_CONT(*t);
+        TORCH_CHECK(t->dtype() == torch::kInt32,
+                    "reduce_apply_by_index: index tensors must be int32");
+    }
+    TORCH_CHECK(seg_off.numel() == n && seg_cnt.numel() == n
+                && perm.numel() == n,
+                "reduce_apply_by_index: index does not match grads");
+    TORCH_CHECK(slots.dtype() == torch::kInt64 && slots.numel() == n,
+                "reduce_apply_by_index: slots must be int64 [n]");
+    TORCH_CHECK(n_long.numel() == 1 && u_dev.numel() == 1);
+    long sd = state.numel() ? state.size(1) : 0;
+    if (sd) {
+        CHECK_GPU(state); CHECK_CONT(state);
+        TORCH_CHECK(state.dtype() == torch::kFloat32
+                    && state.size(0) == weights.size(0),
+                    "reduce_apply_by_index: state must be float32 [R, sd]");
+    }
+    const c10::cuda::CUDAGuard guard(grads.device());
+    float c[7] = {0, 0, 0, 0, 0, 0, 0};
+    for (size_t i = 0; i < cfg.size() && i < 7; ++i) c[i] = (float)cfg[i];
+    emb_reduce_apply_by_index(
+        (int)opt, seg_off.data_ptr<int>(), seg_cnt.data_ptr<int>(),
+        perm.data_ptr<int>(), long_list.data_ptr<int>(),
+        n_long.data_ptr<int>(), long_list.numel(), grads.data_ptr<float>(),
+        n, dim, u_dev.data_ptr<int>(), slots.data_ptr<i64>(),
+        weights.data_ptr<float>(), sd ? state.data_ptr<float>() : nullptr,
+        sd, c, cur_stream());
 }
 
 
@@ -1536,9 +1713,21 @@
           "seg_cnt, perm, long_list, n_long)",
           pybind11::arg("keys"),
           pybind11::arg("field_offsets") = pybind11::none());
+    m.def("unique_bounded_assign", &unique_bounded_assign,
+          "unique_bounded_indexed stopped after the assign kernel (array "
+          "touch inside it when valid is given); pull_merged continues",
+          pybind11::arg("keys"),
+          pybind11::arg("field_offsets") = pybind11::none(),
+          pybind11::arg("valid") = pybind11::none(),
+          pybind11::arg("shard_num") = 1);
+    m.def("pull_merged", &pull_merged,
+          "inverse + index filing + gather/lazy init in one launch");
     m.def("reduce_by_index", &reduce_by_index,
           "grad reduce-by-key with counts through the inverted index "
           "(segmented, no atomics)");
+    m.def("reduce_apply_by_index", &reduce_apply_by_index,
+          "reduce_by_index + apply_optimizer in one launch: the summed "
+          "rows are applied where they are formed");
     m.def("seg_reduce_threshold", &emb_seg_threshold,
           "list length above which a uid is in long_list");
     m.def("seg_reduce_max_dim", &emb_seg_max_dim,
diff --git a/openembedding_amd/ops/csrc/embops.hip b/openembedding_amd/ops/csrc/embops.hip
--- a/openembedding_amd/ops/csrc/embops.hip
+++ b/openembedding_amd/ops/csrc/embops.hip
@@ -207,7 +207,20 @@
     }
 }
 
-template <bool IDX>
+struct UTouch {
+    unsigned char* valid;
+    long shard_num, cap;
+    i64* slots;
+    unsigned char* new_mask;
+};
+
+DEV i64 array_slot(i64 key, long shard_num, long cap) {
+    if (key < 0) return -1;
+    i64 s = shard_num == 1 ? key : key / shard_num;
+    return (s < 0 || s >= cap) ? -1 : s;
+}
+
+template <bool IDX, bool TOUCH = false>
 __global__ void k_unique_assign(const i64* __restrict__ keys, long n,
                                 const int* __restrict__ slot_of,
                                 const unsigned char* __restrict__ is_first,
@@ -216,22 +229,40 @@
                                 int* __restrict__ counter,
                                 i64* __restrict__ inverse,
                                 const i64* __restrict__ foff, int F,
-                                UIdx ix) {
+                                UIdx ix, UTouch tch) {
     const int lane = threadIdx.x & 63;
     const long stride = (long)gridDim.x * blockDim.x;
     long i0 = (long)blockIdx.x * blockDim.x + threadIdx.x;
     u64 ballots[UA_ITERS];
     int sl[IDX ? UA_ITERS : 1], c[IDX ? UA_ITERS : 1];
+    i64 tkey[TOUCH ? UA_ITERS : 1], tslot[TOUCH ? UA_ITERS : 1];
+    unsigned char twas[TOUCH ? UA_ITERS : 1];
     int total = 0;
     #pragma unroll
     for (int t = 0; t < UA_ITERS; ++t) {
         long i = i0 + t * stride;
         if constexpr (IDX) sl[t] = (i < n) ? slot_of[i] : -1;
+        if constexpr (TOUCH) {
+            tkey[t] = -1;
+            if (i < n) {
+                tkey[t] = keys[i];
+                if (foff) tkey[t] += foff[(int)i % F];
+            }
+        }
         bool first = (i < n) && is_first[i];
         ballots[t] = __ballot(first);
         total += __popcll(ballots[t]);
     }
     if (!total) return;
+    if constexpr (TOUCH) {
+        #pragma unroll
+        for (int t = 0; t < UA_ITERS; ++t)
+            tslot[t] = (ballots[t] >> lane & 1ull)
+                ? array_slot(tkey[t], tch.shard_num, tch.cap) : -1;
+        #pragma unroll
+        for (int t = 0; t < UA_ITERS; ++t)
+            twas[t] = tslot[t] >= 0 ? tch.valid[tslot[t]] : 1;
+    }
     int off = 0, wtot = 0;
     if constexpr (IDX) {
         int ctot = 0;
@@ -263,8 +294,16 @@
         if (b & (1ull << lane)) {
             long i = i0 + t * stride;
             int uid = base + __popcll(b & ((1ull << lane) - 1ull));
-            i64 kin = keys[i];
-            if (foff) kin += foff[(int)i % F];
+            i64 kin;
+            if constexpr (TOUCH) {
+                kin = tkey[t];
+                tch.slots[uid] = tslot[t];
+                tch.new_mask[uid] = !twas[t];
+                if (tslot[t] >= 0) tch.valid[tslot[t]] = 1;
+            } else {
+                kin = keys[i];
+                if (foff) kin += foff[(int)i % F];
+            }
             unique_keys[uid] = kin;
             int s;
             if constexpr (IDX) s = sl[t]; else s = slot_of[i];
@@ -465,6 +504,132 @@
         if (nm[t]) {
             for (long j = lane; j < dim; j += G) {
                 float v = init_value(init_cat, p0, p1, p2, seed, key[t],
+                                     (u64)j);
+                wrow[j] = v;
+                if (out) out[g * dim + j] = v;
+            }
+            if (sd > 0) {
+                float* srow = state + (u64)slot[t] * sd;
+                for (long j = lane; j < sd; j += G)
+                    srow[j] = state_init_row[j];
+            }
+        } else if (out) {
+            for (long j = lane; j < dim; j += G)
+                out[g * dim + j] = wrow[j];
+        }
+    }
+}
+
+struct SlotArray {
+    long shard_num, cap;
+    i64* slots_tail;
+    unsigned char* mask_tail;
+    static constexpr bool kTail = true;
+    __device__ __forceinline__ i64 of(i64 key, long) const {
+        return array_slot(key, shard_num, cap);
+    }
+};
+struct SlotMap {
+    const i64* slots;
+    static constexpr bool kTail = false;
+    __device__ __forceinline__ i64 of(i64, long uid) const {
+        return slots[uid];
+    }
+};
+
+template <int G, typename Slot>
+__global__ void k_pull_merged(float* __restrict__ weights,
+                              float* __restrict__ state, long dim, long sd,
+                              const i64* __restrict__ keys,
+                              const i64* __restrict__ foff, int F, long n,
+                              const int* __restrict__ slot_of,
+                              const int* __restrict__ tv,
+                              const int* __restrict__ toff,
+                              const int* __restrict__ rank,
+                              i64* __restrict__ inverse,
+                              int* __restrict__ perm,
+                              const unsigned char* __restrict__ new_mask,
+                              Slot sp, float* __restrict__ out,
+                              int init_cat, float p0, float p1, float p2,
+                              u64 seed,
+                              const float* __restrict__ state_init_row,
+                              const int* __restrict__ u_dev) {
+    const long nthreads = (long)gridDim.x * blockDim.x;
+    const long tid = (long)blockIdx.x * blockDim.x + threadIdx.x;
+    const long stride = nthreads / G;
+    const long g0 = tid / G;
+    const int lane = threadIdx.x % G;
+    long live = *u_dev;
+    live = live < 0 ? 0 : (live > n ? n : live);
+    if constexpr (Slot::kTail) {
+        for (long i = live + tid; i < n; i += nthreads) {
+            sp.slots_tail[i] = -1;
+            sp.mask_tail[i] = 0;
+        }
+    }
+
+    int s[GI_ILP];
+    i64 key[GI_ILP];
+    #pragma unroll
+    for (int t = 0; t < GI_ILP; ++t) {
+        long g = g0 + t * stride;
+        s[t] = 0;
+        key[t] = 0;
+        if (g < n) {
+            s[t] = slot_of[g];
+            key[t] = keys[g];
+            if (foff) key[t] += foff[(int)g % F];
+        }
+    }
+    long uid[GI_ILP];
+    int o[GI_ILP], r[GI_ILP];
+    #pragma unroll
+    for (int t = 0; t < GI_ILP; ++t) {
+        long g = g0 + t * stride;
+        uid[t] = -1;
+        o[t] = 0;
+        r[t] = 0;
+        if (g >= n) continue;
+        if (s[t] >= 0) {
+            uid[t] = tv[s[t]];
+            o[t] = toff[s[t]];
+            r[t] = rank[g];
+        } else if (s[t] == -1) {
+            uid[t] = inverse[g];
+        } else {
+            long wnr = -2 - (long)s[t];
+            uid[t] = wnr < n ? inverse[wnr] : -1;
+        }
+    }
+    i64 slot[GI_ILP];
+    unsigned char nm[GI_ILP];
+    #pragma unroll
+    for (int t = 0; t < GI_ILP; ++t) {
+        long g = g0 + t * stride;
+        if (uid[t] >= live) uid[t] = -1;
+        if (uid[t] < 0) { slot[t] = -1; nm[t] = 0; continue; }
+        if (lane == 0) {
+            if (s[t] != -1) inverse[g] = (i64)uid[t];
+            long p = (long)o[t] + r[t];
+            if (s[t] >= 0 && p >= 0 && p < n) perm[p] = (int)g;
+        }
+        slot[t] = sp.of(key[t], uid[t]);
+        nm[t] = new_mask[uid[t]];
+    }
+    #pragma unroll
+    for (int t = 0; t < GI_ILP; ++t) {
+        long g = g0 + t * stride;
+        if (uid[t] < 0)
+            continue;
+        if (slot[t] < 0) {
+            if (out)
+                for (long j = lane; j < dim; j += G) out[g * dim + j] = 0.0f;
+            continue;
+        }
+        float* wrow = weights + (u64)slot[t] * dim;
+        if (nm[t]) {
+            for (long j = lane; j < dim; j += G) {
+                float v = init_value(init_cat, p0, p1, p2, seed, (u64)key[t],
                                      (u64)j);
                 wrow[j] = v;
                 if (out) out[g * dim + j] = v;
@@ -1316,6 +1481,127 @@
     OPT_ADAMAX = 4, OPT_FTRL = 5, OPT_RMSPROP = 6, OPT_SGD = 7, OPT_TEST = 8
 };
 
+
+template <int G, int OPT>
+DEV float opt_head(float* s, long dim, int lane, float c0,
+                   float c1, float c2) {
+    if (OPT == OPT_ADAM) {
+        const float lr = c0, b1 = c1, b2 = c2;
+        float lr_t = 0.0f;
+        if (lane == 0) {
+            float b1t = s[2 * dim] * b1;
+            float b2t = s[2 * dim + 1] * b2;
+            s[2 * dim] = b1t;
+            s[2 * dim + 1] = b2t;
+            lr_t = lr * sqrtf(1.0f - b2t) / (1.0f - b1t);
+        }
+        return __shfl(lr_t, 0, G);
+    } else if (OPT == OPT_ADAMAX) {
+        const float lr = c0, b1 = c1;
+        float lr_t = 0.0f;
+        if (lane == 0) {
+            float b1t = s[2 * dim] * b1;
+            s[2 * dim] = b1t;
+            lr_t = lr / (1.0f - b1t);
+        }
+        return __shfl(lr_t, 0, G);
+    } else if (OPT == OPT_TEST) {
+        const float flip = c1;
+        float s0 = 0.0f;
+        if (lane == 0) {
+            s0 = flip - s[0];
+            s[0] = s0;
+        }
+        return __shfl(s0, 0, G);
+    }
+    return 0.0f;
+}
+
+template <int OPT>
+DEV void opt_col(float* w, float* s, long dim,
+                 long j, float gj, float head, float cnt, float c0, float c1,
+                 float c2, float c3, float c4, float c5, float c6) {
+    if (OPT == OPT_DEFAULT) {
+        const float lr = c0;
+        w[j] -= lr * gj;
+    } else if (OPT == OPT_ADADELTA) {
+        const float lr = c0, rho = c1, eps = c2;
+        float* accum = s;
+        float* au = s + dim;
+        float a = accum[j] * rho + gj * gj * (1.0f - rho);
+        accum[j] = a;
+        float upd = gj * sqrtf(au[j] + eps) / sqrtf(a + eps);
+        au[j] = au[j] * rho + upd * upd * (1.0f - rho);
+        w[j] -= lr * upd;
+    } else if (OPT == OPT_ADAGRAD) {
+        const float lr = c0, eps = c2;
+        float* accum = s;
+        float a = accum[j] + gj * gj;
+        accum[j] = a;
+        w[j] -= lr * gj / (sqrtf(a) + eps);
+    } else if (OPT == OPT_ADAM) {
+        const float b1 = c1, b2 = c2, eps = c3;
+        float* m = s;
+        float* v = s + dim;
+        const float lr_t = head;
+        float mj = m[j] * b1 + gj * (1.0f - b1);
+        float vj = v[j] * b2 + gj * gj * (1.0f - b2);
+        m[j] = mj; v[j] = vj;
+        w[j] -= lr_t * mj / (sqrtf(vj) + eps);
+    } else if (OPT == OPT_ADAMAX) {
+        const float b1 = c1, b2 = c2, eps = c3;
+        float* m = s;
+        float* v = s + dim;
+        const float lr_t = head;
+        float mj = m[j] * b1 + gj * (1.0f - b1);
+        float vj = fmaxf(fabsf(gj), v[j] * b2);
+        m[j] = mj; v[j] = vj;
+        w[j] -= lr_t * mj / (vj + eps);
+    } else if (OPT == OPT_FTRL) {
+        const float lr = c0, l1 = c1, l2 = c2, l2s = c3, lrp = c4, beta = c5;
+        float* accum = s;
+        float* linear = s + dim;
+        const float adj_l2 = l2 + beta / lr / 2.0f;
+        float wj = w[j];
+        float gg = gj + 2.0f * l2s * wj;
+        float a_old = accum[j];
+        float a_new = a_old + gj * gj;
+        float sigma, quad;
+        if (lrp == -0.5f) {
+            sigma = (sqrtf(a_new) - sqrtf(a_old)) / lr;
+            quad = sqrtf(a_new) / lr + 2.0f * adj_l2;
+        } else {
+            float p = -lrp;
+            sigma = (powf(a_new, p) - powf(a_old, p)) / lr;
+            quad = powf(a_new, p) / lr + 2.0f * adj_l2;
+        }
+        float lin = linear[j] + gg - sigma * wj;
+        linear[j] = lin;
+        accum[j] = a_new;
+        float l1a = fminf(fmaxf(lin, -l1), l1);
+        w[j] = (l1a - lin) / quad;
+    } else if (OPT == OPT_RMSPROP) {
+        const float lr = c0, rho = c1, mom = c2, eps = c3;
+        float* accum = s;
+        float* moment = s + dim;
+        float a = accum[j] * rho + gj * gj * (1.0f - rho);
+        accum[j] = a;
+        float mo = moment[j] * mom + lr * gj / sqrtf(a + eps);
+        moment[j] = mo;
+        w[j] -= mo;
+    } else if (OPT == OPT_SGD) {
+        const float lr = c0, mom = c1;
+        const bool nesterov = c2 != 0.0f;
+        float* moment = s;
+        float mo = moment[j] * mom + lr * gj;
+        moment[j] = mo;
+        w[j] -= nesterov ? (mo * mom + lr * gj) : mo;
+    } else if (OPT == OPT_TEST) {
+        const float lr = c0, s0 = head;
+        w[j] += lr * gj / cnt + s0;
+    }
+}
+
 template <int G, int OPT>
 __global__ void k_apply_opt(float* __restrict__ weights,
                             float* __restrict__ state,
@@ -1336,128 +1622,171 @@
     float* s = state + (u64)slot * sd;
     const float* gr = grads + (u64)g * dim;
 
-    if (OPT == OPT_DEFAULT) {
-        const float lr = c0;
-        if (lr != 0.0f)
-            for (long j = lane; j < dim; j += G) w[j] -= lr * gr[j];
-    } else if (OPT == OPT_ADADELTA) {
-        const float lr = c0, rho = c1, eps = c2;
-        float* accum = s;
-        float* au = s + dim;
-        for (long j = lane; j < dim; j += G) {
-            float gj = gr[j];
-            float a = accum[j] * rho + gj * gj * (1.0f - rho);
-            accum[j] = a;
-            float upd = gj * sqrtf(au[j] + eps) / sqrtf(a + eps);
-            au[j] = au[j] * rho + upd * upd * (1.0f - rho);
-            w[j] -= lr * upd;
-        }
-    } else if (OPT == OPT_ADAGRAD) {
-        const float lr = c0, eps = c2;
-        float* accum = s;
-        for (long j = lane; j < dim; j += G) {
-            float gj = gr[j];
-            float a = accum[j] + gj * gj;
-            accum[j] = a;
-            w[j] -= lr * gj / (sqrtf(a) + eps);
-        }
-    } else if (OPT == OPT_ADAM) {
-        const float lr = c0, b1 = c1, b2 = c2, eps = c3;
-        float* m = s;
-        float* v = s + dim;
-        float lr_t = 0.0f;
-        if (lane == 0) {
-            float b1t = s[2 * dim] * b1;
-            float b2t = s[2 * dim + 1] * b2;
-            s[2 * dim] = b1t;
-            s[2 * dim + 1] = b2t;
-            lr_t = lr * sqrtf(1.0f - b2t) / (1.0f - b1t);
-        }
-        lr_t = __shfl(lr_t, 0, G);
-        for (long j = lane; j < dim; j += G) {
-            float gj = gr[j];
-            float mj = m[j] * b1 + gj * (1.0f - b1);
-            float vj = v[j] * b2 + gj * gj * (1.0f - b2);
-            m[j] = mj; v[j] = vj;
-            w[j] -= lr_t * mj / (sqrtf(vj) + eps);
-        }
-    } else if (OPT == OPT_ADAMAX) {
-        const float lr = c0, b1 = c1, b2 = c2, eps = c3;
-        float* m = s;
-        float* v = s + dim;
-        float lr_t = 0.0f;
-        if (lane == 0) {
-            float b1t = s[2 * dim] * b1;
-            s[2 * dim] = b1t;
-            lr_t = lr / (1.0f - b1t);
-        }
-        lr_t = __shfl(lr_t, 0, G);
-        for (long j = lane; j < dim; j += G) {
-            float gj = gr[j];
-            float mj = m[j] * b1 + gj * (1.0f - b1);
-            float vj = fmaxf(fabsf(gj), v[j] * b2);
-            m[j] = mj; v[j] = vj;
-            w[j] -= lr_t * mj / (vj + eps);
-        }
-    } else if (OPT == OPT_FTRL) {
-        const float lr = c0, l1 = c1, l2 = c2, l2s = c3, lrp = c4, beta = c5;
-        float* accum = s;
-        float* linear = s + dim;
-        const float adj_l2 = l2 + beta / lr / 2.0f;
-        for (long j = lane; j < dim; j += G) {
-            float gj = gr[j];
-            float wj = w[j];
-            float gg = gj + 2.0f * l2s * wj;
-            float a_old = accum[j];
-            float a_new = a_old + gj * gj;
-            float sigma, quad;
-            if (lrp == -0.5f) {
-                sigma = (sqrtf(a_new) - sqrtf(a_old)) / lr;
-                quad = sqrtf(a_new) / lr + 2.0f * adj_l2;
-            } else {
-                float p = -lrp;
-                sigma = (powf(a_new, p) - powf(a_old, p)) / lr;
-                quad = powf(a_new, p) / lr + 2.0f * adj_l2;
+    if (OPT == OPT_DEFAULT && c0 == 0.0f) return;
+    const float head = opt_head<G, OPT>(s, dim, lane, c0, c1, c2);
+    const float cnt = OPT == OPT_TEST ? (float)counts[g] : 0.0f;
+    for (long j = lane; j < dim; j += G)
+        opt_col<OPT>(w, s, dim, j, gr[j], head, cnt, c0, c1, c2, c3, c4, c5,
+                     c6);
+}
+
+template <int G, int CF, int OPT>
+__global__ __launch_bounds__(SEG_BLOCK)
+void k_seg_reduce_apply(const int* __restrict__ seg_off,
+                        const int* __restrict__ seg_cnt,
+                        const int* __restrict__ perm,
+                        const int* __restrict__ long_list,
+                        const int* __restrict__ n_long, long long_cap,
+                        int long_blocks, const float* __restrict__ grads,
+                        long n, long dim, const int* __restrict__ u_dev,
+                        const i64* __restrict__ slots,
+                        float* __restrict__ weights,
+                        float* __restrict__ state, long sd,
+                        float c0, float c1, float c2, float c3, float c4,
+                        float c5, float c6) {
+    __shared__ float red[SEG_BLOCK / 64][G * CF];
+    __shared__ float tot[G * CF];
+    const int lane = threadIdx.x % G;
+    long u = *u_dev;
+    u = u < 0 ? 0 : (u > n ? n : u);
+    if (OPT == OPT_DEFAULT && c0 == 0.0f) return;
+
+    if ((int)blockIdx.x < long_blocks) {
+        long nl = *n_long;
+        nl = nl < 0 ? 0 : (nl > long_cap ? long_cap : nl);
+        const int group = threadIdx.x / G;
+        constexpr int NG = SEG_BLOCK / G;
+        for (long b = blockIdx.x; b < nl; b += long_blocks) {
+            const int uid = long_list[b];
+            int off = 0, cnt = 0;
+            i64 slot = -1;
+            if (uid >= 0 && uid < u) {
+                seg_range(seg_off, seg_cnt, uid, n, off, cnt);
+                slot = slots[uid];
             }
-            float lin = linear[j] + gg - sigma * wj;
-            linear[j] = lin;
-            accum[j] = a_new;
-            float l1a = fminf(fmaxf(lin, -l1), l1);
-            w[j] = (l1a - lin) / quad;
-        }
-    } else if (OPT == OPT_RMSPROP) {
-        const float lr = c0, rho = c1, mom = c2, eps = c3;
-        float* accum = s;
-        float* moment = s + dim;
-        for (long j = lane; j < dim; j += G) {
-            float gj = gr[j];
-            float a = accum[j] * rho + gj * gj * (1.0f - rho);
-            accum[j] = a;
-            float mo = moment[j] * mom + lr * gj / sqrtf(a + eps);
-            moment[j] = mo;
-            w[j] -= mo;
-        }
-    } else if (OPT == OPT_SGD) {
-        const float lr = c0, mom = c1;
-        const bool nesterov = c2 != 0.0f;
-        float* moment = s;
-        for (long j = lane; j < dim; j += G) {
-            float gj = gr[j];
-            float mo = moment[j] * mom + lr * gj;
-            moment[j] = mo;
-            w[j] -= nesterov ? (mo * mom + lr * gj) : mo;
-        }
-    } else if (OPT == OPT_TEST) {
-        const float lr = c0, flip = c1;
-        float s0 = 0.0f;
-        if (lane == 0) {
-            s0 = flip - s[0];
-            s[0] = s0;
-        }
-        s0 = __shfl(s0, 0, G);
-        float cnt = (float)counts[g];
-        for (long j = lane; j < dim; j += G)
-            w[j] += lr * gr[j] / cnt + s0;
+            if (cnt <= SEG_T) continue;
+            float acc[CF];
+            #pragma unroll
+            for (int c = 0; c < CF; ++c) acc[c] = 0.0f;
+            int e[LR_ILP], en[LR_ILP];
+            #pragma unroll
+            for (int t = 0; t < LR_ILP; ++t)
+                en[t] = (group * LR_ILP + t < cnt)
+                            ? perm[off + group * LR_ILP + t] : -1;
+            for (long base = group * LR_ILP; base < cnt;
+                 base += NG * LR_ILP) {
+                #pragma unroll
+                for (int t = 0; t < LR_ILP; ++t) {
+                    e[t] = (en[t] < 0 || en[t] >= n) ? -1 : en[t];
+                    const long nx = base + NG * LR_ILP + t;
+                    en[t] = (nx < cnt) ? perm[off + nx] : -1;
+                }
+                float v[LR_ILP][CF];
+                #pragma unroll
+                for (int t = 0; t < LR_ILP; ++t)
+                    #pragma unroll
+                    for (int c = 0; c < CF; ++c)
+                        v[t][c] = (e[t] >= 0 && lane + c * G < dim)
+                            ? grads[(u64)e[t] * dim + lane + c * G] : 0.0f;
+                #pragma unroll
+                for (int t = 0; t < LR_ILP; ++t)
+                    #pragma unroll
+                    for (int c = 0; c < CF; ++c) acc[c] += v[t][c];
+            }
+            #pragma unroll
+            for (int d = G; d < 64; d <<= 1)
+                #pragma unroll
+                for (int c = 0; c < CF; ++c)
+                    acc[c] += __shfl_xor(acc[c], d, 64);
+            if ((threadIdx.x & 63) < G) {
+                #pragma unroll
+                for (int c = 0; c < CF; ++c)
+                    red[threadIdx.x / 64][lane + c * G] = acc[c];
+            }
+            __syncthreads();
+            if (threadIdx.x < G * CF) {
+                float s = 0.0f;
+                #pragma unroll
+                for (int w = 0; w < SEG_BLOCK / 64; ++w)
+                    s += red[w][threadIdx.x];
+                tot[threadIdx.x] = s;
+            }
+            __syncthreads();
+            if (threadIdx.x < G && slot >= 0) {
+                float* w = weights + (u64)slot * dim;
+                float* s = state + (u64)slot * sd;
+                const float head = opt_head<G, OPT>(s, dim, lane, c0, c1, c2);
+                #pragma unroll
+                for (int c = 0; c < CF; ++c)
+                    if (lane + c * G < dim)
+                        opt_col<OPT>(w, s, dim, lane + c * G,
+                                     tot[lane + c * G], head, (float)cnt, c0,
+                                     c1, c2, c3, c4, c5, c6);
+            }
+        }
+        return;
+    }
+
+    const long ngroups = (long)(gridDim.x - long_blocks) * (SEG_BLOCK / G);
+    const long g0 = ((long)(blockIdx.x - long_blocks) * SEG_BLOCK
+                     + threadIdx.x) / G;
+    int off[SR_ILP], cnt[SR_ILP], e0[SR_ILP];
+    i64 slot[SR_ILP];
+    #pragma unroll
+    for (int t = 0; t < SR_ILP; ++t) {
+        long uid = g0 + t * ngroups;
+        off[t] = 0;
+        cnt[t] = 0;
+        slot[t] = -1;
+        if (uid < u) {
+            seg_range(seg_off, seg_cnt, uid, n, off[t], cnt[t]);
+            slot[t] = slots[uid];
+        }
+    }
+    #pragma unroll
+    for (int t = 0; t < SR_ILP; ++t) {
+        e0[t] = (cnt[t] > 0 && cnt[t] <= SEG_T) ? perm[off[t]] : -1;
+        if (e0[t] < 0 || e0[t] >= n) e0[t] = -1;
+    }
+    float acc[SR_ILP][CF];
+    #pragma unroll
+    for (int t = 0; t < SR_ILP; ++t)
+        #pragma unroll
+        for (int c = 0; c < CF; ++c)
+            acc[t][c] = (e0[t] >= 0 && lane + c * G < dim)
+                ? grads[(u64)e0[t] * dim + lane + c * G] : 0.0f;
+    #pragma unroll
+    for (int t = 0; t < SR_ILP; ++t) {
+        long uid = g0 + t * ngroups;
+        if (uid >= u || cnt[t] > SEG_T) continue;
+        for (int k = 1; k < cnt[t]; k += SR_ILP) {
+            int e[SR_ILP];
+            #pragma unroll
+            for (int q = 0; q < SR_ILP; ++q) {
+                e[q] = (k + q < cnt[t]) ? perm[off[t] + k + q] : -1;
+                if (e[q] < 0 || e[q] >= n) e[q] = -1;
+            }
+            float v[SR_ILP][CF];
+            #pragma unroll
+            for (int q = 0; q < SR_ILP; ++q)
+                #pragma unroll
+                for (int c = 0; c < CF; ++c)
+                    v[q][c] = (e[q] >= 0 && lane + c * G < dim)
+                        ? grads[(u64)e[q] * dim + lane + c * G] : 0.0f;
+            #pragma unroll
+            for (int q = 0; q < SR_ILP; ++q)
+                #pragma unroll
+                for (int c = 0; c < CF; ++c) acc[t][c] += v[q][c];
+        }
+        if (slot[t] < 0) continue;
+        float* w = weights + (u64)slot[t] * dim;
+        float* s = state + (u64)slot[t] * sd;
+        const float head = opt_head<G, OPT>(s, dim, lane, c0, c1, c2);
+        #pragma unroll
+        for (int c = 0; c < CF; ++c)
+            if (lane + c * G < dim)
+                opt_col<OPT>(w, s, dim, lane + c * G, acc[t][c], head,
+                             (float)cnt[t], c0, c1, c2, c3, c4, c5, c6);
     }
 }
 
@@ -2064,7 +2393,7 @@
                           int* slot_of, unsigned char* is_first,
                           i64* unique_keys, i64* inverse, int* counter,
                           const i64* foff, int F, const UIdx& ix,
-                          hipStream_t stream) {
+                          hipStream_t stream, const UTouch* tch = nullptr) {
     {
         long mx = cap > n ? cap : n;
         k_unique_reset<IDX><<<(int)((mx + 255) / 256), 256, 0, stream>>>(
@@ -2075,9 +2404,20 @@
         keys, n, tk, mask, slot_of, is_first, foff, F, ix);
     int ga = grid1d((n + UA_ITERS - 1) / UA_ITERS);
     int gi = grid1d((n + UI_ILP - 1) / UI_ILP);
+    if (tch) {
+        if (IDX && tch->valid)
+            k_unique_assign<IDX, IDX><<<ga, BLOCK, 0, stream>>>(
+                keys, n, slot_of, is_first, tv, unique_keys, counter,
+                inverse, foff, F, ix, *tch);
+        else
+            k_unique_assign<IDX><<<ga, BLOCK, 0, stream>>>(
+                keys, n, slot_of, is_first, tv, unique_keys, counter,
+                inverse, foff, F, ix, UTouch{});
+        return;
+    }
     k_unique_assign<IDX><<<ga, BLOCK, 0, stream>>>(
         keys, n, slot_of, is_first, tv, unique_keys, counter, inverse, foff,
-        F, ix);
+        F, ix, UTouch{});
     k_unique_inverse<IDX><<<gi, BLOCK, 0, stream>>>(n, slot_of, tv, inverse,
                                                     ix);
 }
@@ -2104,6 +2444,50 @@
             off_counter, n_long, long_cap};
     unique_launch<true>(keys, n, tk, tv, cap, slot_of, is_first, unique_keys,
                         inverse, counter, foff, F, ix, stream);
+}
+
+void emb_unique_indexed_assign(const i64* keys, long n, u64* tk, int* tv,
+                               long cap, int* slot_of,
+                               unsigned char* is_first, i64* unique_keys,
+                               i64* inverse, int* counter, const i64* foff,
+                               int F, int* tcount, int* toff, int* rank,
+                               int* seg_off, int* seg_cnt, int* perm,
+                               int* long_list, long long_cap,
+                               int* off_counter, int* n_long,
+                               unsigned char* valid, long shard_num,
+                               long table_cap, i64* slots,
+                               unsigned char* new_mask, hipStream_t stream) {
+    UIdx ix{tcount, toff, rank, seg_off, seg_cnt, perm, long_list,
+            off_counter, n_long, long_cap};
+    UTouch tch{valid, shard_num, table_cap, slots, new_mask};
+    unique_launch<true>(keys, n, tk, tv, cap, slot_of, is_first, unique_keys,
+                        inverse, counter, foff, F, ix, stream, &tch);
+}
+
+void emb_pull_merged(float* weights, float* state, long dim, long sd,
+                     const i64* keys, const i64* foff, int F, long n,
+                     const int* slot_of, const int* tv, const int* toff,
+                     const int* rank, i64* inverse, int* perm, i64* slots,
+                     unsigned char* new_mask, int array, long shard_num,
+                     long table_cap, float* out, int init_cat, float p0,
+                     float p1, float p2, u64 seed,
+                     const float* state_init_row, const int* u_dev,
+                     hipStream_t stream) {
+    if (n == 0) return;
+    long npg = (n + GI_ILP - 1) / GI_ILP;
+#define LAUNCH_PM(G, SP)                                                    \
+    k_pull_merged<G><<<grid1d(npg * G), BLOCK, 0, stream>>>(                \
+        weights, state, dim, sd, keys, foff, F, n, slot_of, tv, toff, rank, \
+        inverse, perm, new_mask, SP, out, init_cat, p0, p1, p2, seed,       \
+        state_init_row, u_dev)
+    if (array) {
+        SlotArray sp{shard_num, table_cap, slots, new_mask};
+        if (dim <= 32) LAUNCH_PM(16, sp); else LAUNCH_PM(64, sp);
+    } else {
+        SlotMap sp{slots};
+        if (dim <= 32) LAUNCH_PM(16, sp); else LAUNCH_PM(64, sp);
+    }
+#undef LAUNCH_PM
 }
 
 int emb_seg_threshold() { return SEG_T; }
@@ -2388,6 +2772,42 @@
     }
 }
 
+void emb_reduce_apply_by_index(int opt, const int* seg_off,
+                               const int* seg_cnt, const int* perm,
+                               const int* long_list, const int* n_long,
+                               long long_cap, const float* grads, long n,
+                               long dim, const int* u_dev, const i64* slots,
+                               float* weights, float* state, long sd,
+                               const float* c, hipStream_t stream) {
+    if (n == 0) return;
+    int lb = (int)(long_cap < SEG_LONG_BLOCKS ? long_cap : SEG_LONG_BLOCKS);
+    long groups = (n + SR_ILP - 1) / SR_ILP;
+#define LAUNCH_SEG_OPT(G, CF, OPT)                                          \
+    k_seg_reduce_apply<G, CF, OPT>                                          \
+        <<<lb + cdiv(groups * G, SEG_BLOCK), SEG_BLOCK, 0, stream>>>(       \
+            seg_off, seg_cnt, perm, long_list, n_long, long_cap, lb, grads, \
+            n, dim, u_dev, slots, weights, state, sd, c[0], c[1], c[2],     \
+            c[3], c[4], c[5], c[6])
+#define SWITCH_SEG_OPT(G, CF)                                               \
+    switch (opt) {                                                          \
+        case OPT_DEFAULT: LAUNCH_SEG_OPT(G, CF, OPT_DEFAULT); break;        \
+        case OPT_ADADELTA: LAUNCH_SEG_OPT(G, CF, OPT_ADADELTA); break;      \
+        case OPT_ADAGRAD: LAUNCH_SEG_OPT(G, CF, OPT_ADAGRAD); break;        \
+        case OPT_ADAM: LAUNCH_SEG_OPT(G, CF, OPT_ADAM); break;              \
+        case OPT_ADAMAX: LAUNCH_SEG_OPT(G, CF, OPT_ADAMAX); break;          \
+        case OPT_FTRL: LAUNCH_SEG_OPT(G, CF, OPT_FTRL); break;              \
+        case OPT_RMSPROP: LAUNCH_SEG_OPT(G, CF, OPT_RMSPROP); break;        \
+        case OPT_SGD: LAUNCH_SEG_OPT(G, CF, OPT_SGD); break;                \
+        case OPT_TEST: LAUNCH_SEG_OPT(G, CF, OPT_TEST); break;              \
+    }
+    if (dim <= 16) { SWITCH_SEG_OPT(16, 1) }
+    else if (dim <= 32) { SWITCH_SEG_OPT(16, 2) }
+    else if (dim <= 64) { SWITCH_SEG_OPT(64, 1) }
+    else { SWITCH_SEG_OPT(64, 2) }
+#undef SWITCH_SEG_OPT
+#undef LAUNCH_SEG_OPT
+}
+
 void emb_mask_tail(i64* keys, float* grads, u64* counts, long n, long dim,
                    const int* u_dev, hipStream_t stream) {
     if (n)
diff --git a/openembedding_amd/ops/dispatch.py b/openembedding_amd/ops/dispatch.py
--- a/openembedding_amd/ops/dispatch.py
+++ b/openembedding_amd/ops/dispatch.py
@@ -65,6 +65,24 @@
     counts = torch.zeros(n, dtype=torch.int64, device=dev)
     counts[:u] = cnt
     return ugrads, counts
+
+
+def reduce_apply_by_index(opt_id: int, weights: torch.Tensor,
+                          state: torch.Tensor, slots: torch.Tensor, index,
+                          grads: torch.Tensor, cfg, u_dev) -> None:
+    ext = require_hip() if _use_hip(grads) else None
+    if ext is None or weights.dtype != torch.float32:
+        raise NotImplementedError(
+            "reduce_apply_by_index serves float32 GPU tables; other "
+            "variables reduce at push time and commit through their shard")
+    grads = grads.contiguous()
+    if seg_reduce_covers(grads):
+        ext.reduce_apply_by_index(opt_id, weights, state, slots, *index,
+                                  grads, list(cfg), u_dev)
+        return
+    ugrads, counts = reduce_by_index(index, grads, u_dev)
+    ext.apply_optimizer(opt_id, weights, state, slots, ugrads, counts,
+                        list(cfg), u_dev)
 
 
 
diff --git a/openembedding_amd/parallel/sharded.py b/openembedding_amd/parallel/sharded.py
--- a/openembedding_amd/parallel/sharded.py
+++ b/openembedding_amd/parallel/sharded.py
@@ -14,6 +14,8 @@
 
 
 _SEG_REDUCE = os.environ.get("OEAMD_SEG_REDUCE", "1") != "0"
+_FUSED_APPLY = os.environ.get("OEAMD_FUSED_APPLY", "1") != "0"
+_FUSED_PULL = os.environ.get("OEAMD_FUSED_PULL", "1") != "0"
 
 
 def _unique_bounded(ext, flat: torch.Tensor, field_offsets):
@@ -145,9 +147,14 @@
     def _pull_local_bounded(self, indices: torch.Tensor, flat: torch.Tensor,
                             field_offsets: torch.Tensor = None):
         ext = self.shard.ext
-        uk_buf, inverse, u_dev, index = _unique_bounded(ext, flat,
-                                                        field_offsets)
-        out, slots = self.shard.pull_bounded(uk_buf, u_dev, inverse)
+        if (_FUSED_PULL and _SEG_REDUCE and flat.numel()
+                and getattr(self.shard, "fused_pull", False)):
+            out, uk_buf, inverse, u_dev, index, slots = \
+                self.shard.pull_bounded_fused(flat, field_offsets)
+        else:
+            uk_buf, inverse, u_dev, index = _unique_bounded(ext, flat,
+                                                            field_offsets)
+            out, slots = self.shard.pull_bounded(uk_buf, u_dev, inverse)
         h = PullHandle(shape=indices.shape, unique=uk_buf, inverse=inverse,
                        bounded=True, u_dev=u_dev, slots=slots, index=index)
         return out.view(*indices.shape, self.shard.dim), h
@@ -447,6 +454,12 @@
     def push(self, h: PullHandle, grads: torch.Tensor) -> None:
         dim = self.shard.dim
         g = grads.reshape(-1, dim)
+        if (_FUSED_APPLY and h.index is not None and h.bounded
+                and not h.padded and g.is_contiguous()
+                and getattr(self.shard, "fused_apply", False)
+                and ops.seg_reduce_covers(g)):
+            self.shard.push_index(h.unique, h.u_dev, h.slots, g, h.index)
+            return
         if h.index is not None and ops.seg_reduce_covers(g):
             ugrads, counts = ops.reduce_by_index(h.index, g, h.u_dev)
         else:
```

Result: faster. 20.06 million samples/s (median of 6 runs) (+4.5%).
